# AdmiralenOla/Scoary

Hardware: AMD Instinct MI355X
Metric: gene x permutation Fisher tests/sec (higher is better)
Workload: dtype u32 bit-words (bit-sliced adders / AND + popcount), f64 for Fisher p; 1 GPU; cfg3: 50000 genes x 2000 isolates x 10 traits, --permute 10000 per GPU; counts + Fisher + label permutations + exceedance counts; gene_kind=config, gene_order=config, gene_partition=every rank its own genes (weak scaling), genes_per_gpu=50000, genes_total=50000, isolates=2000, traits=10, permutations=10000, parallelism=gene-shard x1, hip_graph=False, hip_graph_auto=False, label_tiles=generated on every rank, exchange=none (single GPU)

## Files before the change

### __graft_entry__.py

```python
import os
import subprocess
import sys

ROOT = os.path.dirname(os.path.abspath(__file__))
if ROOT not in sys.path:
    sys.path.insert(0, ROOT)

CSRC = os.path.join(ROOT, "scoary_amd", "csrc")
HIP_SRCS = [os.path.join(CSRC, f) for f in ("scoary_context.hip", "scoary_assoc.hip",
                                            "scoary_lists.hip", "scoary_listbuild.hip",
                                            "scoary_mfma.hip", "scoary_labels.hip", "scoary_tree.hip", "scoary_scipy.hip",
                                            "scoary_minp.hip", "scoary_cmh.hip", "scoary_cmh_exact.hip")]
HIP_LIB = os.path.join(ROOT, "scoary_amd", "csrc", "libscoary_hip.so")
HIP_RESOURCES = os.path.join(ROOT, "scoary_amd", "csrc", "libscoary_hip.resources.json")
HIPCC_FLAGS = ["--offload-arch=gfx950", "-O3", "-std=c++17", "-fPIC", "-shared",
               "-ffp-contract=off", "-I" + os.path.join(ROOT, "include"),
               "-Rpass-analysis=kernel-resource-usage"]


def _stale(target, sources):
    if not os.path.exists(target):
        return True
    t = os.path.getmtime(target)
    return any(os.path.getmtime(s) > t for s in sources)


def _hip_deps():
    import glob
    return (HIP_SRCS + glob.glob(os.path.join(CSRC, "*.hpp")) + glob.glob(os.path.join(CSRC, "*.inc"))
            + glob.glob(os.path.join(ROOT, "include", "*.h")))


def parse_resource_usage(text):
    import re
    out, cur = {}, None
    for line in text.splitlines():
        m = re.search(r"remark: (?:\s*)Function Name: (\S+)", line)
        if m:
            cur = out.setdefault(m.group(1), {})
            continue
        m = re.search(r"remark:\s+([A-Za-z ]+?)(?: \[[^\]]*\])?: (\d+)", line)
        if m and cur is not None:
            cur[m.group(1).strip()] = int(m.group(2))
    return out


def _rule(name, count, exclude=None, cap=None, no_static_lds=False):
    return dict(name=name, exclude=exclude, count=count, cap=cap, no_static_lds=no_static_lds)


LIST_RULES = (
    _rule("k_permute_lists", 4, cap=(("VGPRs",), 128), no_static_lds=True),
    _rule("k_permute_seglists", 1, cap=(("VGPRs",), 128), no_static_lds=True),
)
RESOURCE_RULES = LIST_RULES + (
    _rule("k_permute_mfma", 1, cap=(("VGPRs", "AGPRs"), 256)),
    _rule("k_permute_minp", 9, exclude="chunked", cap=(("VGPRs",), 128)),
    _rule("k_permute_minp_chunked", 1),
    _rule("k_stepdown_minp", 18, exclude="chunked", cap=(("VGPRs",), 128)),
    _rule("k_stepdown_minp_chunked", 2),
)
CMH_RULES = (
    _rule("k_cmhE", 1, cap=(("VGPRs",), 128)),
    _rule("k_cmh_support", 1, cap=(("VGPRs",), 128)),
    _rule("k_cmh_fill", 1, cap=(("VGPRs",), 128)),
)
CMH_EXACT_RULES = (
    _rule("k_cmh_exact", 1, cap=(("VGPRs",), 48)),
)
CMH_EXACT_ODDS_RULES = (
    _rule("k_cmh_odds_exact", 1, cap=(("VGPRs",), 152)),
)
CMH_HOMOG_RULES = (
    _rule("k_cmh_homog", 1, cap=(("VGPRs",), 64)),
)


def check_kernel_resources(res, rules=LIST_RULES):
    bad = []
    for rule in rules:
        hit = {k: v for k, v in res.items()
               if rule["name"] in k and not (rule["exclude"] and rule["exclude"] in k)}
        if len(hit) != rule["count"]:
            bad.append("expected %d %s instance%s, compiler reported %d"
                       % (rule["count"], rule["name"], "" if rule["count"] == 1 else "s", len(hit)))
        for name, r in hit.items():
            if r.get("ScratchSize", 0) or r.get("VGPRs Spill", 0) or r.get("SGPRs Spill", 0):
                bad.append("%s: scratch %s, VGPR spills %s, SGPR spills %s" % (
                    name, r.get("ScratchSize"), r.get("VGPRs Spill"), r.get("SGPRs Spill")))
            if rule["cap"]:
                fields, most = rule["cap"]
                if sum(r.get(f, 999) for f in fields) > most:
                    bad.append("%s: %s > %d" % (name, " + ".join("%d %s" % (r.get(f, 999), f) for f in fields), most))
            if rule["no_static_lds"] and r.get("LDS Size", 0) != 0:
                bad.append("%s: static LDS %d bytes (label tile must sit at LDS address 0)" % (name, r["LDS Size"]))
    for name, r in res.items():
        if r.get("ScratchSize", 0) and "k_fisher" not in name:
            bad.append("%s uses %d bytes of scratch per lane" % (name, r["ScratchSize"]))
    if bad:
        raise RuntimeError("libscoary_hip.so: kernel resource check failed:\n  " + "\n  ".join(bad))


def check_ctr_banks():
    import re
    txt = open(os.path.join(CSRC, "scoary_ctr_regs.inc")).read()
    regs = re.findall(r"SCOARY_CTR\((\d+),\s*(\d+),\s*\"v(\d+)\"\)", txt)
    if not regs:
        raise RuntimeError("scoary_ctr_regs.inc: no SCOARY_CTR entries found")
    seen = set()
    for w, k, r in regs:
        w, k, r = int(w), int(k), int(r)
        if r in seen:
            raise RuntimeError("scoary_ctr_regs.inc: v%d pinned twice" % r)
        seen.add(r)
        if (r - w) % 2 == 0:
            raise RuntimeError("scoary_ctr_regs.inc: counter plane (%d, %d) in v%d shares a bank "
                               "with its row words" % (w, k, r))


def check_isa_banks(hipcc, max_frac=0.06):
    import re
    import tempfile
    llvm = os.path.join(os.environ.get("ROCM_PATH", "/opt/rocm"), "lib", "llvm", "bin")
    out = {}
    with tempfile.TemporaryDirectory() as tmp:
        fat, co = os.path.join(tmp, "lists.o"), os.path.join(tmp, "lists.gfx950.o")
        flags = [f for f in HIPCC_FLAGS if f not in ("-shared", "-fPIC") and not f.startswith("-Rpass")]
        subprocess.check_call([hipcc] + flags + ["--cuda-device-only", "-c", "-o", fat,
                                                os.path.join(CSRC, "scoary_lists.hip")],
                              cwd=ROOT, stderr=subprocess.DEVNULL)
        subprocess.check_call([os.path.join(llvm, "clang-offload-bundler"), "--unbundle", "--type=o",
                               "--input=" + fat, "--targets=hipv4-amdgcn-amd-amdhsa--gfx950",
                               "--output=" + co])
        dis = subprocess.run([os.path.join(llvm, "llvm-objdump"), "-d", co], check=True,
                             stdout=subprocess.PIPE, text=True).stdout
    name = None
    for line in dis.splitlines():
        m = re.match(r"[0-9a-f]+ <(\S+)>:", line)
        if m:
            name = m.group(1) if ("k_permute_lists" in m.group(1) or "k_permute_seglists" in m.group(1)) else None
            if name:
                out[name] = [0, 0]
            continue
        if name:
            m = re.search(r"v_bitop3_b32 v\d+, v(\d+), v(\d+), v\d+", line)
            if m:
                out[name][0] += 1
                out[name][1] += int(m.group(1)) % 4 == int(m.group(2)) % 4
    bad = ["%s: %d of %d v_bitop3_b32 have src0 and src1 in one VGPR bank" % (k, same, n)
           for k, (n, same) in out.items() if n == 0 or same > max_frac * n]
    nlists = sum("k_permute_lists" in k for k in out)
    nseg = sum("k_permute_seglists" in k for k in out)
    if nlists != 4 or nseg != 1:
        bad.append("expected 4 k_permute_lists + 1 k_permute_seglists instances in the ISA, found %d + %d"
                   % (nlists, nseg))
    if bad:
        raise RuntimeError("libscoary_hip.so: ISA bank check failed:\n  " + "\n  ".join(bad))
    return out


def build(force=False):
    import json
    if force or _stale(HIP_LIB, _hip_deps()) or not os.path.exists(HIP_RESOURCES):
        hipcc = os.environ.get("HIPCC", "hipcc")
        cmd = [hipcc] + HIPCC_FLAGS + HIP_SRCS + ["-o", HIP_LIB]
        proc = subprocess.run(cmd, cwd=ROOT, stderr=subprocess.PIPE, text=True)
        if proc.returncode != 0:
            sys.stderr.write(proc.stderr)
            raise subprocess.CalledProcessError(proc.returncode, cmd)
        res = parse_resource_usage(proc.stderr)
        try:
            check_kernel_resources(res, RESOURCE_RULES + CMH_RULES + CMH_EXACT_RULES + CMH_EXACT_ODDS_RULES +
                                   CMH_HOMOG_RULES)
            check_ctr_banks()
            for k, (n, same) in check_isa_banks(hipcc).items():
                res.setdefault(k, {}).update({"v_bitop3_b32": n, "v_bitop3_b32 src0/src1 same bank": same})
        except RuntimeError:
            os.remove(HIP_LIB)
            raise
        with open(HIP_RESOURCES, "w") as f:
            json.dump(res, f, indent=1, sort_keys=True)
    io_src = os.path.join(ROOT, "scoary_amd", "csrc", "scoary_io.cpp")
    io_lib = os.path.join(ROOT, "scoary_amd", "csrc", "libscoary_io.so")
    if force or _stale(io_lib, [io_src, os.path.join(ROOT, "include", "scoary_io.h")]):
        subprocess.check_call([os.environ.get("CXX", "g++"), "-O3", "-std=c++17", "-fPIC",
                               "-shared", "-Wall", "-fopenmp", "-ffp-contract=off", "-I" + os.path.join(ROOT, "include"), io_src,
                               "-o", io_lib], cwd=ROOT)
    from oracle import oracle as orc
    orc.build(force=force)
    import scoary_amd
    from scoary_amd import _abi
    if not os.path.exists(_abi.LIB_PATH):
        raise RuntimeError("build() did not produce " + _abi.LIB_PATH)


def smoke():
    import numpy as np
    import torch
    from oracle import oracle as orc
    from scoary_amd.engine import AssociationEngine, pack_bits_rows

    assert torch.cuda.is_available(), "smoke() needs cuda:0"
    torch.cuda.set_device(0)
    rng = np.random.default_rng(5)
    G, N, T, P, seed = 700, 333, 3, 200, 77
    genes = (rng.random((G, N)) < rng.uniform(0.02, 0.98, (G, 1))).astype(np.uint8)
    genes[3] = 0
    genes[4] = 1
    traits = (rng.random((T, N)) < 0.4).astype(np.uint8)
    traits[1, ::29] = 2

    eng = AssociationEngine(0)
    gm = eng.pack_dense(genes)
    tb = pack_bits_rows((traits == 1).astype(np.uint8))
    mb = pack_bits_rows((traits != 2).astype(np.uint8))
    trv, mkv = eng.vecrows(tb, N), eng.vecrows(mb, N)
    dense = eng.associate(gm, trv, mkv, permutations=P, seed=seed, use_lists=False)
    eng.build_lists(gm)
    res = eng.associate(gm, trv, mkv, permutations=P, seed=seed, use_lists=True)
    torch.cuda.synchronize()
    assert np.array_equal(res["r"].cpu().numpy(), dense["r"].cpu().numpy()), \
        "list-driven and dense permutation kernels disagree"

    gb = orc.pack_rows(genes)
    want = orc.counts_packed(gb, tb, mb).transpose(1, 0, 2)
    got = res["counts"].cpu().numpy()
    assert np.array_equal(got, want), "contingency counts differ from the oracle"
    o, p = orc.fisher_many(want.reshape(-1, 4))
    assert np.max(np.abs(res["p"].cpu().numpy().ravel() - p)) < 1e-12, "Fisher p differs"
    r = orc.permute_r(gb, tb, mb, N, P, seed).T
    got_r = res["r"].cpu().numpy().view(np.uint32)
    assert np.array_equal(got_r, r), "permutation exceedance counts differ from the oracle"
    print("smoke ok: %d genes x %d isolates x %d traits x %d permutations, "
          "counts/r bit-exact, max|dp| < 1e-12" % (G, N, T, P))


if __name__ == "__main__":
    build()
    if len(sys.argv) > 1 and sys.argv[1] == "smoke":
        smoke()
```

### include/scoary_hip.h

```cpp
#ifndef SCOARY_HIP_H
#define SCOARY_HIP_H

#include <stdint.h>

#ifdef __cplusplus
extern "C" {
#endif

#define SCOARY_ABI_VERSION 11

#define SCOARY_OK 0
#define SCOARY_ERR_ARG (-1)
#define SCOARY_ERR_HIP (-2)
#define SCOARY_ERR_SIZE (-3)
#define SCOARY_ERR_DEVICE (-4)

typedef struct scoary_ctx *scoary_handle;
typedef void *scoary_stream_t;

int scoary_abi_version(void);

int scoary_create(int device, scoary_handle *out);
void scoary_destroy(scoary_handle h);
const char *scoary_last_error(scoary_handle h);
// ... 10 lines not shown

int scoary_counts(scoary_handle h, const uint32_t *d_tiled,
                  const uint32_t *d_traits, const uint32_t *d_masks, int64_t G,
                  int64_t T, int64_t N, int32_t *d_counts, int32_t *d_margins,
                  scoary_stream_t stream);
int64_t scoary_counts_traits_per_pass(int64_t T);
int64_t scoary_trait_plan_bytes(int64_t T, int64_t N);
int scoary_trait_plan(scoary_handle h, const uint32_t *d_traits, const uint32_t *d_masks,
                      int64_t T, int64_t N, int32_t *d_margins, int32_t *d_mask_class,
                      void *d_plan, scoary_stream_t stream);
int scoary_counts_planned(scoary_handle h, const uint32_t *d_tiled, const void *d_plan,
                          const int32_t *d_margins, int64_t G, int64_t T, int64_t N,
                          int32_t *d_counts, scoary_stream_t stream);

int scoary_fisher(scoary_handle h, const int32_t *d_tables, int64_t M,
                  double *d_p, double *d_or, uint32_t *d_crit,
                  scoary_stream_t stream);
int64_t scoary_fisher_scipy_max_isolates(void);
int scoary_fisher_scipy(scoary_handle h, const int32_t *d_tables, int64_t M, double *d_p,
                        uint64_t *d_skipped, scoary_stream_t stream);
int scoary_fisher_lists(scoary_handle h, const int32_t *d_tables, int64_t T, int64_t G,
                        const int32_t *d_lorder, const uint8_t *d_lflipped,
                        double *d_p, double *d_or, uint32_t *d_crit, uint32_t *d_lcrit,
                        scoary_stream_t stream);

int64_t scoary_perm_max_isolates(void);
int scoary_perm_generate(scoary_handle h, const uint32_t *d_masks,
                         const int32_t *d_margins, int64_t T, int64_t N,
                         int64_t P, int64_t perm_base, int64_t trait_base,
                         uint64_t seed, uint32_t *d_perms, scoary_stream_t stream);

int scoary_permute(scoary_handle h, const uint32_t *d_tiled,
                   const uint32_t *d_perms, const uint32_t *d_crit, int64_t G,
                   int64_t T, int64_t N, int64_t P, uint32_t *d_r,
                   scoary_stream_t stream);

int scoary_permute_seq(scoary_handle h, const uint32_t *d_tiled, const uint32_t *d_perms,
                       const uint32_t *d_crit, const uint32_t *d_thr, int64_t G, int64_t T,
                       int64_t N, int64_t P, int64_t perm_base, uint32_t *d_r,
                       uint32_t *d_nstop, scoary_stream_t stream);

int64_t scoary_minp_fill_scratch_bytes(int64_t entries);
int scoary_minp_plan(scoary_handle h, const int32_t *d_counts, int64_t T, int64_t G, int64_t *d_off,
                     int32_t *d_lo, int64_t *entries_out, scoary_stream_t stream);
int scoary_minp_fill(scoary_handle h, const int32_t *d_counts, const int64_t *d_off,
                     const int32_t *d_lo, int64_t T, int64_t G, int64_t entries, void *d_scratch,
                     double *d_tab, scoary_stream_t stream);
int scoary_permute_minp(scoary_handle h, const uint32_t *d_tiled, const uint32_t *d_perms,
                        const int64_t *d_off, const int32_t *d_lo, const double *d_tab, int64_t G,
                        int64_t T, int64_t N, int64_t P, int64_t perm_base, int64_t minp_stride,
                        double *d_minp, scoary_stream_t stream);

int64_t scoary_stepdown_chunks(scoary_handle h, int64_t G, int64_t T, int64_t P);
int64_t scoary_stepdown_scratch_bytes(scoary_handle h, int64_t G, int64_t T, int64_t N, int64_t P);
int scoary_permute_stepdown(scoary_handle h, const uint32_t *d_tiled, const uint32_t *d_perms,
                            const int64_t *d_off, const int32_t *d_lo, const double *d_tab,
                            const int32_t *d_order, const double *d_psorted, int64_t G, int64_t T,
                            int64_t N, int64_t P, int64_t perm_base, int64_t minp_stride,
                            double *d_minp, uint32_t *d_c, void *d_scratch, scoary_stream_t stream);

int64_t scoary_list_tiles_words(int64_t N, int64_t P, int64_t T);
int64_t scoary_list_tile_words(int64_t N);
int64_t scoary_list_max_isolates(void);
int64_t scoary_list_segments(int64_t N);
int scoary_list_params(int64_t N, int64_t *out5);
int scoary_perm_generate_tiles(scoary_handle h, const uint32_t *d_masks,
                               const int32_t *d_margins, int64_t T, int64_t N, int64_t P,
                               int64_t perm_base, int64_t trait_base, uint64_t seed,
                               uint32_t *d_tiles, scoary_stream_t stream);
int scoary_perm_generate_tiles_range(scoary_handle h, const uint32_t *d_masks,
                                     const int32_t *d_margins, int64_t T, int64_t N, int64_t P,
                                     int64_t perm_base, int64_t trait_base, uint64_t seed,
                                     int64_t first_tile, int64_t n_tiles, uint32_t *d_tiles,
                                     scoary_stream_t stream);
int scoary_perm_max_strata(void);
int64_t scoary_perm_strata_max_isolates(void);
int scoary_strata_margins(scoary_handle h, const uint32_t *d_labels, const uint32_t *d_masks,
                          const uint16_t *d_strata, int64_t T, int64_t N, int64_t S,
                          int32_t *d_smargins, scoary_stream_t stream);
int scoary_perm_generate_strata(scoary_handle h, const uint32_t *d_masks, const uint16_t *d_strata,
                                const int32_t *d_members, const int32_t *d_offsets,
                                const int32_t *d_smargins, int64_t T, int64_t N, int64_t S, int64_t P,
                                int64_t perm_base, int64_t trait_base, uint64_t seed,
                                uint32_t *d_perms, scoary_stream_t stream);
int scoary_perm_generate_tiles_strata_range(scoary_handle h, const uint32_t *d_masks,
                                            const uint16_t *d_strata, const int32_t *d_members,
                                            const int32_t *d_offsets, const int32_t *d_smargins,
                                            int64_t T, int64_t N, int64_t S, int64_t P,
                                            int64_t perm_base, int64_t trait_base, uint64_t seed,
                                            int64_t first_tile, int64_t n_tiles, uint32_t *d_tiles,
                                            scoary_stream_t stream);
int64_t scoary_cmh_scratch_bytes(int64_t N);
int scoary_cmh(scoary_handle h, const uint32_t *d_tiled, const uint32_t *d_labels, const uint32_t *d_masks,
               const uint16_t *d_strata, const int32_t *d_members, const int32_t *d_offsets,
               const int32_t *d_smargins, int64_t G, int64_t T, int64_t N, int64_t S, double *d_stat,
               double *d_p, double *d_odds, double *d_e2, double *d_var, int32_t *d_a, uint32_t *d_crit,
               int32_t *d_scounts, void *d_scratch, scoary_stream_t stream);
int scoary_cmh_minp_plan(scoary_handle h, const uint32_t *d_tiled, const uint32_t *d_masks,
                         const uint16_t *d_strata, const int32_t *d_members, const int32_t *d_offsets,
                         const int32_t *d_smargins, int64_t G, int64_t T, int64_t N, int64_t S,
                         void *d_scratch, int64_t *d_off, int32_t *d_lo, int64_t *entries_out,
                         scoary_stream_t stream);
int scoary_cmh_minp_fill(scoary_handle h, const double *d_e2, const double *d_var, const int64_t *d_off,
                         const int32_t *d_lo, int64_t T, int64_t G, int64_t entries, double *d_tab,
                         scoary_stream_t stream);
int64_t scoary_cmh_exact_max_isolates(void);
int scoary_cmh_exact(scoary_handle h, const uint32_t *d_tiled, const uint32_t *d_masks, const uint16_t *d_strata,
                     const int32_t *d_members, const int32_t *d_offsets, const int32_t *d_smargins, int64_t G,
                     int64_t T, int64_t N, int64_t S, const int32_t *d_a, const uint32_t *d_crit,
                     const int64_t *d_off, const int32_t *d_lo, int64_t entries, double *d_p, double *d_p_region,
                     double *d_tab, void *d_scratch, scoary_stream_t stream);
int scoary_cmh_exact_odds(scoary_handle h, const uint32_t *d_tiled, const uint32_t *d_masks,
                          const uint16_t *d_strata, const int32_t *d_members, const int32_t *d_offsets,
                          const int32_t *d_smargins, int64_t G, int64_t T, int64_t N, int64_t S,
                          const int32_t *d_a, const int64_t *d_off, const int32_t *d_lo, int64_t entries, double half,
                          double *d_or, double *d_or_lo, double *d_or_hi, void *d_scratch,
                          scoary_stream_t stream);
int scoary_cmh_homogeneity(scoary_handle h, const uint32_t *d_tiled, const uint32_t *d_labels,
                           const uint32_t *d_masks, const uint16_t *d_strata, const int32_t *d_members,
                           const int32_t *d_offsets, const int32_t *d_smargins, int64_t G, int64_t T, int64_t N,
                           int64_t S, const double *d_odds, double *d_stat_bd, double *d_stat_tarone, int32_t *d_df,
                           double *d_p, void *d_scratch, scoary_stream_t stream);
int64_t scoary_permute_lists_scratch_bytes(int64_t G, int64_t T, int64_t N, int64_t P);
int scoary_permute_lists(scoary_handle h, const uint32_t *d_tiles, const uint32_t *d_lidx,
                         int64_t entries, const int32_t *d_lstart, const int32_t *d_lngroups,
                         const int32_t *d_lorder, const uint8_t *d_lflipped,
                         const uint32_t *d_crit, const uint32_t *d_lcrit,
                         const int32_t *d_margins, void *d_scratch,
                         int64_t G, int64_t T, int64_t N, int64_t P, uint32_t *d_r,
                         int accumulate, scoary_stream_t stream);

#define SCOARY_MFMA_ROUTE_NONE 0
#define SCOARY_MFMA_ROUTE_ALL 1
#define SCOARY_MFMA_ROUTE_AUTO 2
int64_t scoary_mfma_max_isolates(void);
int64_t scoary_mfma_panels_bytes(int64_t G, int64_t N);
int64_t scoary_mfma_bfrag_bytes(int64_t N, int64_t P, int64_t T);
int64_t scoary_mfma_breakeven_entries(void);
int scoary_mfma_panels_build(scoary_handle h, const uint32_t *d_tiled, int64_t G, int64_t N,
                             const int32_t *d_order, const uint8_t *d_flipped, void *d_panels,
                             scoary_stream_t stream);
int scoary_set_mfma_route(scoary_handle h, int mode);
int64_t scoary_mfma_route(scoary_handle h, const int64_t *block_start, int64_t G, int64_t T,
                          int64_t N, int64_t P);
int scoary_mfma_plan(int num_cu, int64_t k_split, int64_t T, int64_t P, int64_t *out);
int scoary_permute_hybrid(scoary_handle h, const uint32_t *d_tiles, const uint32_t *d_lidx,
                          int64_t entries, const int32_t *d_lstart, const int32_t *d_lngroups,
                          const int32_t *d_lorder, const uint8_t *d_lflipped,
                          const uint32_t *d_crit, const uint32_t *d_lcrit,
                          const int32_t *d_margins, void *d_scratch,
                          int64_t G, int64_t T, int64_t N, int64_t P, uint32_t *d_r,
                          int accumulate, const void *d_panels, void *d_bfrag, int64_t k_split,
                          int64_t routed_entries, scoary_stream_t stream);

int64_t scoary_lists_scratch_bytes(int64_t G, int64_t N);
int64_t scoary_lists_slack_entries(void);
int scoary_lists_plan(scoary_handle h, const uint32_t *d_tiled, int64_t G, int64_t N,
                      void *d_scratch, int32_t *d_start, int32_t *d_ngroups, int32_t *d_order,
                      uint8_t *d_flipped, int64_t *entries_out, scoary_stream_t stream);
int scoary_lists_fill(scoary_handle h, const uint32_t *d_tiled, int64_t G, int64_t N,
                      const void *d_scratch, const int32_t *d_order, const uint8_t *d_flipped,
                      int64_t entries, uint32_t *d_idx, scoary_stream_t stream);


int scoary_hamming(scoary_handle h, const uint32_t *d_tiled, const uint32_t *d_vecrows,
                   int64_t R, int64_t N, int32_t *d_out, scoary_stream_t stream);

int64_t scoary_upgma_scratch_bytes(int64_t n);
int scoary_upgma(scoary_handle h, const int32_t *d_counts, int64_t n, int64_t ncols, void *d_scratch,
                 int32_t *d_merges, int32_t *d_status, scoary_stream_t stream);

int scoary_gather_bits(scoary_handle h, const uint32_t *d_rows, int64_t R, int64_t Wsrc,
                       const int32_t *d_index, int64_t K, uint32_t *d_out,
                       scoary_stream_t stream);

int scoary_tree_pairs(scoary_handle h, const int32_t *d_ops, int64_t nops, int64_t stack_depth,
                      const uint32_t *d_gene_bits, const uint32_t *d_label_bits, int64_t G,
                      int64_t L, int64_t K, int32_t *d_out, scoary_stream_t stream);

int scoary_tree_permute(scoary_handle h, const int32_t *d_ops, int64_t nops,
                        int64_t stack_depth, const uint32_t *d_gene_bits,
                        const uint32_t *d_label_bits, int64_t G, int64_t L, int64_t K,
                        const int32_t *d_obs, uint8_t *d_exceed, scoary_stream_t stream);

int scoary_row_hash(scoary_handle h, const uint32_t *d_tiled, const uint32_t *d_masks,
                    int64_t G, int64_t T, int64_t N, uint64_t *d_out, scoary_stream_t stream);

int scoary_pack_records(scoary_handle h, const int32_t *d_counts, const double *d_p,
                        const double *d_odds, const uint32_t *d_r, const uint32_t *d_nstop,
                        int64_t M, uint32_t *d_rec, scoary_stream_t stream);

int scoary_gather(scoary_handle h, void *rccl_dl, void *comm, const void *d_send, void *d_recv,
                  int64_t bytes, int rank, int nranks, int root, scoary_stream_t stream);

typedef struct scoary_graph *scoary_graph_t;
int scoary_graph_begin(scoary_handle h, scoary_stream_t stream);
int scoary_graph_end(scoary_handle h, scoary_stream_t stream, scoary_graph_t *out);
int scoary_graph_launch(scoary_handle h, scoary_graph_t g, scoary_stream_t stream);
void scoary_graph_destroy(scoary_graph_t g);

int scoary_set_timing(scoary_handle h, int enabled);
int scoary_last_kernel_ms(scoary_handle h, const char *kernel, double *ms_out);

#ifdef __cplusplus
}
#endif
#endif
```

### scoary_amd/_abi.py

```python
import ctypes
import os

_HERE = os.path.dirname(os.path.abspath(__file__))
LIB_PATH = os.environ.get("SCOARY_HIP_LIB") or os.path.join(_HERE, "csrc", "libscoary_hip.so")
HEADER_PATH = os.path.join(os.path.dirname(_HERE), "include", "scoary_hip.h")

ABI_VERSION = 11
PERM_MAX_STRATA = 1024
PERM_STRATA_MAX_ISOLATES = 20479

_i64, _u64, _i32, _vp, _cp = (ctypes.c_int64, ctypes.c_uint64, ctypes.c_int,
                              ctypes.c_void_p, ctypes.c_char_p)

SIGNATURES = {
    "scoary_abi_version": (_i32, []),
    "scoary_create": (_i32, [_i32, ctypes.POINTER(_vp)]),
    "scoary_destroy": (None, [_vp]),
    "scoary_last_error": (_cp, [_vp]),
    "scoary_tiled_quads": (_i64, [_i64]),
    "scoary_tiled_genes": (_i64, [_i64]),
    "scoary_tiled_bytes": (_i64, [_i64, _i64]),
    "scoary_row_words": (_i64, [_i64]),
    "scoary_pack_dense": (_i32, [_vp, _vp, _i64, _i64, _vp, _vp]),
    "scoary_tile_rows": (_i32, [_vp, _vp, _i64, _i64, _vp, _vp]),
    "scoary_counts": (_i32, [_vp, _vp, _vp, _vp, _i64, _i64, _i64, _vp, _vp, _vp]),
    "scoary_counts_traits_per_pass": (_i64, [_i64]),
    "scoary_trait_plan_bytes": (_i64, [_i64, _i64]),
    "scoary_trait_plan": (_i32, [_vp, _vp, _vp, _i64, _i64, _vp, _vp, _vp, _vp]),
    "scoary_counts_planned": (_i32, [_vp, _vp, _vp, _vp, _i64, _i64, _i64, _vp, _vp]),
    "scoary_fisher": (_i32, [_vp, _vp, _i64, _vp, _vp, _vp, _vp]),
    "scoary_fisher_lists": (_i32, [_vp, _vp, _i64, _i64] + [_vp] * 7),
    "scoary_fisher_scipy": (_i32, [_vp, _vp, _i64, _vp, _vp, _vp]),
    "scoary_fisher_scipy_max_isolates": (_i64, []),
    "scoary_perm_generate": (_i32, [_vp, _vp, _vp, _i64, _i64, _i64, _i64, _i64, _u64, _vp, _vp]),
    "scoary_permute": (_i32, [_vp, _vp, _vp, _vp, _i64, _i64, _i64, _i64, _vp, _vp]),
    "scoary_permute_seq": (_i32, [_vp, _vp, _vp, _vp, _vp, _i64, _i64, _i64, _i64, _i64, _vp, _vp,
                                  _vp]),
    "scoary_minp_fill_scratch_bytes": (_i64, [_i64]),
    "scoary_minp_plan": (_i32, [_vp, _vp, _i64, _i64, _vp, _vp, ctypes.POINTER(_i64), _vp]),
    "scoary_minp_fill": (_i32, [_vp, _vp, _vp, _vp, _i64, _i64, _i64, _vp, _vp, _vp]),
    "scoary_permute_minp": (_i32, [_vp] * 6 + [_i64] * 6 + [_vp, _vp]),
    "scoary_stepdown_chunks": (_i64, [_vp, _i64, _i64, _i64]),
    "scoary_stepdown_scratch_bytes": (_i64, [_vp, _i64, _i64, _i64, _i64]),
    "scoary_permute_stepdown": (_i32, [_vp] * 8 + [_i64] * 6 + [_vp] * 4),
    "scoary_list_tiles_words": (_i64, [_i64, _i64, _i64]),
    "scoary_list_tile_words": (_i64, [_i64]),
    "scoary_list_params": (_i32, [_i64, _vp]),
    "scoary_list_max_isolates": (_i64, []),
    "scoary_list_segments": (_i64, [_i64]),
    "scoary_perm_generate_tiles": (_i32, [_vp, _vp, _vp, _i64, _i64, _i64, _i64, _i64, _u64, _vp,
                                          _vp]),
    "scoary_perm_generate_tiles_range": (_i32, [_vp, _vp, _vp, _i64, _i64, _i64, _i64, _i64, _u64, _i64,
                                                _i64, _vp, _vp]),
    "scoary_perm_max_isolates": (_i64, []),
    "scoary_perm_max_strata": (_i32, []),
    "scoary_perm_strata_max_isolates": (_i64, []),
    "scoary_strata_margins": (_i32, [_vp, _vp, _vp, _vp, _i64, _i64, _i64, _vp, _vp]),
    "scoary_perm_generate_strata": (_i32, [_vp] * 6 + [_i64] * 6 + [_u64, _vp, _vp]),
    "scoary_perm_generate_tiles_strata_range": (_i32, [_vp] * 6 + [_i64] * 6 + [_u64, _i64, _i64, _vp, _vp]),
    "scoary_cmh_scratch_bytes": (_i64, [_i64]),
    "scoary_cmh": (_i32, [_vp] * 8 + [_i64] * 4 + [_vp] * 10),
    "scoary_cmh_minp_plan": (_i32, [_vp] * 7 + [_i64] * 4 + [_vp] * 3 + [ctypes.POINTER(_i64), _vp]),
    "scoary_cmh_minp_fill": (_i32, [_vp] * 5 + [_i64] * 3 + [_vp, _vp]),
    "scoary_cmh_exact_max_isolates": (_i64, []),
    "scoary_cmh_exact": (_i32, [_vp] * 7 + [_i64] * 4 + [_vp] * 4 + [_i64] + [_vp] * 5),
    "scoary_cmh_exact_odds": (_i32, [_vp] * 7 + [_i64] * 4 + [_vp] * 3 + [_i64, ctypes.c_double] + [_vp] * 5),
    "scoary_cmh_homogeneity": (_i32, [_vp] * 8 + [_i64] * 4 + [_vp] * 7),
    "scoary_permute_lists_scratch_bytes": (_i64, [_i64, _i64, _i64, _i64]),
    "scoary_permute_lists": (_i32, [_vp, _vp, _vp, _i64] + [_vp] * 8 + [_i64, _i64, _i64, _i64, _vp,
                                                                       _i32, _vp]),
    "scoary_mfma_max_isolates": (_i64, []),
    "scoary_mfma_panels_bytes": (_i64, [_i64, _i64]),
    "scoary_mfma_bfrag_bytes": (_i64, [_i64, _i64, _i64]),
    "scoary_mfma_breakeven_entries": (_i64, []),
    "scoary_mfma_panels_build": (_i32, [_vp, _vp, _i64, _i64, _vp, _vp, _vp, _vp]),
    "scoary_set_mfma_route": (_i32, [_vp, _i32]),
    "scoary_mfma_route": (_i64, [_vp, _vp, _i64, _i64, _i64, _i64]),
    "scoary_mfma_plan": (_i32, [_i32, _i64, _i64, _i64, ctypes.POINTER(_i64)]),
    "scoary_permute_hybrid": (_i32, [_vp, _vp, _vp, _i64] + [_vp] * 8 + [_i64, _i64, _i64, _i64, _vp,
                                                                        _i32, _vp, _vp, _i64, _i64, _vp]),
    "scoary_lists_scratch_bytes": (_i64, [_i64, _i64]),
    "scoary_lists_slack_entries": (_i64, []),
    "scoary_lists_plan": (_i32, [_vp, _vp, _i64, _i64, _vp, _vp, _vp, _vp, _vp,
                                 ctypes.POINTER(_i64), _vp]),
    "scoary_lists_fill": (_i32, [_vp, _vp, _i64, _i64, _vp, _vp, _vp, _i64, _vp, _vp]),
    "scoary_hamming": (_i32, [_vp, _vp, _vp, _i64, _i64, _vp, _vp]),
    "scoary_upgma_scratch_bytes": (_i64, [_i64]),
    "scoary_upgma": (_i32, [_vp, _vp, _i64, _i64, _vp, _vp, _vp, _vp]),
    "scoary_gather_bits": (_i32, [_vp, _vp, _i64, _i64, _vp, _i64, _vp, _vp]),
    "scoary_tree_pairs": (_i32, [_vp, _vp, _i64, _i64, _vp, _vp, _i64, _i64, _i64, _vp, _vp]),
    "scoary_tree_permute": (_i32, [_vp, _vp, _i64, _i64, _vp, _vp, _i64, _i64, _i64, _vp, _vp,
                                   _vp]),
    "scoary_row_hash": (_i32, [_vp, _vp, _vp, _i64, _i64, _i64, _vp, _vp]),
    "scoary_pack_records": (_i32, [_vp, _vp, _vp, _vp, _vp, _vp, _i64, _vp, _vp]),
    "scoary_gather": (_i32, [_vp, _vp, _vp, _vp, _vp, _i64, _i32, _i32, _i32, _vp]),
    "scoary_graph_begin": (_i32, [_vp, _vp]),
    "scoary_graph_end": (_i32, [_vp, _vp, ctypes.POINTER(_vp)]),
    "scoary_graph_launch": (_i32, [_vp, _vp, _vp]),
    "scoary_graph_destroy": (None, [_vp]),
    "scoary_set_timing": (_i32, [_vp, _i32]),
    "scoary_last_kernel_ms": (_i32, [_vp, _cp, ctypes.POINTER(ctypes.c_double)]),
}

_lib = None


class ScoaryHipError(RuntimeError):
    pass


def load():
    global _lib
    if _lib is not None:
        return _lib
    if not os.path.exists(LIB_PATH):
        raise ScoaryHipError(
            "HIP extension not built: %s is missing. Run "
            "`python -c 'import __graft_entry__ as g; g.build()'` (needs hipcc). "
            "scoary_amd has no CPU fallback." % LIB_PATH)
    try:
        import torch
    except ImportError:
        pass
    lib = ctypes.CDLL(LIB_PATH, mode=ctypes.RTLD_GLOBAL)
    for name, (res, args) in SIGNATURES.items():
        fn = getattr(lib, name)
        fn.restype = res
        fn.argtypes = args
    got = lib.scoary_abi_version()
    if got != ABI_VERSION:
        raise ScoaryHipError("ABI version mismatch: library %d, binding %d" % (got, ABI_VERSION))
    if (lib.scoary_perm_max_strata(), lib.scoary_perm_strata_max_isolates()) != \
            (PERM_MAX_STRATA, PERM_STRATA_MAX_ISOLATES):
        raise ScoaryHipError("the library's strata limits differ from the binding's")
    _lib = lib
    return lib
```

### scoary_amd/csrc/scoary_common.hpp

```cpp
#ifndef SCOARY_COMMON_HPP
#define SCOARY_COMMON_HPP
#include <hip/hip_runtime.h>

#include <algorithm>
#include <cmath>
#include <cstdint>
#include <cstdio>
#include <cstdlib>
#include <cstring>
#include <string>
#include <utility>
#include <vector>

#include "scoary_hip.h"

struct scoary_ctx {
  int device = 0;
  int num_cu = 256;
  std::string err;
  bool timing = false;
  int lists_lds_optin = 0;
  int labels_lds_optin = 0;
  int mfma_lds_optin = 0;
  int cmh_exact_lds_optin = 0;
  int cmh_exact_odds_lds_optin = 0;
  int mfma_route = SCOARY_MFMA_ROUTE_AUTO;
  uint32_t* scipy_primes = nullptr;
  float* scipy_inv = nullptr;
  int scipy_nprimes = 0;
  struct Timed {
    std::string name;
    hipEvent_t start, stop;
  };
  std::vector<Timed> timed;
};

struct MfmaGeom {
  int64_t stages, Q, ranges, L, gene_blocks, blocks;
  double cost;
};
MfmaGeom scoary_mfma_geom(int num_cu, int64_t k_split, int64_t T, int64_t P, int64_t ntiles);
int scoary_mfma_launch(scoary_handle h, hipStream_t s, const uint32_t* d_tiles, const void* d_panels, void* d_bfrag,
                       const uint32_t* d_lcrit, uint16_t* d_partial, int64_t k_split, int64_t G, int64_t T,
                       int64_t N, int64_t P, int64_t ntiles, int64_t gs);

int scoary_cmh_segments_launch(scoary_handle h, hipStream_t s, const uint16_t* d_strata, const int32_t* d_members,
                               int64_t N, int64_t S, void* d_scratch, const char* event);

namespace {

constexpr int kWave = 64;
constexpr int kGeneAlign = 256;

using RegQuads = std::integer_sequence<int, 1, 2, 4, 6, 8, 12, 16, 20, 24>;
constexpr int kChunkQuads = 8;

template <int... Q>
constexpr int quads_at_least(std::integer_sequence<int, Q...>, int64_t q) {
  int r = 0;
  ((r = (Q >= q && (r == 0 || Q < r)) ? Q : r), ...);
  return r;
}
template <int... Q>
constexpr int quads_max(std::integer_sequence<int, Q...>) {
  int r = 0;
  ((r = Q > r ? Q : r), ...);
  return r;
}
constexpr int kMaxRegQuads = quads_max(RegQuads{});

template <int... Q, class F>
inline bool with_quads(std::integer_sequence<int, Q...>, int64_t Qp, F&& f) {
  return ((Qp == Q && (f(std::integral_constant<int, Q>{}), true)) || ...);
}
template <class F>
inline bool with_reg_quads(int64_t Qp, F&& f) {
  return with_quads(RegQuads{}, Qp, f);
}

inline int64_t round_up(int64_t x, int64_t m) { return (x + m - 1) / m * m; }

inline int64_t tiled_quads(int64_t N) {
  int64_t q = (((N + 31) / 32) + 3) / 4;
  if (q < 1) q = 1;
  const int r = quads_at_least(RegQuads{}, q);
  return r ? r : round_up(q, kChunkQuads);
}

inline bool tiled_quads_ok(int64_t Qp) {
  return Qp > kMaxRegQuads ? Qp % kChunkQuads == 0 : with_reg_quads(Qp, [](auto) {});
}

constexpr int kSegRows = 20352;
constexpr int kSegTW = 2;
constexpr int kSegStride = ((kSegRows + 1) * kSegTW + 3) / 4 * 4;
constexpr int kSegPiece = 8;
constexpr int kMaxListIsolates = 131070;
__host__ __device__ constexpr int list_segments(int64_t N) {
  return N <= 20479 ? 1 : (N <= kMaxListIsolates ? (int)((N + kSegRows - 1) / kSegRows) : 0);
}
__host__ __device__ constexpr int list_tw(int64_t N) {
  return N <= 2559 ? 16 : (N <= 5119 ? 8 : (N <= 10239 ? 4 : (list_segments(N) ? 2 : 0)));
}
__host__ __device__ constexpr int list_lpg(int TW) { return TW >= 4 ? TW / 4 : 1; }
__host__ __device__ constexpr int list_nw(int TW) { return TW >= 4 ? 4 : TW; }
__host__ __device__ constexpr int64_t list_tile_dwords(int64_t N, int TW) {
  return ((N + 1) * TW + 3) / 4 * 4;
}
__host__ __device__ constexpr int64_t list_tile_dwords_seg(int64_t N, int TW) {
  return list_segments(N) > 1 ? (int64_t)list_segments(N) * kSegStride : list_tile_dwords(N, TW);
}
__host__ __device__ constexpr int64_t list_seg_rows(int64_t N, int s) {
  return list_segments(N) > 1 ? (N - (int64_t)s * kSegRows < kSegRows ? N - (int64_t)s * kSegRows : kSegRows) : N;
}
__host__ __device__ constexpr int64_t list_row_dword(int64_t N, int64_t row) {
  return list_segments(N) > 1 ? row / kSegRows * kSegStride + row % kSegRows * kSegTW : row * kSegTW;
}

constexpr int kListPad = 16;
constexpr int kListStartUnit = 32;
constexpr int kListChunkMB = 2;
constexpr int kListSlack = 256;

int fail(scoary_handle h, int code, const std::string& msg) {
  if (h) h->err = msg;
  return code;
}

inline int check_args(scoary_handle h, const char* what, bool ok) {
  return ok ? SCOARY_OK : fail(h, SCOARY_ERR_ARG, std::string(what) + ": bad argument");
}
inline int strata_check(scoary_handle h, const char* what, bool ok, int64_t T, int64_t N, int64_t S) {
  if (int rc = check_args(h, what, ok && T >= 1 && N >= 1 && S >= 1)) return rc;
  if (T > 65535) return fail(h, SCOARY_ERR_SIZE, std::string(what) + ": T > 65535");
  if (S > scoary_perm_max_strata())
    return fail(h, SCOARY_ERR_SIZE, std::string(what) + ": more strata than scoary_perm_max_strata()");
  if (N > scoary_perm_strata_max_isolates())
    return fail(h, SCOARY_ERR_SIZE, std::string(what) + ": more isolates than scoary_perm_strata_max_isolates()");
  return SCOARY_OK;
}

#define HIP_TRY(h, expr)                                                              \
  do {                                                                                \
    hipError_t e_ = (expr);                                                           \
    if (e_ != hipSuccess)                                                             \
      return fail(h, SCOARY_ERR_HIP, std::string(#expr) + ": " + hipGetErrorString(e_)); \
  } while (0)

struct DeviceGuard {
  int prev = -1;
  bool switched = false;
  explicit DeviceGuard(int dev) {
    if (hipGetDevice(&prev) == hipSuccess && prev != dev) switched = (hipSetDevice(dev) == hipSuccess);
  }
  ~DeviceGuard() {
    if (switched) (void)hipSetDevice(prev);
  }
};

struct KernelTimer {
  scoary_handle h;
  hipStream_t s;
  hipEvent_t start = nullptr, stop = nullptr;
  KernelTimer(scoary_handle h_, hipStream_t s_, const char* name) : h(h_), s(s_) {
    if (!name || !h->timing) return;
    if (hipEventCreate(&start) != hipSuccess || hipEventCreate(&stop) != hipSuccess) {
      start = stop = nullptr;
      return;
    }
    (void)hipEventRecord(start, s);
    h->timed.push_back({name, start, stop});
  }
  ~KernelTimer() {
    if (stop) (void)hipEventRecord(stop, s);
  }
};

__device__ __forceinline__ void philox4x32_10(uint32_t c0, uint32_t c1, uint32_t c2, uint32_t c3,
                                              uint32_t k0, uint32_t k1, uint32_t (&out)[4]) {
#pragma unroll
  for (int r = 0; r < 10; ++r) {
    const uint64_t p0 = (uint64_t)0xD2511F53u * c0, p1 = (uint64_t)0xCD9E8D57u * c2;
    const uint32_t h0 = (uint32_t)(p0 >> 32), l0 = (uint32_t)p0;
    const uint32_t h1 = (uint32_t)(p1 >> 32), l1 = (uint32_t)p1;
    const uint32_t n0 = __builtin_amdgcn_bitop3_b32(h1, c1, k0, 0x96), n2 = __builtin_amdgcn_bitop3_b32(h0, c3, k1, 0x96);
    c0 = n0;
    c1 = l1;
    c2 = n2;
    c3 = l0;
    k0 += 0x9E3779B9u;
    k1 += 0xBB67AE85u;
  }
  out[0] = c0;
  out[1] = c1;
  out[2] = c2;
  out[3] = c3;
}

struct CmhSegments {
  uint32_t count, pad[3];
  uint2 seg[1];
};

__device__ __forceinline__ void bcnt_acc(uint32_t& acc, uint32_t x) {
  asm("v_bcnt_u32_b32 %0, %1, %0" : "+v"(acc) : "v"(x));
}

__device__ __forceinline__ void and_popc(uint32_t& acc, const uint4 a, const uint4 b) {
  bcnt_acc(acc, a.x & b.x);
  bcnt_acc(acc, a.y & b.y);
  bcnt_acc(acc, a.z & b.z);
  bcnt_acc(acc, a.w & b.w);
}


template <int THREADS, class T, class Op>
__device__ __forceinline__ void block_scan(T* s, int idx, Op op) {
  __syncthreads();
  for (int o = 1; o < THREADS; o <<= 1) {
    const T v = idx >= o ? s[idx - o] : T(0);
    __syncthreads();
    s[idx] = op(s[idx], v);
    __syncthreads();
  }
}

__global__ __launch_bounds__(1024) void k_minp_scan(int64_t* __restrict__ off, int64_t M) {
  __shared__ int64_t s_wave[16];
  __shared__ int64_t s_carry;
  const int tid = threadIdx.x, lane = tid & 63, wave = tid >> 6;
  if (tid == 0) s_carry = 0;
  __syncthreads();
  for (int64_t base = 0; base < M; base += 1024) {
    const int64_t i = base + tid;
    const int64_t v = i < M ? off[i] : 0;
    int64_t x = v;
#pragma unroll
    for (int d = 1; d < 64; d <<= 1) {
      const int64_t y = __shfl_up(x, d);
      if (lane >= d) x += y;
    }
    if (lane == 63) s_wave[wave] = x;
    __syncthreads();
    int64_t before = s_carry;
    for (int w = 0; w < wave; ++w) before += s_wave[w];
    if (i < M) off[i] = before + x - v;
    __syncthreads();
    if (tid == 1023) s_carry = before + x;
    __syncthreads();
  }
  if (tid == 0) off[M] = s_carry;
}

}
#endif
```

### scoary_amd/csrc/scoary_labels.hip

```cpp
#include "scoary_common.hpp"

namespace {

constexpr uint32_t kDomBernLo = 0x53434F42u;
constexpr uint32_t kDomBernHi = 0x53434F43u;
constexpr uint32_t kDomFix = 0x53434F44u;
constexpr uint32_t kFixMaxCalls = 1u << 20;
constexpr int kCntPlanes = 10;
constexpr int kSumPlanes = 16;
constexpr int kMaxRowsPerThread = (1 << kCntPlanes) - 1;
constexpr int kLabelsMaxLds = 160 * 1024;

struct LabelPlan {
  uint32_t m, q;
  bool flip;
};
__device__ __forceinline__ uint32_t isqrt64(uint64_t v) {
  uint64_t r = 0;
  for (int s = 31; s >= 0; --s) {
    const uint64_t c = r | ((uint64_t)1 << s);
    if (c * c <= v) r = c;
  }
  return (uint32_t)r;
}
__device__ __forceinline__ LabelPlan label_plan(int32_t npos_i, int32_t nval_i) {
  const int64_t npos = npos_i, nval = nval_i;
  LabelPlan p;
  p.flip = 2 * npos > nval;
  const int64_t m = p.flip ? nval - npos : npos;
  p.m = m > 0 ? (uint32_t)m : 0u;
  p.q = 0u;
  if (m > 0 && nval > 0) {
    const uint64_t s = isqrt64((uint64_t)m * (uint64_t)(nval - m) / (uint64_t)nval);
    const uint64_t b = 12u * s * (uint64_t)(nval - 2 * m) / (5u * (uint64_t)nval);
    const uint64_t target = (uint64_t)m > b ? (uint64_t)m - b : 0u;
    p.q = (uint32_t)(256u * target / (uint64_t)nval);
  }
  return p;
}

__device__ __forceinline__ uint32_t bern_word(uint32_t i, uint32_t B, uint32_t t, uint32_t q,
                                              uint32_t k0, uint32_t k1) {
  uint32_t x = 0u, r[4];
  if (q == 0u) return 0u;
  if (q & 0xFu) {
    philox4x32_10(i, B, t, kDomBernLo, k0, k1, r);
#pragma unroll
    for (int j = 0; j < 4; ++j) x = ((q >> j) & 1u) ? (x | r[j]) : (x & r[j]);
  }
  philox4x32_10(i, B, t, kDomBernHi, k0, k1, r);
#pragma unroll
  for (int j = 0; j < 4; ++j) x = ((q >> (4 + j)) & 1u) ? (x | r[j]) : (x & r[j]);
  return x;
}

struct LabelArgs {
  const uint32_t* masks;
  const int32_t* margins;
  int N, Wp;
  int64_t P, perm_base;
  int trait_base;
  uint32_t k0, k1;
  int elt_log2;
  int ntiles, TW;
  int64_t first_flat, nflat;
  uint32_t* out;
};

template <int NB>
struct LabelBlock {
  int t, bit0;
  uint32_t Bglob;
  uint32_t* tile_base;
  uint32_t live[NB];
};
template <int NB, int OUT, bool SUB>
__device__ __forceinline__ bool label_block(const LabelArgs& a, LabelBlock<NB>& b) {
  const int elt_log2 = SUB ? a.elt_log2 : 5;
  const int elt = 1 << elt_log2;
  const int subs = 32 >> elt_log2;
  int64_t lc0 = 0;
  b.tile_base = nullptr;
  if constexpr (OUT == 0) {
    const int units = a.TW * subs / NB;
    const int64_t id = blockIdx.x;
    const int64_t qd = id >> 3;
    const int unit = (int)(qd % units);
    const int64_t fl = (qd / units) * 8 + (id & 7);
    if (fl >= a.nflat) return false;
    const int64_t f = a.first_flat + fl;
    b.t = (int)(f / a.ntiles);
    const int tile = (int)(f % a.ntiles);
    const int col = unit / subs * NB;
    b.bit0 = (unit % subs) * elt;
    lc0 = (int64_t)tile * a.TW + col;
    b.Bglob = (uint32_t)((a.perm_base >> 5) + lc0);
    b.tile_base = a.out + f * list_tile_dwords_seg(a.N, a.TW) + col;
  } else {
    b.t = blockIdx.y;
    b.Bglob = (uint32_t)((a.perm_base >> 5) + blockIdx.x / subs);
    b.bit0 = (int)(blockIdx.x % subs) * elt;
  }
#pragma unroll
  for (int w = 0; w < NB; ++w) {
    int64_t lo, hi;
    if constexpr (OUT == 0) {
      lo = 0;
      hi = a.P - (lc0 + w) * 32;
    } else {
      const int64_t first = (int64_t)(b.Bglob + w) * 32;
      lo = a.perm_base - first;
      hi = a.perm_base + a.P - first;
    }
    lo = lo < 0 ? 0 : (lo > 32 ? 32 : lo);
    hi = hi < 0 ? 0 : (hi > 32 ? 32 : hi);
    const uint32_t below_hi = hi >= 32 ? 0xffffffffu : ((1u << hi) - 1u);
    const uint32_t below_lo = lo >= 32 ? 0xffffffffu : ((1u << lo) - 1u);
    b.live[w] = hi > lo ? (below_hi & ~below_lo) : 0u;
  }
  return true;
}

template <class I>
struct LdsMap {
  I vm, own, end;
  __host__ __device__ I bytes() const { return end * 4; }
};
template <class I>
__host__ __device__ inline LdsMap<I> lds_map(I N, int stride_bits, I own_dwords) {
  LdsMap<I> m;
  m.vm = (((N * stride_bits + 31) >> 5) + 3) & ~(I)3;
  m.own = m.vm + ((((N + 31) >> 5) + 3) & ~(I)3);
  m.end = m.own + own_dwords;
  return m;
}
template <class I>
__host__ __device__ inline LdsMap<I> labels_lds(I N, int elt, int NB) { return lds_map<I>(N, elt * NB, 32 * NB); }
template <class I>
__host__ __device__ inline LdsMap<I> strata_lds(I N, int NB, I S) {
  return lds_map<I>(N, 32 * NB, 4 * S + (N + 1) / 2);
}

template <int NB>
__device__ __forceinline__ void store_row0(uint32_t* xs, int row, const uint32_t (&x)[NB], int elt_log2) {
  if (elt_log2 == 5) {
    if constexpr (NB == 2) {
      *reinterpret_cast<uint2*>(xs + (int64_t)row * 2) = make_uint2(x[0], x[1]);
    } else {
      xs[row] = x[0];
    }
  } else if (x[0]) {
    const uint32_t bp = (uint32_t)row << elt_log2;
    atomicOr(&xs[bp >> 5], x[0] << (bp & 31u));
  }
}

struct FixGroup {
  uint32_t* xs;
  const uint32_t* vm;
  uint32_t stride_bits;
  int L, l, pidx;
  bool in_group, alive;
  uint32_t pi;
  uint64_t gmask;
  uint32_t tglob, k0, k1;
};
template <int NB>
__device__ __forceinline__ FixGroup fix_group(const LabelArgs& a, const LabelBlock<NB>& b, uint32_t* xs,
                                              const uint32_t* vm, int nperm) {
  const int tid = threadIdx.x, lane = tid & 63;
  FixGroup g;
  g.xs = xs, g.vm = vm, g.stride_bits = (uint32_t)nperm;
  g.L = min(kWave, (int)blockDim.x / nperm);
  g.pidx = tid / g.L, g.l = tid & (g.L - 1);
  g.in_group = g.pidx < nperm;
  const int w = g.pidx >> 5, j = g.pidx & 31;
  g.alive = g.in_group && ((((w & (NB - 1)) ? b.live[NB - 1] : b.live[0]) >> (b.bit0 + j)) & 1u);
  g.pi = (b.Bglob + (uint32_t)w) * 32u + (uint32_t)(b.bit0 + j);
  g.gmask = (g.L == 64 ? ~(uint64_t)0 : (((uint64_t)1 << g.L) - 1)) << (lane & ~(g.L - 1));
  g.tglob = (uint32_t)(a.trait_base + b.t), g.k0 = a.k0, g.k1 = a.k1;
  return g;
}
template <class Iso>
__device__ __forceinline__ int toggle4(const FixGroup& g, const uint32_t (&rnd)[4], bool add, uint32_t n,
                                       uint32_t reject_below, Iso iso) {
  uint32_t idx[4], bit[4];
  bool ok[4];
#pragma unroll
  for (int u = 0; u < 4; ++u) {
    const uint64_t prod = (uint64_t)rnd[u] * (uint64_t)n;
    const uint32_t pos = iso((uint32_t)(prod >> 32));
    const uint32_t bp = pos * g.stride_bits + (uint32_t)g.pidx;
    idx[u] = bp >> 5;
    bit[u] = 1u << (bp & 31u);
    ok[u] = (uint32_t)prod >= reject_below;
    if (add) ok[u] = ok[u] && ((g.vm[pos >> 5] >> (pos & 31u)) & 1u);
  }
  uint32_t old[4];
#pragma unroll
  for (int u = 0; u < 4; ++u) {
    old[u] = add ? bit[u] : 0u;
    if (ok[u])
      old[u] = add ? __hip_atomic_fetch_or(&g.xs[idx[u]], bit[u], __ATOMIC_RELAXED, __HIP_MEMORY_SCOPE_WORKGROUP)
                   : __hip_atomic_fetch_and(&g.xs[idx[u]], ~bit[u], __ATOMIC_RELAXED, __HIP_MEMORY_SCOPE_WORKGROUP);
  }
  int won = 0;
#pragma unroll
  for (int u = 0; u < 4; ++u) won += add ? ((old[u] & bit[u]) ? 0 : 1) : ((old[u] & bit[u]) ? 1 : 0);
  return won;
}
template <class Iso>
__device__ __forceinline__ int toggle1(const FixGroup& g, uint32_t rnd, bool add, uint32_t n, uint32_t reject_below,
                                       Iso iso) {
  const uint64_t prod = (uint64_t)rnd * (uint64_t)n;
  if ((uint32_t)prod < reject_below) return 0;
  const uint32_t pos = iso((uint32_t)(prod >> 32));
  const uint32_t bp = pos * g.stride_bits + (uint32_t)g.pidx, b1 = 1u << (bp & 31u);
  if (add) {
    if (!((g.vm[pos >> 5] >> (pos & 31u)) & 1u)) return 0;
    return (__hip_atomic_fetch_or(&g.xs[bp >> 5], b1, __ATOMIC_RELAXED, __HIP_MEMORY_SCOPE_WORKGROUP) & b1) ? 0 : 1;
  }
  return (__hip_atomic_fetch_and(&g.xs[bp >> 5], ~b1, __ATOMIC_RELAXED, __HIP_MEMORY_SCOPE_WORKGROUP) & b1) ? 1 : 0;
}
template <bool CLAMP, class Iso>
__device__ __forceinline__ void fix_rounds(const FixGroup& g, int& d, uint32_t& base, uint32_t ctr_hi, uint32_t n,
                                           uint32_t reject_below, Iso iso) {
  while ((d >= 4 || d <= -4) && base < kFixMaxCalls) {
    const bool add = d > 0;
    const int need = add ? d : -d;
    int k = min(g.L, need >> 2);
    if constexpr (CLAMP) k = min(k, (int)(kFixMaxCalls - base));
    uint32_t r[4];
    int won = 0;
    if (g.l < k) {
      philox4x32_10(ctr_hi | (base + (uint32_t)g.l), g.pi, g.tglob, kDomFix, g.k0, g.k1, r);
      won = toggle4(g, r, add, n, reject_below, iso);
    }
    int got = 0;
#pragma unroll
    for (int bitn = 0; bitn < 3; ++bitn) got += __popcll(__ballot((won >> bitn) & 1) & g.gmask) << bitn;
    d = add ? d - got : d + got;
    base += (uint32_t)k;
  }
}
template <class Iso>
__device__ __forceinline__ void fix_tail(const FixGroup& g, int d, uint32_t base, uint32_t ctr_hi, uint32_t n,
                                         uint32_t reject_below, Iso iso) {
  const bool add = d > 0;
  int left = add ? d : -d;
  while (left > 0 && base < kFixMaxCalls) {
    uint32_t r[4];
    philox4x32_10(ctr_hi | base, g.pi, g.tglob, kDomFix, g.k0, g.k1, r);
#pragma unroll
    for (int u = 0; u < 4; ++u)
      if (left > 0) left -= toggle1(g, r[u], add, n, reject_below, iso);
    ++base;
  }
}

template <int NB, int OUT, class RowField>
__device__ __forceinline__ void emit_labels(const LabelArgs& a, const LabelBlock<NB>& b, RowField row_field) {
  const int tid = threadIdx.x, lane = tid & 63, tpb = blockDim.x, nwaves = tpb >> 6;
  const int wave = __builtin_amdgcn_readfirstlane(tid >> 6);
  const int N = a.N, elt = 1 << a.elt_log2, bit0 = b.bit0;
  uint32_t* tile_base = b.tile_base;
  if constexpr (OUT == 0) {
    const bool seg = a.TW == kSegTW;
    auto row_off = [&](int64_t row) -> int64_t { return seg ? list_row_dword(N, row) : row * a.TW; };
    if (elt == 32) {
      for (int row = tid; row < N; row += tpb) {
        uint32_t* dst = tile_base + row_off(row);
        if constexpr (NB == 2) {
          *reinterpret_cast<uint2*>(dst) = make_uint2(row_field(row, 0), row_field(row, 1));
        } else {
          dst[0] = row_field(row, 0);
        }
      }
    } else {
      for (int row = tid; row < N; row += tpb) {
        uint8_t* dst = reinterpret_cast<uint8_t*>(tile_base + row_off(row)) + (bit0 >> 3);
        const uint32_t f = row_field(row, 0);
        if (elt == 16) *reinterpret_cast<uint16_t*>(dst) = (uint16_t)f;
        else *dst = (uint8_t)f;
      }
    }
    const int nseg = seg ? list_segments(N) : 1;
    if (tid < nseg) {
      const int64_t z = nseg > 1 ? (int64_t)tid * kSegStride + list_seg_rows(N, tid) * kSegTW : row_off(N);
      if (elt == 32) {
#pragma unroll
        for (int w = 0; w < NB; ++w) tile_base[z + w] = 0u;
      } else {
        uint8_t* dst = reinterpret_cast<uint8_t*>(tile_base + z) + (bit0 >> 3);
        if (elt == 16) *reinterpret_cast<uint16_t*>(dst) = 0;
        else *dst = 0;
      }
    }
  } else {
    static_assert(OUT == 0 || NB == 1, "bit rows: one dword column per block");
    const int nchunks = (N + 63) >> 6;
    const int64_t pl = (int64_t)b.Bglob * 32 + bit0 + lane - a.perm_base;
    const bool mine = lane < elt && ((b.live[0] >> (bit0 + (lane & 31))) & 1u);
    uint32_t* prow = a.out + ((int64_t)b.t * a.P + (mine ? pl : 0)) * a.Wp;
    for (int c = wave; c < nchunks; c += nwaves) {
      const int row = c * 64 + lane;
      const uint32_t f = row < N ? row_field(row, 0) : 0u;
      uint32_t lo = 0u, hi = 0u;
      for (int j = 0; j < elt; ++j) {
        const uint64_t m64 = __ballot((f >> j) & 1u);
        if (lane == j) {
          lo = (uint32_t)m64;
          hi = (uint32_t)(m64 >> 32);
        }
      }
      if (mine) *reinterpret_cast<uint2*>(prow + 2 * c) = make_uint2(lo, hi);
    }
    if (mine)
      for (int k = 2 * nchunks + wave; k < a.Wp; k += nwaves) prow[k] = 0u;
  }
}

template <int NB, int OUT>
__global__ __launch_bounds__(1024) void k_labels(const LabelArgs a) {
  extern __shared__ __attribute__((aligned(16))) uint32_t lds[];
  const int tid = threadIdx.x, lane = tid & 63, tpb = blockDim.x;
  const int N = a.N;
  const int elt = 1 << a.elt_log2;
  LabelBlock<NB> blk;
  if (!label_block<NB, OUT, true>(a, blk)) return;
  const int t = blk.t, bit0 = blk.bit0;
  const uint32_t Bglob = blk.Bglob;
  const uint32_t (&live)[NB] = blk.live;
  const uint32_t fieldmask = elt == 32 ? 0xffffffffu : ((1u << elt) - 1u);
  const uint32_t tglob = (uint32_t)(a.trait_base + t);
  const LabelPlan plan = label_plan(__builtin_amdgcn_readfirstlane(a.margins[2 * t]),
                                    __builtin_amdgcn_readfirstlane(a.margins[2 * t + 1]));
  const uint32_t* mrow = a.masks + (int64_t)t * a.Wp;

  const LdsMap<int> lm = labels_lds(N, elt, NB);
  uint32_t* xs = lds;
  uint32_t* vm = lds + lm.vm;
  int* kc = reinterpret_cast<int*>(lds + lm.own);
  const int nmw = (N + 31) >> 5;
  for (int k = tid; k < nmw; k += tpb) vm[k] = mrow[k];
  if (tid < 32 * NB) kc[tid] = 0;
  if (elt != 32) {
    for (int k = tid; k < lm.vm; k += tpb) xs[k] = 0u;
    __syncthreads();
  }

  uint32_t cp[NB][kCntPlanes];
#pragma unroll
  for (int w = 0; w < NB; ++w)
#pragma unroll
    for (int k = 0; k < kCntPlanes; ++k) cp[w][k] = 0u;
  const int rows_per_thread = (N + tpb - 1) / tpb;
  const int kpl = 32 - __builtin_clz((unsigned)rows_per_thread | 1u);
  for (int row = tid; row < N; row += tpb) {
    const bool valid = (mrow[row >> 5] >> (row & 31)) & 1u;
    uint32_t x[NB];
#pragma unroll
    for (int w = 0; w < NB; ++w) {
      x[w] = 0u;
      if (valid)
        x[w] = ((bern_word((uint32_t)row, Bglob + (uint32_t)w, tglob, plan.q, a.k0, a.k1) & live[w]) >> bit0) &
               fieldmask;
      uint32_t carry = x[w];
#pragma unroll
      for (int k = 0; k < kCntPlanes; ++k)
        if (k < kpl) {
          const uint32_t nc = cp[w][k] & carry;
          cp[w][k] ^= carry;
          carry = nc;
        }
    }
    store_row0<NB>(xs, row, x, a.elt_log2);
  }
#pragma unroll
  for (int w = 0; w < NB; ++w) {
    uint32_t c[kSumPlanes];
#pragma unroll
    for (int k = 0; k < kSumPlanes; ++k) c[k] = k < kCntPlanes ? cp[w][k] : 0u;
#pragma unroll
    for (int s = 0; s < 6; ++s) {
      uint32_t carry = 0u;
#pragma unroll
      for (int k = 0; k < kSumPlanes; ++k)
        if (k < kpl + s + 1) {
          const uint32_t y = (uint32_t)__shfl_xor((int)c[k], 1 << s);
          const uint32_t sum = c[k] ^ y ^ carry;
          carry = (c[k] & y) | (carry & (c[k] | y));
          c[k] = sum;
        }
    }
    if (lane < 32) {
      int K = 0;
#pragma unroll
      for (int k = 0; k < kSumPlanes; ++k) K |= (int)((c[k] >> lane) & 1u) << k;
      cp[w][0] = (uint32_t)K;
    }
  }
  __syncthreads();
  if (lane < 32) {
#pragma unroll
    for (int w = 0; w < NB; ++w)
      if (cp[w][0]) atomicAdd(&kc[w * 32 + lane], (int)cp[w][0]);
  }
  __syncthreads();

  {
    const FixGroup g = fix_group<NB>(a, blk, xs, vm, elt * NB);
    int d = g.alive ? (int)plan.m - kc[g.in_group ? g.pidx : 0] : 0;
    const uint32_t reject_below = (uint32_t)(((uint64_t)1 << 32) % (uint64_t)N);
    const auto isolate = [](uint32_t pos) { return pos; };
    uint32_t base = 0;
    fix_rounds<false>(g, d, base, 0u, (uint32_t)N, reject_below, isolate);
    if (g.l == 0) fix_tail(g, d, base, 0u, (uint32_t)N, reject_below, isolate);
  }
  __syncthreads();

  auto row_field = [&](int row, int w) -> uint32_t {
    uint32_t f;
    if (elt == 32) {
      f = xs[(int64_t)row * NB + w];
    } else {
      const uint32_t bp = (uint32_t)row << a.elt_log2;
      f = (xs[bp >> 5] >> (bp & 31u)) & fieldmask;
    }
    if (plan.flip) {
      const bool valid = (vm[row >> 5] >> (row & 31)) & 1u;
      f = valid ? (~f & (live[w] >> bit0) & fieldmask) : 0u;
    }
    return f;
  };
  emit_labels<NB, OUT>(a, blk, row_field);
}

constexpr int kMaxStrata = 1024;
constexpr int kStrataMaxIsolates = 20479;

struct StrataArgs {
  const uint16_t* strata;
  const int32_t* members;
  const int32_t* offsets;
  const int32_t* smargins;
  int S;
};

template <int NB, int OUT>
__global__ __launch_bounds__(1024) void k_labels_strata(const LabelArgs a, const StrataArgs sa) {
  extern __shared__ __attribute__((aligned(16))) uint32_t lds[];
  const int tid = threadIdx.x, tpb = blockDim.x;
  const int N = a.N, S = sa.S;
  LabelBlock<NB> blk;
  if (!label_block<NB, OUT, false>(a, blk)) return;
  const int t = blk.t;
  const uint32_t Bglob = blk.Bglob;
  const uint32_t (&live)[NB] = blk.live;
  const uint32_t tglob = (uint32_t)(a.trait_base + t);
  const uint32_t* mrow = a.masks + (int64_t)t * a.Wp;

  const LdsMap<int> lm = strata_lds(N, NB, S);
  const int nmw = (N + 31) >> 5;
  uint32_t* xs = lds;
  uint32_t* vm = lds + lm.vm;
  uint4* tab = reinterpret_cast<uint4*>(lds + lm.own);
  uint16_t* mem = reinterpret_cast<uint16_t*>(tab + S);
  for (int k = tid; k < nmw; k += tpb) vm[k] = mrow[k];
  for (int s = tid; s < S; s += tpb) {
    const int off = min(max(sa.offsets[s], 0), N);
    const int n = min(max(sa.offsets[s + 1] - off, 0), N - off);
    const int32_t* mg = sa.smargins + ((int64_t)t * S + s) * 2;
    const LabelPlan plan = label_plan(mg[0], mg[1]);
    const uint32_t rej = n > 0 ? (0u - (uint32_t)n) % (uint32_t)n : 0u;
    tab[s] = make_uint4(plan.m, (uint32_t)n, rej, (uint32_t)off | (plan.q << 16) | ((plan.flip ? 1u : 0u) << 24));
  }
  for (int k = tid; k < N; k += tpb) mem[k] = (uint16_t)min(max(sa.members[k], 0), N - 1);
  __syncthreads();
  auto stratum_of = [&](int row) -> uint32_t { return tab[min((int)sa.strata[row], S - 1)].w; };

  for (int row = tid; row < N; row += tpb) {
    const bool valid = (vm[row >> 5] >> (row & 31)) & 1u;
    uint32_t x[NB];
#pragma unroll
    for (int w = 0; w < NB; ++w) x[w] = 0u;
    if (valid) {
      const uint32_t q = (stratum_of(row) >> 16) & 0xffu;
#pragma unroll
      for (int w = 0; w < NB; ++w)
        x[w] = bern_word((uint32_t)row, Bglob + (uint32_t)w, tglob, q, a.k0, a.k1) & live[w];
    }
    store_row0<NB>(xs, row, x, 5);
  }
  __syncthreads();

  {
    const FixGroup g = fix_group<NB>(a, blk, xs, vm, 32 * NB);
    const int L = g.L, l = g.l, j = g.pidx & 31;
    const uint32_t* xw = xs + (g.pidx >> 5);
    const auto member_at = [mem](uint32_t off) {
      return [mem, off](uint32_t pos) -> uint32_t { return mem[off + pos]; };
    };
    for (int s0 = 0; s0 < S; s0 += L) {
      int my_d = 0;
      uint32_t my_base = 0;
      const int s1 = min(S, s0 + L);
      for (int s = s0; s < s1; ++s) {
        const uint4 e = tab[s];
        const uint32_t n = e.y, off = e.w & 0xffffu;
        if (n == 0u) continue;
        int K = 0;
        if (g.alive)
          for (uint32_t k = (uint32_t)l; k < n; k += (uint32_t)L) K += (xw[(uint32_t)mem[off + k] * NB] >> j) & 1u;
        for (int o = 1; o < L; o <<= 1) K += __shfl_xor(K, o);
        int d = g.alive ? (int)e.x - K : 0;
        uint32_t base = 0;
        fix_rounds<true>(g, d, base, (uint32_t)s << 20, n, e.z, member_at(off));
        if (l == s - s0) my_d = d, my_base = base;
      }
      if (my_d != 0) {
        const uint4 e = tab[s0 + l];
        fix_tail(g, my_d, my_base, (uint32_t)(s0 + l) << 20, e.y, e.z, member_at(e.w & 0xffffu));
      }
    }
  }
  __syncthreads();

  auto row_field = [&](int row, int w) -> uint32_t {
    uint32_t f = xs[(int64_t)row * NB + w];
    if ((stratum_of(row) >> 24) & 1u) {
      const bool valid = (vm[row >> 5] >> (row & 31)) & 1u;
      f = valid ? (~f & live[w]) : 0u;
    }
    return f;
  };
  emit_labels<NB, OUT>(a, blk, row_field);
}

__global__ __launch_bounds__(256) void k_strata_margins(const uint32_t* __restrict__ labels,
                                                        const uint32_t* __restrict__ masks,
                                                        const uint16_t* __restrict__ strata, int N, int Wp, int S,
                                                        int32_t* __restrict__ out) {
  __shared__ int hist[2 * kMaxStrata];
  const int t = blockIdx.x, tid = threadIdx.x;
  for (int k = tid; k < 2 * S; k += blockDim.x) hist[k] = 0;
  __syncthreads();
  const uint32_t* lrow = labels + (int64_t)t * Wp;
  const uint32_t* mrow = masks + (int64_t)t * Wp;
  for (int row = tid; row < N; row += blockDim.x) {
    const uint32_t valid = (mrow[row >> 5] >> (row & 31)) & 1u;
    if (!valid) continue;
    const int s = min((int)strata[row], S - 1);
    if ((lrow[row >> 5] >> (row & 31)) & 1u) atomicAdd(&hist[2 * s], 1);
    atomicAdd(&hist[2 * s + 1], 1);
  }
  __syncthreads();
  for (int k = tid; k < 2 * S; k += blockDim.x) out[(int64_t)t * 2 * S + k] = hist[k];
}

int labels_elt(int64_t N, int min_elt) {
  for (int elt = 32; elt >= min_elt; elt >>= 1)
    if (labels_lds(N, elt, 1).bytes() <= kLabelsMaxLds) return elt;
  return 0;
}
int ilog2(int v) {
  int l = 0;
  while ((1 << l) < v) ++l;
  return l;
}
int labels_threads(int64_t blocks, int64_t N, int num_cu) {
  int tpb = 256;
  while (tpb < 1024 && blocks * (tpb / 64) < (int64_t)num_cu * 8 && N / tpb >= 4) tpb *= 2;
  while (tpb < 1024 && (N + tpb - 1) / tpb > kMaxRowsPerThread) tpb *= 2;
  return tpb;
}
template <class... Args>
int launch_block(scoary_handle h, hipStream_t s, void (*kernel)(Args...), int optin_bit, int64_t lds_bytes,
                 bool fits, const char* why, dim3 grid, int tpb, const Args&... args) {
  if (tpb < 64 || tpb > 1024 || (tpb & (tpb - 1)) || !fits) return fail(h, SCOARY_ERR_SIZE, why);
  const void* fn = reinterpret_cast<const void*>(kernel);
  if (lds_bytes > 64 * 1024 && !(h->labels_lds_optin & optin_bit)) {
    HIP_TRY(h, hipFuncSetAttribute(fn, hipFuncAttributeMaxDynamicSharedMemorySize, kLabelsMaxLds));
    h->labels_lds_optin |= optin_bit;
  }
  hipLaunchKernelGGL(kernel, grid, dim3((unsigned)tpb), (size_t)lds_bytes, s, args...);
  HIP_TRY(h, hipGetLastError());
  return SCOARY_OK;
}
int launch_labels(scoary_handle h, hipStream_t s, const LabelArgs& a, int NB, int OUT, dim3 grid, int tpb) {
  const bool fits = (int64_t)tpb * kMaxRowsPerThread >= a.N;
  return launch_block(h, s, OUT ? k_labels<1, 1> : (NB == 2 ? k_labels<2, 0> : k_labels<1, 0>),
                      1 << (NB + 8 * OUT) , labels_lds<int64_t>(a.N, 1 << a.elt_log2, NB).bytes(), fits,
                      "k_labels: more than 1023 isolates per thread (or a block size that is no power of two in "
                      "64..1024)", grid, tpb, a);
}
int launch_labels_strata(scoary_handle h, hipStream_t s, const LabelArgs& a, const StrataArgs& sa, int NB, int OUT,
                         dim3 grid, int tpb) {
  const int64_t lds_bytes = strata_lds<int64_t>(a.N, NB, sa.S).bytes();
  return launch_block(h, s, OUT ? k_labels_strata<1, 1> : (NB == 2 ? k_labels_strata<2, 0> : k_labels_strata<1, 0>),
                      1 << (16 + NB + 8 * OUT), lds_bytes, lds_bytes <= kLabelsMaxLds,
                      "k_labels_strata: rows, members and the stratum table do not fit LDS (or a block size that is "
                      "no power of two in 64..1024)", grid, tpb, a, sa);
}

LabelArgs label_args(const uint32_t* d_masks, const int32_t* d_margins, int64_t N, int64_t P, int64_t perm_base,
                     int64_t trait_base, uint64_t seed, int elt, uint32_t* d_out) {
  LabelArgs a{};
  a.masks = d_masks, a.margins = d_margins, a.N = (int)N, a.Wp = (int)scoary_row_words(N);
  a.P = P, a.perm_base = perm_base, a.trait_base = (int)trait_base;
  a.k0 = (uint32_t)seed, a.k1 = (uint32_t)(seed >> 32), a.elt_log2 = ilog2(elt), a.out = d_out;
  return a;
}

int check_tile_base(scoary_handle h, const char* what, int64_t perm_base) {
  return (perm_base & 31) ? fail(h, SCOARY_ERR_ARG, std::string(what) + ": perm_base must be a multiple of 32")
                          : SCOARY_OK;
}
int check_grid(scoary_handle h, const char* what, int64_t gx) {
  return gx > 0x7fffffffLL ? fail(h, SCOARY_ERR_SIZE, std::string(what) + ": grid too large") : SCOARY_OK;
}

int64_t row_blocks(int64_t perm_base, int64_t P, int elt) {
  return (((perm_base + P - 1) >> 5) - (perm_base >> 5) + 1) * (32 / elt);
}

struct TileShape {
  int TW, NB, tpb;
  int64_t ntiles, gx;
};
template <class Lds>
int tile_shape(scoary_handle h, const char* what, int64_t T, int64_t N, int64_t P, int64_t first_tile,
               int64_t n_tiles, int elt, Lds lds, TileShape& ts) {
  ts = TileShape{};
  ts.TW = list_tw(N);
  if (!ts.TW) return fail(h, SCOARY_ERR_SIZE, std::string(what) + ": N too large for LDS tiles");
  const int64_t tile_perms = ts.TW * 32;
  ts.ntiles = (P + tile_perms - 1) / tile_perms;
  if (first_tile + n_tiles > T * ts.ntiles)
    return fail(h, SCOARY_ERR_ARG, std::string(what) + ": tile range past the last (trait, tile)");
  if (n_tiles == 0) return SCOARY_OK;
  if (!elt) return fail(h, SCOARY_ERR_SIZE, std::string(what) + ": N too large for the label generator");
  ts.NB = (elt == 32 && 2 <= ts.TW && n_tiles * (ts.TW / 2) >= 2 * (int64_t)h->num_cu &&
           lds(2).bytes() <= kLabelsMaxLds / 2) ? 2 : 1;
  const int64_t units = (int64_t)ts.TW * (32 / elt) / ts.NB;
  ts.gx = (n_tiles + 7) / 8 * 8 * units;
  if (int rc = check_grid(h, what, ts.gx)) return rc;
  ts.tpb = labels_threads(n_tiles * units, N, h->num_cu);
  return SCOARY_OK;
}
void tile_args(LabelArgs& a, const TileShape& ts, int64_t first_tile, int64_t n_tiles) {
  a.ntiles = (int)ts.ntiles, a.TW = ts.TW, a.first_flat = first_tile, a.nflat = n_tiles;
}

}

extern "C" {

int64_t scoary_perm_max_isolates(void) {
  int64_t lo = 1, hi = (int64_t)1 << 24;
  while (lo < hi) {
    const int64_t mid = (lo + hi + 1) / 2;
    if (labels_elt(mid, 1)) lo = mid; else hi = mid - 1;
  }
  return lo;
}

int scoary_perm_generate(scoary_handle h, const uint32_t* d_masks, const int32_t* d_margins,
                         int64_t T, int64_t N, int64_t P, int64_t perm_base, int64_t trait_base,
                         uint64_t seed, uint32_t* d_perms, scoary_stream_t stream) {
  const char* what = "scoary_perm_generate";
  if (!h) return SCOARY_ERR_ARG;
  if (int rc = check_args(h, what, d_masks && d_margins && d_perms && T >= 1 && N >= 1 && P >= 1 && perm_base >= 0 &&
                                       trait_base >= 0))
    return rc;
  if (T > 65535 || trait_base + T > 0x7fffffffLL || perm_base + P > 0xffffffffLL)
    return fail(h, SCOARY_ERR_SIZE, "scoary_perm_generate: T > 65535 or permutation index >= 2^32");
  const int elt = labels_elt(N, 1);
  if (!elt) return fail(h, SCOARY_ERR_SIZE, "scoary_perm_generate: more isolates than scoary_perm_max_isolates()");
  DeviceGuard guard(h->device);
  hipStream_t s = static_cast<hipStream_t>(stream);
  const LabelArgs a = label_args(d_masks, d_margins, N, P, perm_base, trait_base, seed, elt, d_perms);
  const int64_t gx = row_blocks(perm_base, P, elt);
  if (int rc = check_grid(h, what, gx)) return rc;
  KernelTimer kt(h, s, "k_perm_generate");
  return launch_labels(h, s, a, 1, 1, dim3((unsigned)gx, (unsigned)T), labels_threads(gx * T, N, h->num_cu));
}

int scoary_perm_generate_tiles_range(scoary_handle h, const uint32_t* d_masks, const int32_t* d_margins,
                                     int64_t T, int64_t N, int64_t P, int64_t perm_base,
                                     int64_t trait_base, uint64_t seed, int64_t first_tile,
                                     int64_t n_tiles, uint32_t* d_tiles, scoary_stream_t stream) {
  const char* what = "scoary_perm_generate_tiles";
  if (!h) return SCOARY_ERR_ARG;
  if (int rc = check_args(h, what, d_masks && d_margins && d_tiles && T >= 1 && N >= 1 && P >= 1 && perm_base >= 0 &&
                                       trait_base >= 0 && first_tile >= 0 && n_tiles >= 0))
    return rc;
  if (int rc = check_tile_base(h, what, perm_base)) return rc;
  if (T > 65535 || perm_base + P > 0xffffffffLL)
    return fail(h, SCOARY_ERR_SIZE, "scoary_perm_generate_tiles: T > 65535 or permutation index >= 2^32");
  const int elt = labels_elt(N, 8);
  TileShape ts;
  if (int rc = tile_shape(h, what, T, N, P, first_tile, n_tiles, elt,
                          [&](int nb) { return labels_lds(N, 32, nb); }, ts))
    return rc;
  if (ts.gx == 0) return SCOARY_OK;
  DeviceGuard guard(h->device);
  hipStream_t s = static_cast<hipStream_t>(stream);
  LabelArgs a = label_args(d_masks, d_margins, N, P, perm_base, trait_base, seed, elt, d_tiles);
  tile_args(a, ts, first_tile, n_tiles);
  KernelTimer kt(h, s, "k_perm_generate_tiles");
  return launch_labels(h, s, a, ts.NB, 0, dim3((unsigned)ts.gx), ts.tpb);
}

int scoary_perm_generate_tiles(scoary_handle h, const uint32_t* d_masks, const int32_t* d_margins,
                               int64_t T, int64_t N, int64_t P, int64_t perm_base,
                               int64_t trait_base, uint64_t seed, uint32_t* d_tiles,
                               scoary_stream_t stream) {
  const int TW = list_tw(N);
  const int64_t ntiles = TW && P > 0 ? (P + TW * 32 - 1) / (TW * 32) : 0;
  return scoary_perm_generate_tiles_range(h, d_masks, d_margins, T, N, P, perm_base, trait_base, seed,
                                          0, T * ntiles, d_tiles, stream);
}


int scoary_perm_max_strata(void) { return kMaxStrata; }
int64_t scoary_perm_strata_max_isolates(void) { return kStrataMaxIsolates; }

int scoary_strata_margins(scoary_handle h, const uint32_t* d_labels, const uint32_t* d_masks,
                          const uint16_t* d_strata, int64_t T, int64_t N, int64_t S, int32_t* d_smargins,
                          scoary_stream_t stream) {
  if (!h) return SCOARY_ERR_ARG;
  if (int rc = strata_check(h, "scoary_strata_margins", d_labels && d_masks && d_strata && d_smargins, T, N, S))
    return rc;
  DeviceGuard guard(h->device);
  hipStream_t s = static_cast<hipStream_t>(stream);
  KernelTimer kt(h, s, "k_strata_margins");
  hipLaunchKernelGGL(k_strata_margins, dim3((unsigned)T), dim3(256), 0, s, d_labels, d_masks, d_strata, (int)N,
                     (int)scoary_row_words(N), (int)S, d_smargins);
  HIP_TRY(h, hipGetLastError());
  return SCOARY_OK;
}

int scoary_perm_generate_strata(scoary_handle h, const uint32_t* d_masks, const uint16_t* d_strata,
                                const int32_t* d_members, const int32_t* d_offsets, const int32_t* d_smargins,
                                int64_t T, int64_t N, int64_t S, int64_t P, int64_t perm_base, int64_t trait_base,
                                uint64_t seed, uint32_t* d_perms, scoary_stream_t stream) {
  const char* what = "scoary_perm_generate_strata";
  if (!h) return SCOARY_ERR_ARG;
  if (int rc = strata_check(h, what, d_masks && d_strata && d_members && d_offsets && d_smargins && d_perms &&
                                         P >= 1 && perm_base >= 0 && trait_base >= 0, T, N, S))
    return rc;
  if (trait_base + T > 0x7fffffffLL || perm_base + P > 0xffffffffLL)
    return fail(h, SCOARY_ERR_SIZE, "scoary_perm_generate_strata: permutation index >= 2^32");
  DeviceGuard guard(h->device);
  hipStream_t s = static_cast<hipStream_t>(stream);
  const LabelArgs a = label_args(d_masks, nullptr, N, P, perm_base, trait_base, seed, 32, d_perms);
  const StrataArgs sa{d_strata, d_members, d_offsets, d_smargins, (int)S};
  const int64_t gx = row_blocks(perm_base, P, 32);
  if (int rc = check_grid(h, what, gx)) return rc;
  KernelTimer kt(h, s, "k_perm_generate_strata");
  return launch_labels_strata(h, s, a, sa, 1, 1, dim3((unsigned)gx, (unsigned)T),
                              labels_threads(gx * T, N, h->num_cu));
}

int scoary_perm_generate_tiles_strata_range(scoary_handle h, const uint32_t* d_masks, const uint16_t* d_strata,
                                            const int32_t* d_members, const int32_t* d_offsets,
                                            const int32_t* d_smargins, int64_t T, int64_t N, int64_t S, int64_t P,
                                            int64_t perm_base, int64_t trait_base, uint64_t seed,
                                            int64_t first_tile, int64_t n_tiles, uint32_t* d_tiles,
                                            scoary_stream_t stream) {
  const char* what = "scoary_perm_generate_tiles_strata_range";
  if (!h) return SCOARY_ERR_ARG;
  if (int rc = strata_check(h, what, d_masks && d_strata && d_members && d_offsets && d_smargins && d_tiles &&
                                         P >= 1 && perm_base >= 0 && trait_base >= 0 && first_tile >= 0 &&
                                         n_tiles >= 0, T, N, S))
    return rc;
  if (int rc = check_tile_base(h, what, perm_base)) return rc;
  if (trait_base + T > 0x7fffffffLL || perm_base + P > 0xffffffffLL)
    return fail(h, SCOARY_ERR_SIZE, "scoary_perm_generate_tiles_strata_range: permutation index >= 2^32");
  TileShape ts;
  if (int rc = tile_shape(h, what, T, N, P, first_tile, n_tiles, 32,
                          [&](int nb) { return strata_lds(N, nb, S); }, ts))
    return rc;
  if (ts.gx == 0) return SCOARY_OK;
  DeviceGuard guard(h->device);
  hipStream_t s = static_cast<hipStream_t>(stream);
  LabelArgs a = label_args(d_masks, nullptr, N, P, perm_base, trait_base, seed, 32, d_tiles);
  tile_args(a, ts, first_tile, n_tiles);
  const StrataArgs sa{d_strata, d_members, d_offsets, d_smargins, (int)S};
  KernelTimer kt(h, s, "k_perm_generate_tiles_strata");
  return launch_labels_strata(h, s, a, sa, ts.NB, 0, dim3((unsigned)ts.gx), ts.tpb);
}

}
```

### scoary_amd/csrc/scoary_lists.hip

```cpp
#include "scoary_common.hpp"

namespace {


__device__ __forceinline__ void scoary_bank_defs() {
  asm volatile(".ifndef scoary_bank_defs\n"
               ".set scoary_bank_defs, 1\n"
#include "scoary_vgpr_banks.inc"
               ".endif");
}
#define SCOARY_SYM3(LUT)                                                        \
  ".if scoary_bank_%1 != scoary_bank_%2\n v_bitop3_b32 %0, %1, %2, %3 bitop3:" LUT \
  "\n.elseif scoary_bank_%1 != scoary_bank_%3\n v_bitop3_b32 %0, %1, %3, %2 bitop3:" LUT \
  "\n.else\n v_bitop3_b32 %0, %2, %3, %1 bitop3:" LUT "\n.endif"
__device__ __forceinline__ uint32_t bit_xor3(uint32_t a, uint32_t b, uint32_t c) {
  uint32_t d;
  asm(SCOARY_SYM3("0x96") : "=v"(d) : "v"(a), "v"(b), "v"(c));
  return d;
}
__device__ __forceinline__ uint32_t bit_maj(uint32_t a, uint32_t b, uint32_t c) {
  uint32_t d;
  asm(SCOARY_SYM3("0xe8") : "=v"(d) : "v"(a), "v"(b), "v"(c));
  return d;
}
// ... 268 lines not shown
                                                           const uint32_t* __restrict__ lidx,
                                                           const int32_t* __restrict__ lstart,
                                                           const int32_t* __restrict__ lngroups,
                                                           const uint2* __restrict__ lcrit, int G,
                                                           int N, int64_t P, int ntiles,
                                                           int groups_per_block, int64_t lidx_bytes,
                                                           int nseg, uint16_t* __restrict__ partial) {
  extern __shared__ __attribute__((aligned(16))) uint32_t tile_lds[];
  scoary_bank_defs();
  constexpr int LPG = 1, NW = kSegTW, TW = kSegTW, GPW = kWave;
  static_assert(kSegTW == 2, "two permutation words per lane");
  const int ngroups = (G + GPW - 1) / GPW;
  const int t = blockIdx.x / ntiles, tile = blockIdx.x % ntiles;
  const int tid = threadIdx.x, lane = tid & 63, nwaves = blockDim.x >> 6;
  const int wave = __builtin_amdgcn_readfirstlane(tid >> 6);
  const int q_lo = blockIdx.y * groups_per_block;
  const int q_hi = min(ngroups, q_lo + groups_per_block);
  const uint32_t lane_off = (uint32_t)lane * 16u;
  uint16_t* out = partial + (int64_t)blockIdx.x * ((int64_t)ngroups * GPW);
  const uint32_t lds0 = (uint32_t)(uintptr_t)(const __attribute__((address_space(3))) uint32_t*)tile_lds;
  const uint32_t three = 3u;
  const uint32_t* src = tiles + (int64_t)blockIdx.x * ((int64_t)nseg * kSegStride);
  const int rounds = (q_hi - q_lo + nwaves - 1) / nwaves;
  for (int rnd = 0; rnd < rounds; ++rnd) {
    const int q = q_lo + rnd * nwaves + wave;
    const bool active = q < q_hi;
    uint32_t c0[16], c1[16], c2[16], c3[16];
#pragma unroll
    for (int k = 0; k < 16; ++k) c0[k] = c1[k] = c2[k] = c3[k] = 0u;
    for (int sgm = 0; sgm < nseg; ++sgm) {
      const int64_t qg = (int64_t)min(q, q_hi - 1) * GPW;
      const Group cur = open_group(lidx, lstart, lngroups, (int64_t)sgm * G + qg, 2, lidx_bytes);
      Ent ring[4] = {load_from(cur, lane_off, 0), load_from(cur, lane_off, 1), load_from(cur, lane_off, 2),
                     load_from(cur, lane_off, 3)};
      __syncthreads();
      {
        const uint4* src4 = reinterpret_cast<const uint4*>(src + (int64_t)sgm * kSegStride);
        constexpr int n4 = kSegStride / 4;
        for (int i = wave * kWave; i < n4; i += nwaves * kWave)
          if (i + lane < n4) lds_dma16(lds0 + (uint32_t)i * 16u, lane_off, src4 + i);
        asm volatile("s_waitcnt vmcnt(0)" ::: "memory");
      }
      __syncthreads();
      if (active) {
        const int nhalf = cur.nhalf;
        const int nsuper = (nhalf + 1) >> 1;
        constexpr int kVecSub = 2;
#define SCOARY_READ4(H, X, E) read4x4_half<H>(X, E, three)
#include "scoary_list_walk.inc"
#undef SCOARY_READ4
      }
    }
    if (active) {
      const int lg = fresh_lane();
      const int slot = min(q * GPW + lg, G - 1);
      const bool have = q * GPW + lg < G;
      const uint2 cr = lcrit[(int64_t)t * G + slot];
      uint32_t valid[NW];
#pragma unroll
      for (int w = 0; w < NW; ++w) {
        const int64_t p_first = ((int64_t)tile * TW + w) * 32;
        valid[w] = p_first >= P ? 0u : (P - p_first >= 32 ? 0xffffffffu : ((1u << (P - p_first)) - 1u));
      }
      int cnt = __popc(region_bits<KC>(c0, cr.x, cr.y) & valid[0]) +
                __popc(region_bits<KC>(c1, cr.x, cr.y) & valid[1]);
      if (!have) cnt = 0;
      out[(int64_t)q * GPW + lg] = (uint16_t)cnt;
    }
  }
}

__global__ __launch_bounds__(256) void k_lists_reduce(const uint16_t* __restrict__ partial,
                                                      int ntiles, int64_t gs, int G,
                                                      const int32_t* __restrict__ order,
                                                      int accumulate, uint32_t* __restrict__ r) {
  __shared__ uint32_t s_part[4][kWave];
  const int lane = threadIdx.x & 63, part = threadIdx.x >> 6;
  const int k = blockIdx.x * kWave + lane;
  const int t = blockIdx.y;
  uint32_t sum = 0u;
  if (k < G) {
    const uint16_t* in = partial + (int64_t)t * ntiles * gs + k;
#pragma unroll 4
    for (int tile = part; tile < ntiles; tile += 4) sum += in[(int64_t)tile * gs];
  }
  s_part[part][lane] = sum;
  __syncthreads();
  if (part != 0 || k >= G) return;
  sum = s_part[0][lane] + s_part[1][lane] + s_part[2][lane] + s_part[3][lane];
  uint32_t* dst = r + (int64_t)t * G + order[k];
  *dst = accumulate ? *dst + sum : sum;
}

}

extern "C" {

int64_t scoary_list_tiles_words(int64_t N, int64_t P, int64_t T) {
  const int TW = list_tw(N);
  if (!TW) return 0;
  const int64_t tile_perms = TW * 32;
  const int64_t ntiles = (P + tile_perms - 1) / tile_perms;
  return T * ntiles * list_tile_dwords_seg(N, TW);
}
int64_t scoary_list_tile_words(int64_t N) { return list_tw(N) ? list_tile_dwords_seg(N, list_tw(N)) : 0; }
int64_t scoary_list_max_isolates(void) { return kMaxListIsolates; }
int64_t scoary_list_segments(int64_t N) { return N < 1 ? 0 : list_segments(N); }
int scoary_list_params(int64_t N, int64_t* out5) {
  if (!out5) return SCOARY_ERR_ARG;
  const int TW = list_tw(N);
  out5[0] = TW;
  out5[1] = TW * 4;
  out5[2] = TW ? kWave / list_lpg(TW) : 0;
  out5[3] = TW ? 64 / TW : 0;
  out5[4] = TW ? (list_segments(N) > 1 ? kSegPiece : 4 * list_lpg(TW)) : 0;
  return TW ? SCOARY_OK : SCOARY_ERR_SIZE;
}

extern "C++" {
static int64_t list_chunk_bytes(int TW) {
  return (int64_t)(TW <= 4 ? 16 : kListChunkMB) << 20;
}
struct ListGeom {
  int64_t ntiles, ngroups, gs, gpb, chunks;
};
static ListGeom list_geom(int num_cu, int64_t G, int64_t T, int64_t N, int64_t P, int64_t entries,
                          int64_t first = 0) {
  ListGeom g{};
  const int TW = list_tw(N), GPW = kWave / list_lpg(TW);
  const int64_t tile_perms = TW * 32;
  g.ntiles = (P + tile_perms - 1) / tile_perms;
  g.ngroups = (G + GPW - 1) / GPW;
  g.gs = g.ngroups * GPW;
  int64_t chunks = ((int64_t)num_cu * 16 + g.ntiles * T - 1) / (g.ntiles * T);
  const int64_t chunk_bytes = list_chunk_bytes(TW);
  const int64_t by_l2 = (entries * 4 + chunk_bytes - 1) / chunk_bytes;
  if (chunks < by_l2) chunks = by_l2;
  if (chunks > 65535) chunks = 65535;
  if (chunks < 1) chunks = 1;
  const int64_t walked = g.ngroups - first;
  g.gpb = (walked + chunks - 1) / chunks;
  g.gpb = (g.gpb + 15) / 16 * 16;
  g.chunks = g.gpb ? (walked + g.gpb - 1) / g.gpb : 0;
  return g;
}

template <typename Kernel, typename... Extra>
static int launch_lists(scoary_handle h, hipStream_t s, Kernel kernel, const char* name, size_t lds, int optin,
                        const uint32_t* d_tiles, const uint32_t* d_lidx, int64_t entries,
                        const int32_t* d_lstart, const int32_t* d_lngroups, const int32_t* d_lorder,
                        const uint8_t* d_lflipped, const uint32_t* d_crit, const uint32_t* d_lcrit_in,
                        const int32_t* d_margins, uint32_t* d_scratch, int64_t G, int64_t T, int64_t N,
                        int64_t P, uint32_t* d_r, int accumulate, const void* d_panels, void* d_bfrag,
                        int64_t k_split, int64_t routed_entries, Extra... extra) {
  uint32_t* d_lcrit_sc = d_scratch;
  uint16_t* d_partial = reinterpret_cast<uint16_t*>(d_scratch + 2 * T * G);
  const uint32_t* d_lcrit = d_lcrit_in ? d_lcrit_in : d_lcrit_sc;
  if (!d_lcrit_in) {
    KernelTimer kt(h, s, "k_lists_crit");
    hipLaunchKernelGGL(k_lists_crit, dim3((unsigned)((G + 255) / 256), (unsigned)T), dim3(256), 0, s,
                       reinterpret_cast<const uint2*>(d_crit), d_margins, d_lorder, d_lflipped,
                       (int)G, reinterpret_cast<uint2*>(d_lcrit_sc));
  }
  const int64_t gpw = kWave / list_lpg(list_tw(N));
  const int64_t q_first = (k_split + gpw - 1) / gpw;
  const ListGeom g = list_geom(h->num_cu, G, T, N, P, entries - routed_entries, q_first);
  if (k_split > 0) {
    const int rc = scoary_mfma_launch(h, s, d_tiles, d_panels, d_bfrag, d_lcrit, d_partial, k_split, G, T, N, P,
                                      g.ntiles, g.gs);
    if (rc != SCOARY_OK) return rc;
  }
  if (T * g.ntiles > 0x7fffffffLL || g.chunks > 65535)
    return fail(h, SCOARY_ERR_SIZE, "scoary_permute_lists: grid too large");
  if (!(h->lists_lds_optin & optin)) {
    const void* fn = reinterpret_cast<const void*>(kernel);
    hipFuncAttributes attr;
    HIP_TRY(h, hipFuncGetAttributes(&attr, fn));
    if (attr.sharedSizeBytes != 0)
      return fail(h, SCOARY_ERR_SIZE, std::string("scoary_permute_lists: ") + name +
                                          " has static LDS; the label tile would not sit at LDS address 0");
    HIP_TRY(h, hipFuncSetAttribute(fn, hipFuncAttributeMaxDynamicSharedMemorySize, 160 * 1024));
    h->lists_lds_optin |= optin;
  }
  if (g.chunks > 0) {
    KernelTimer kt(h, s, name);
    hipLaunchKernelGGL(kernel, dim3((unsigned)(T * g.ntiles), (unsigned)g.chunks), dim3(1024), lds, s, d_tiles,
                       d_lidx, d_lstart, d_lngroups, reinterpret_cast<const uint2*>(d_lcrit), (int)G,
                       (int)N, P, (int)g.ntiles, (int)g.gpb,
                       (entries + kListSlack) * (int64_t)sizeof(uint32_t), extra..., d_partial);
  }
  {
    KernelTimer kt(h, s, "k_lists_reduce");
    hipLaunchKernelGGL(k_lists_reduce, dim3((unsigned)((G + kWave - 1) / kWave), (unsigned)T), dim3(256), 0, s,
                       d_partial, (int)g.ntiles, g.gs, (int)G, d_lorder, accumulate, d_r);
  }
  HIP_TRY(h, hipGetLastError());
  return SCOARY_OK;
}
}

int64_t scoary_permute_lists_scratch_bytes(int64_t G, int64_t T, int64_t N, int64_t P) {
  if (G < 1 || T < 1 || N < 1 || P < 1 || !list_tw(N)) return 0;
  const ListGeom g = list_geom(256, G, T, N, P, 0);
  return 2 * T * G * (int64_t)sizeof(uint32_t) + (T * g.ntiles * g.gs * (int64_t)sizeof(uint16_t) + 3) / 4 * 4;
}

int scoary_permute_lists(scoary_handle h, const uint32_t* d_tiles, const uint32_t* d_lidx,
                         int64_t entries, const int32_t* d_lstart, const int32_t* d_lngroups,
                         const int32_t* d_lorder, const uint8_t* d_lflipped,
                         const uint32_t* d_crit, const uint32_t* d_lcrit, const int32_t* d_margins,
                         void* d_scratch, int64_t G, int64_t T, int64_t N, int64_t P,
                         uint32_t* d_r, int accumulate, scoary_stream_t stream) {
  return scoary_permute_hybrid(h, d_tiles, d_lidx, entries, d_lstart, d_lngroups, d_lorder, d_lflipped, d_crit,
                               d_lcrit, d_margins, d_scratch, G, T, N, P, d_r, accumulate, nullptr, nullptr, 0, 0,
                               stream);
}

int scoary_permute_hybrid(scoary_handle h, const uint32_t* d_tiles, const uint32_t* d_lidx,
                          int64_t entries, const int32_t* d_lstart, const int32_t* d_lngroups,
                          const int32_t* d_lorder, const uint8_t* d_lflipped,
                          const uint32_t* d_crit, const uint32_t* d_lcrit, const int32_t* d_margins,
                          void* d_scratch, int64_t G, int64_t T, int64_t N, int64_t P,
                          uint32_t* d_r, int accumulate, const void* d_panels, void* d_bfrag,
                          int64_t k_split, int64_t routed_entries, scoary_stream_t stream) {
  if (!h) return SCOARY_ERR_ARG;
  if (k_split < 0 || k_split > G || routed_entries < 0 || routed_entries > entries ||
      (k_split > 0 && (!d_panels || !d_bfrag || N > scoary_mfma_max_isolates() ||
                       (k_split % 256 != 0 && k_split != G))))
    return fail(h, SCOARY_ERR_ARG, "scoary_permute_hybrid: bad k_split (scoary_mfma_route gives a valid one)");
  if (!d_tiles || !d_lidx || !d_lstart || !d_lngroups || !d_lorder || !d_lflipped ||
      (!d_crit && !d_lcrit) || (!d_lcrit && !d_margins) || !d_scratch || !d_r || G < 1 || T < 1 ||
      N < 1 || P < 1 || entries < 0)
    return fail(h, SCOARY_ERR_ARG, "scoary_permute_lists: bad argument");
  const int TW = list_tw(N);
  if (!TW)
    return fail(h, SCOARY_ERR_SIZE, "scoary_permute_lists: label tile does not fit in LDS for this N");
  if (T > 65535) return fail(h, SCOARY_ERR_SIZE, "scoary_permute_lists: T > 65535");
  DeviceGuard guard(h->device);
  hipStream_t s = static_cast<hipStream_t>(stream);
  uint32_t* sc = static_cast<uint32_t*>(d_scratch);
  if (list_segments(N) > 1)
    return launch_lists(h, s, &k_permute_seglists<16>, "k_permute_seglists", (size_t)kSegStride * sizeof(uint32_t),
                        32, d_tiles, d_lidx, entries, d_lstart, d_lngroups, d_lorder, d_lflipped, d_crit, d_lcrit,
                        d_margins, sc, G, T, N, P, d_r, accumulate, nullptr, nullptr, 0, 0, list_segments(N));
#define LAUNCH(TWV, KCV)                                                                             \
  return launch_lists(h, s, &k_permute_lists<list_lpg(TWV), list_nw(TWV), KCV>, "k_permute_lists",  \
                      (size_t)list_tile_dwords(N, TWV) * sizeof(uint32_t), TWV, d_tiles, d_lidx,     \
                      entries, d_lstart, d_lngroups, d_lorder, d_lflipped, d_crit, d_lcrit, d_margins, \
                      sc, G, T, N, P, d_r, accumulate, d_panels, d_bfrag, k_split, routed_entries,       \
                      (int)((k_split + kWave / list_lpg(TWV) - 1) / (kWave / list_lpg(TWV))))
  if (TW == 16) LAUNCH(16, 11);
  if (TW == 8) LAUNCH(8, 12);
  if (TW == 4) LAUNCH(4, 13);
  LAUNCH(2, 14);
#undef LAUNCH
}

}
```

### scoary_amd/csrc/scoary_mfma.hip

```cpp
#include "scoary_common.hpp"

const double kMfmaNsPerGene = 58.0;
const double kListNsPerEntry = 0.18;
const double kMfmaBlockStartStages = 6.0;
const double kMfmaTraitSwitchStages = 2.0;

namespace {

typedef int v8i __attribute__((ext_vector_type(8)));
typedef int v4i __attribute__((ext_vector_type(4)));
typedef float v16f __attribute__((ext_vector_type(16)));

constexpr int kKSteps = 32;
constexpr int kBlockGenes = 256;
constexpr int kBlockWaves = 8;
constexpr int kFragBytes = 1024;
constexpr int kStageBytes = 2 * kKSteps * kFragBytes;
constexpr int kHalfBytes = kStageBytes / 2;
constexpr int kRingSlots = 4;
constexpr int kAhead = kRingSlots - 2;
constexpr int kRingBytes = kRingSlots * kHalfBytes;
constexpr int kDmaPerHalf = kHalfBytes / kBlockWaves / kFragBytes;
constexpr int kThrBytes = 32 * 8;
constexpr int kMfmaLds = kRingBytes + kBlockWaves * kThrBytes;
static_assert(kRingSlots >= 4 && kMfmaLds <= 160 * 1024 && (kAhead - 1) * kDmaPerHalf < 64,
              "a half stage is issued at least two ticks ahead, within the LDS of a CU and the vmcnt field");

__device__ __forceinline__ uint32_t fp4_of_bits8(uint32_t b) {
  uint32_t y = b | (b << 12);
  y = (y | (y << 6)) & 0x03030303u;
  return __builtin_amdgcn_perm(0u, 0x22200200u, y);
}
__device__ __forceinline__ v4i fp4_of_bits32(uint32_t w) {
  return v4i{(int)fp4_of_bits8(w & 0xffu), (int)fp4_of_bits8((w >> 8) & 0xffu),
             (int)fp4_of_bits8((w >> 16) & 0xffu), (int)fp4_of_bits8(w >> 24)};
}

__global__ __launch_bounds__(256) void k_mfma_panels(const uint32_t* __restrict__ tiled, int64_t Gp, int G, int N,
                                                     const int32_t* __restrict__ order,
                                                     const uint8_t* __restrict__ flipped, int64_t total,
                                                     v4i* __restrict__ panels) {
  const int64_t idx = (int64_t)blockIdx.x * 256 + threadIdx.x;
  if (idx >= total) return;
  const int lane = (int)(idx & 63);
  const int64_t f = idx >> 6;
  const int k = (int)(f & 31), i = (int)((f >> 5) & 1);
  const int64_t slot = (f >> 6) * 64 + i * 32 + (lane & 31);
  const int w = 2 * k + (lane >> 5);
  uint32_t bits = 0u;
  if (slot < G && 32 * w < N) {
    const int g = order[slot];
    bits = tiled[((int64_t)(w >> 2) * Gp + g) * 4 + (w & 3)];
    if (flipped[g]) bits = ~bits;
    if (32 * w + 32 > N) bits &= (1u << (N - 32 * w)) - 1u;
  }
  panels[idx] = fp4_of_bits32(bits);
}

__global__ __launch_bounds__(256) void k_mfma_bfrag(const uint32_t* __restrict__ tiles, int N, int ntiles,
                                                    int64_t tile_dwords, int S, v4i* __restrict__ bfrag) {
  const int s = blockIdx.x, t = blockIdx.y;
  const int lane = threadIdx.x & 63, wave = threadIdx.x >> 6;
  const uint32_t* tile = tiles + ((int64_t)t * ntiles + (s >> 3)) * tile_dwords + 2 * (s & 7);
  v4i* out = bfrag + ((int64_t)t * S + s) * (kStageBytes / 16);
  for (int k = wave; k < kKSteps; k += 4) {
    const int row = k * 64 + lane;
    uint2 w = make_uint2(0u, 0u);
    if (row < N) w = *reinterpret_cast<const uint2*>(tile + (int64_t)row * 16);
#pragma unroll
    for (int j = 0; j < 2; ++j) {
      const uint32_t x = j ? w.y : w.x;
      uint32_t mine = 0u;
#pragma unroll
      for (int c = 0; c < 32; ++c) {
        const uint64_t bal = __ballot((x >> c) & 1u);
        const uint32_t v = (lane >> 5) ? (uint32_t)(bal >> 32) : (uint32_t)bal;
        if ((lane & 31) == c) mine = v;
      }
      out[(k * 2 + j) * 64 + lane] = fp4_of_bits32(mine);
    }
  }
}

__device__ __forceinline__ void mfma_dma16(uint32_t lds, uint32_t lane_off, const unsigned char* src) {
  uint32_t m0_saved;
  asm volatile("s_mov_b32 %0, m0\n\ts_mov_b32 m0, %1\n\ts_nop 0\n\t"
               "global_load_lds_dwordx4 %2, %3\n\ts_mov_b32 m0, %0"
               : "=&s"(m0_saved)
               : "s"(lds), "v"(lane_off), "s"(src)
               : "memory");
}

__device__ __forceinline__ void mfma_dma4(uint32_t lds, uint32_t lane_off, const unsigned char* src) {
  uint32_t m0_saved;
  asm volatile("s_mov_b32 %0, m0\n\ts_mov_b32 m0, %1\n\ts_nop 0\n\t"
               "global_load_lds_dword %2, %3\n\ts_mov_b32 m0, %0"
               : "=&s"(m0_saved)
               : "s"(lds), "v"(lane_off), "s"(src)
               : "memory");
}

__device__ __forceinline__ int xcd_item(int orig, int n) {
  const int q = n >> 3, r = n & 7, x = orig & 7;
  return (x < r ? x * (q + 1) : r * (q + 1) + (x - r) * q) + (orig >> 3);
}

__global__ __launch_bounds__(kBlockWaves * 64) __attribute__((amdgpu_waves_per_eu(2, 2)))
void k_permute_mfma(const v4i* __restrict__ panels, const unsigned char* __restrict__ bfrag,
                    const uint2* __restrict__ lcrit, int G, int64_t P, int S, int64_t Q, int L, int nblk_genes,
                    int ntiles, int64_t gs, uint16_t* __restrict__ partial) {
  extern __shared__ __attribute__((aligned(16))) unsigned char lds[];
  const int item = xcd_item(blockIdx.x, gridDim.x);
  const int gb = item % nblk_genes, rng = item / nblk_genes;
  const int64_t q0 = (int64_t)rng * L;
  const int ns = (int)min((int64_t)L, Q - q0);
  int t = (int)(q0 / S), s = (int)(q0 % S);
  int jt = rng - (int)((int64_t)t * S / L);
  const int tid = threadIdx.x, lane = tid & 63, half = lane >> 5, l31 = lane & 31;
  const int wave = __builtin_amdgcn_readfirstlane(tid >> 6);
  const bool late = wave >= kBlockWaves / 2;
  const int wslot0 = gb * kBlockGenes + wave * 32;
  const int rows_mine = min(32, G - wslot0) - 4 * half;
  v16f negc;
  float hw[16];
  const uint32_t lds0 = (uint32_t)(uintptr_t)(const __attribute__((address_space(3))) unsigned char*)lds;
  const uint32_t lane_off = (uint32_t)lane * 16u;
  const int thr_slot0 = min(wslot0, G - 1);
  const uint32_t thr_lds = kRingBytes + (uint32_t)wave * kThrBytes;
  auto fetch_thresholds = [&](int tt) {
    uint32_t l = lane_off;
    asm volatile("" : "+v"(l));
    l >>= 4;
    const uint32_t off = (uint32_t)min((int)(l >> 1), G - 1 - thr_slot0) * 8u + (l & 1u) * 4u;
    mfma_dma4(lds0 + thr_lds, off, reinterpret_cast<const unsigned char*>(lcrit + ((int64_t)tt * G + thr_slot0)));
  };
  auto take_thresholds = [&]() {
    int h4 = 4 * half, mine = rows_mine;
    asm volatile("" : "+v"(h4), "+v"(mine));
    const uint2* thr = reinterpret_cast<const uint2*>(lds + thr_lds) + h4;
#pragma unroll
    for (int r = 0; r < 16; ++r) {
      const int row = (r & 3) + 8 * (r >> 2);
      const uint2 cr = thr[row];
      negc[r] = -0.5f * (float)((int)cr.x + (int)cr.y - 1);
      hw[r] = row < mine ? 0.5f * (float)((int)cr.y - 1 - (int)cr.x) : 1e30f;
    }
    asm volatile("" : "+v"(negc));
#pragma unroll
    for (int r = 0; r < 16; ++r) asm volatile("" : "+v"(hw[r]));
  };
  v4i a[kKSteps];
  {
    fetch_thresholds(t);
    const v4i* ap = panels + ((int64_t)gb * kBlockWaves + wave) * (kKSteps * 64) + lane;
#pragma unroll
    for (int k = 0; k < kKSteps; ++k) a[k] = ap[k * 64];
#pragma unroll
    for (int k = 0; k < kKSteps; ++k) asm volatile("" : "+v"(a[k]));
    asm volatile("s_waitcnt vmcnt(0)" ::: "memory");
    take_thresholds();
  }

  const unsigned char* bsrc = bfrag + q0 * kStageBytes + wave * (kHalfBytes / kBlockWaves);
  const int nh = 2 * ns;
  auto issue_half = [&](int n) {
    const unsigned char* src = bsrc + (int64_t)min(n, nh - 1) * kHalfBytes;
    const uint32_t dst = lds0 + (uint32_t)(n % kRingSlots) * kHalfBytes + (uint32_t)wave * (kHalfBytes / kBlockWaves);
#pragma unroll
    for (int p = 0; p < kDmaPerHalf; ++p) mfma_dma16(dst + p * kFragBytes, lane_off, src + p * kFragBytes);
  };
#pragma unroll
  for (int n = 0; n < kAhead; ++n) issue_half(n);
  int tick = 0;
  auto next_tick = [&]() {
    asm volatile("s_waitcnt vmcnt(%0)" ::"n"((kAhead - 1) * kDmaPerHalf) : "memory");
    __builtin_amdgcn_s_barrier();
    issue_half(tick + kAhead);
    ++tick;
  };

  uint32_t ex[16];
#pragma unroll
  for (int r = 0; r < 16; ++r) ex[r] = 0u;
  const int ragged = (int)(P - (int64_t)(S - 1) * 64);

  v16f acc[2];
  auto region_test = [&](int nvalid) {
    if (nvalid < 64) {
      const bool v0 = l31 < nvalid, v1 = l31 + 32 < nvalid;
#pragma unroll
      for (int r = 0; r < 16; ++r) {
        acc[0][r] = v0 ? acc[0][r] : __builtin_nanf("");
        acc[1][r] = v1 ? acc[1][r] : __builtin_nanf("");
      }
    }
#pragma unroll
    for (int r = 0; r < 16; ++r)
      ex[r] += (uint32_t)(__builtin_fabsf(acc[0][r]) > hw[r]) + (uint32_t)(__builtin_fabsf(acc[1][r]) > hw[r]);
  };
  const int jt0 = jt;
  auto end_segment = [&](int tt) {
    uint16_t* out = partial + ((int64_t)tt * ntiles + jt) * gs + wslot0;
    int rl = l31, h4 = 4 * half, mine = rows_mine;
    asm volatile("" : "+v"(rl), "+v"(h4), "+v"(mine));
    uint32_t count = 0u;
#pragma unroll
    for (int r = 0; r < 16; ++r) {
      uint32_t v = ex[r];
#pragma unroll
      for (int off = 16; off > 0; off >>= 1) v += __shfl_xor(v, off);
      ex[r] = 0u;
      count = rl == r ? v : count;
    }
    const int row = (rl & 3) + 8 * (rl >> 2);
    if (rl < 16 && row < mine) out[h4 + row] = (uint16_t)count;
    jt = 0;
  };
  if (late) next_tick();
  int rslot = 0;
  for (int st = 0; st < ns; ++st) {
#pragma unroll
    for (int h = 0; h < 2; ++h) {
      next_tick();
      const unsigned char* bbuf = lds + rslot * kHalfBytes + lane * 16;
      rslot = rslot == kRingSlots - 1 ? 0 : rslot + 1;
      v4i bq[3][2];
      auto read_b = [&](int kk) {
#pragma unroll
        for (int j = 0; j < 2; ++j)
          bq[kk % 3][j] = *reinterpret_cast<const v4i*>(bbuf + (kk * 2 + j) * kFragBytes);
      };
      read_b(0);
      read_b(1);
      if (h == 0) {
        __builtin_amdgcn_sched_barrier(0);
        if (st > 0) {
          const bool entered = s == 0;
          region_test(entered ? ragged : 64);
          if (entered) {
            end_segment(t - 1);
            take_thresholds();
          }
        }
        if (s == S - 1 && st + 1 < ns) fetch_thresholds(t + 1);
        __builtin_amdgcn_sched_barrier(0);
      }
#pragma unroll
      for (int kk = 0; kk < kKSteps / 2; ++kk) {
        const int k = h * (kKSteps / 2) + kk;
        if (kk + 2 < kKSteps / 2) read_b(kk + 2);
        __builtin_amdgcn_sched_barrier(0);
        const v8i aa = v8i{a[k].x, a[k].y, a[k].z, a[k].w, 0, 0, 0, 0};
#pragma unroll
        for (int j = 0; j < 2; ++j) {
          const v4i x = bq[kk % 3][j];
          acc[j] = __builtin_amdgcn_mfma_scale_f32_32x32x64_f8f6f4(aa, v8i{x.x, x.y, x.z, x.w, 0, 0, 0, 0},
                                                                   k == 0 ? negc : acc[j], 4, 4, 0, 0x7f7f7f7f, 0,
                                                                   0x7f7f7f7f);
        }
        __builtin_amdgcn_sched_barrier(0);
      }
    }
    if (++s == S) s = 0, ++t;
  }
  if (!late) next_tick();
  const bool trait_done = s == 0;
  region_test(trait_done ? ragged : 64);
  asm volatile("s_waitcnt vmcnt(0)" ::: "memory");
  end_segment(trait_done ? t - 1 : t);

  {
    int rl = l31, h4 = 4 * half, mine = rows_mine;
    asm volatile("" : "+v"(rl), "+v"(h4), "+v"(mine));
    const int row = (rl & 3) + 8 * (rl >> 2);
    const bool stores = rl < 16 && row < mine;
    const int t0 = (int)(q0 / S);
    for (int tt = t0; tt < t; ++tt) {
      uint16_t* out = partial + (int64_t)tt * ntiles * gs + wslot0 + h4 + row;
      for (int tile = (tt == t0 ? jt0 : 0) + 1; tile < ntiles; ++tile)
        if (stores) out[(int64_t)tile * gs] = 0;
    }
  }
}

}

struct MfmaRange {
  int64_t L, ranges, switches;
};
static std::vector<MfmaRange> mfma_ranges(int64_t T, int64_t P, int64_t ntiles) {
  std::vector<MfmaRange> out;
  const int64_t S = (P + 63) / 64, Q = T * S;
  for (int64_t L = std::min<int64_t>(Q, 1023); L >= 1; --L) {
    const int64_t ranges = (Q + L - 1) / L;
    if ((Q + ranges - 1) / ranges != L) continue;
    bool ok = true;
    for (int64_t t = 0; t < std::min(T, L) && ok; ++t) ok = ((t + 1) * S - 1) / L - t * S / L + 1 <= ntiles;
    if (!ok) continue;
    MfmaRange c{L, ranges, 0};
    for (int64_t r = 0; r < std::min(ranges, S); ++r)
      c.switches = std::max(c.switches, (std::min(Q, (r + 1) * L) - 1) / S - r * L / S);
    out.push_back(c);
  }
  return out;
}

static MfmaGeom mfma_pick(const std::vector<MfmaRange>& cands, int num_cu, int64_t gene_blocks, int64_t S,
                          int64_t T) {
  MfmaGeom g{};
  g.stages = S;
  g.Q = T * S;
  g.gene_blocks = gene_blocks;
  for (const MfmaRange& c : cands) {
    const int64_t blocks = gene_blocks * c.ranges;
    const double cost = (double)((blocks + num_cu - 1) / num_cu) *
                        ((double)c.L + kMfmaBlockStartStages + (double)c.switches * kMfmaTraitSwitchStages);
    if (g.L == 0 || cost < g.cost) g.cost = cost, g.ranges = c.ranges, g.L = c.L, g.blocks = blocks;
  }
  return g;
}

MfmaGeom scoary_mfma_geom(int num_cu, int64_t k_split, int64_t T, int64_t P, int64_t ntiles) {
  return mfma_pick(mfma_ranges(T, P, ntiles), num_cu, (k_split + kBlockGenes - 1) / kBlockGenes, (P + 63) / 64, T);
}

int scoary_mfma_launch(scoary_handle h, hipStream_t s, const uint32_t* d_tiles, const void* d_panels, void* d_bfrag,
                       const uint32_t* d_lcrit, uint16_t* d_partial, int64_t k_split, int64_t G, int64_t T,
                       int64_t N, int64_t P, int64_t ntiles, int64_t gs) {
  const MfmaGeom g = scoary_mfma_geom(h->num_cu, k_split, T, P, ntiles);
  if (g.blocks > 0x7fffffffLL || g.stages > 0x7fffffffLL / 64)
    return fail(h, SCOARY_ERR_SIZE, "scoary_permute_hybrid: grid too large");
  if (!h->mfma_lds_optin) {
    HIP_TRY(h, hipFuncSetAttribute(reinterpret_cast<const void*>(&k_permute_mfma),
                                   hipFuncAttributeMaxDynamicSharedMemorySize, 160 * 1024));
    h->mfma_lds_optin = 1;
  }
  {
    KernelTimer kt(h, s, "k_mfma_bfrag");
    hipLaunchKernelGGL(k_mfma_bfrag, dim3((unsigned)g.stages, (unsigned)T), dim3(256), 0, s, d_tiles, (int)N,
                       (int)ntiles, list_tile_dwords(N, 16), (int)g.stages, static_cast<v4i*>(d_bfrag));
  }
  {
    KernelTimer kt(h, s, "k_permute_mfma");
    hipLaunchKernelGGL(k_permute_mfma, dim3((unsigned)g.blocks), dim3(kBlockWaves * 64), kMfmaLds, s,
                       static_cast<const v4i*>(d_panels), static_cast<const unsigned char*>(d_bfrag),
                       reinterpret_cast<const uint2*>(d_lcrit), (int)G, P, (int)g.stages, g.Q, (int)g.L,
                       (int)g.gene_blocks, (int)ntiles, gs, d_partial);
  }
  HIP_TRY(h, hipGetLastError());
  return SCOARY_OK;
}

extern "C" {

int64_t scoary_mfma_max_isolates(void) { return kKSteps * 64; }
int64_t scoary_mfma_panels_bytes(int64_t G, int64_t N) {
  if (G < 1 || N < 1 || N > kKSteps * 64) return 0;
  return round_up(G, kBlockGenes) * (2 * kKSteps * 16);
}
int64_t scoary_mfma_bfrag_bytes(int64_t N, int64_t P, int64_t T) {
  if (N < 1 || N > kKSteps * 64 || P < 1 || T < 1) return 0;
  return T * ((P + 63) / 64) * kStageBytes;
}
int64_t scoary_mfma_breakeven_entries(void) { return (int64_t)std::ceil(kMfmaNsPerGene / kListNsPerEntry); }

int scoary_mfma_panels_build(scoary_handle h, const uint32_t* d_tiled, int64_t G, int64_t N, const int32_t* d_order,
                             const uint8_t* d_flipped, void* d_panels, scoary_stream_t stream) {
  if (!h) return SCOARY_ERR_ARG;
  if (!d_tiled || !d_order || !d_flipped || !d_panels || G < 1 || N < 1)
    return fail(h, SCOARY_ERR_ARG, "scoary_mfma_panels_build: bad argument");
  if (N > kKSteps * 64 || G > 0x7fffffffLL - kBlockGenes)
    return fail(h, SCOARY_ERR_SIZE, "scoary_mfma_panels_build: N > 2048 or G >= 2^31");
  DeviceGuard guard(h->device);
  hipStream_t s = static_cast<hipStream_t>(stream);
  const int64_t total = scoary_mfma_panels_bytes(G, N) / 16;
  KernelTimer kt(h, s, "k_mfma_panels");
  hipLaunchKernelGGL(k_mfma_panels, dim3((unsigned)((total + 255) / 256)), dim3(256), 0, s, d_tiled,
                     scoary_tiled_genes(G), (int)G, (int)N, d_order, d_flipped, total, static_cast<v4i*>(d_panels));
  HIP_TRY(h, hipGetLastError());
  return SCOARY_OK;
}

int scoary_mfma_plan(int num_cu, int64_t k_split, int64_t T, int64_t P, int64_t* out) {
  if (num_cu < 1 || k_split < 1 || T < 1 || P < 1 || !out) return SCOARY_ERR_ARG;
  const MfmaGeom g = scoary_mfma_geom(num_cu, k_split, T, P, (P + 511) / 512);
  out[0] = g.gene_blocks, out[1] = g.ranges, out[2] = g.L, out[3] = g.blocks;
  return SCOARY_OK;
}

int scoary_set_mfma_route(scoary_handle h, int mode) {
  if (!h) return SCOARY_ERR_ARG;
  if (mode < SCOARY_MFMA_ROUTE_NONE || mode > SCOARY_MFMA_ROUTE_AUTO)
    return fail(h, SCOARY_ERR_ARG, "scoary_set_mfma_route: mode is 0 (none), 1 (all) or 2 (auto)");
  h->mfma_route = mode;
  return SCOARY_OK;
}

int64_t scoary_mfma_route(scoary_handle h, const int64_t* block_start, int64_t G, int64_t T, int64_t N, int64_t P) {
  if (!h || G < 1 || T < 1 || P < 1 || N < 1 || N > kKSteps * 64 || h->mfma_route == SCOARY_MFMA_ROUTE_NONE)
    return 0;
  if (h->mfma_route == SCOARY_MFMA_ROUTE_ALL) return G;
  if (!block_start) return 0;
  const int64_t nb = G / kBlockGenes, total = block_start[(G + kBlockGenes - 1) / kBlockGenes];
  const double tests = (double)T * (double)P / 1e5;
  const double stage_ns = kMfmaNsPerGene * h->num_cu * kBlockGenes * 64 / 1e5;
  double best = kListNsPerEntry * (double)total * tests;
  int64_t best_nb = 0;
  const std::vector<MfmaRange> cands = mfma_ranges(T, P, (P + 511) / 512);
  for (int64_t b = 1; b <= nb; ++b) {
    const MfmaGeom g = mfma_pick(cands, h->num_cu, b, (P + 63) / 64, T);
    if (g.blocks < h->num_cu) continue;
    const double cost = g.cost * stage_ns + kListNsPerEntry * (double)(total - block_start[b]) * tests;
    if (cost < best) best = cost, best_nb = b;
  }
  return best_nb * kBlockGenes;
}

}
```

### scoary_amd/engine.py

```python
import ctypes

import numpy as np

from . import _abi


def _torch():
    import torch
    return torch


def pack_bits_rows(dense01):
    dense01 = np.ascontiguousarray(dense01, dtype=np.uint8)
    R, N = dense01.shape
    W = (N + 63) // 64
    by = np.packbits(dense01, axis=1, bitorder="little")
    out = np.zeros((R, W * 8), dtype=np.uint8)
    out[:, :by.shape[1]] = by
    return out.view("<u8")


class GeneMatrix:

    def __init__(self, tiled, G, N):
# ... 13 lines not shown
            self.minp_caches.pop("fisher", None)
        else:
            self.minp_caches["fisher"] = slot


class ListMemoryError(_abi.ScoaryHipError):
    """The index lists of a gene matrix would not fit the memory budget (build_lists): the
    caller falls back to the dense permutation kernels, which need no lists."""


class GeneLists:

    def __init__(self, idx, start, ngroups, order, flipped, entries):
        self.idx, self.start, self.ngroups = idx, start, ngroups
        self.order, self.flipped, self.entries = order, flipped, entries
        self.panels, self.block_start, self.routes = None, None, {}


class MinpTables:

    def __init__(self, off, lo, tab, entries):
        self.off, self.lo, self.tab, self.entries = off, lo, tab, int(entries)


class TableSource:

    def __init__(self, kind, key, build, observed):
        self.kind, self.key, self.build, self.observed = kind, key, build, observed


class TraitPlan:

    def __init__(self, margins, mask_class, buf, traits, masks, N):
        self.margins, self.mask_class, self.buf, self.N = margins, mask_class, buf, int(N)
        self.traits, self.masks = traits, masks
        self.versions = (traits._version, masks._version)

    def fits(self, traits, masks):
        return (traits is self.traits and masks is self.masks
                and self.versions == (traits._version, masks._version))


class StrataPlan:

    def __init__(self, strata, members, offsets, smargins, S, N, sizes, checked=False):
        self.strata, self.members, self.offsets, self.smargins = strata, members, offsets, smargins
        self.S, self.N, self.T, self.sizes = int(S), int(N), int(smargins.shape[0]), sizes
        if not checked:
            off = offsets.cpu().numpy().astype(np.int64)
            mem = members.cpu().numpy().astype(np.int64)
            if off.shape != (self.S + 1,) or off[0] != 0 or off[-1] != self.N or (np.diff(off) < 0).any():
                raise ValueError("StrataPlan: the stratum offsets must rise from 0 to N = %d in S + 1 = %d entries"
                                 % (self.N, self.S + 1))
            if mem.shape != (self.N,) or not np.array_equal(np.sort(mem), np.arange(self.N)):
                raise ValueError("StrataPlan: members must hold every isolate 0 .. N - 1 exactly once")

    def rows(self, t0, t1):
        if t0 == 0 and t1 == self.T:
            return self
        return StrataPlan(self.strata, self.members, self.offsets, self.smargins[t0:t1], self.S, self.N, self.sizes,
                          checked=True)


class Workspace:

    def __init__(self, eng, genes, T, permutations, use_lists, perm_buffer=None):
        torch = _torch()
        G, N = genes.G, genes.N
        self.key = (G, N, int(T), int(permutations), bool(use_lists and permutations > 0))
        self.eng = eng
        self.counts = eng._empty((T, G, 4), torch.int32)
        self.margins = eng._empty((T, 2), torch.int32)
        self.mask_class = eng._empty((T,), torch.int32)
        self.plan_buf = eng._empty((int(eng.lib.scoary_trait_plan_bytes(int(T), N)) // 4,), torch.int32)
        self.p = eng._empty((T, G), torch.float64)
        self.odds = eng._empty((T, G), torch.float64)
        self.crit = eng._empty((T, G, 2), torch.int32) if permutations > 0 else None
        self.r = eng._empty((T, G), torch.int32) if permutations > 0 else None
        self.tiles = self.scratch = self.perms = self.lcrit = self.bfrag = None
        self.label_shards = None
        self.auto = None
        self.batch = 0
        if permutations > 0 and use_lists:
            self.batch = eng.list_batch(T, N, permutations, G)
            nb0 = min(self.batch, permutations)
            words = int(eng.lib.scoary_list_tiles_words(N, nb0, T))
            if eng.label_shards is not None:
                words = max(words, eng.label_shards.padded_words(*eng.tiles_per_batch(N, nb0, T)))
            self.tiles = eng._empty((words,), torch.int32)
            self.label_shards = eng.label_shards
            self.scratch = eng.permute_lists_scratch(G, T, N, nb0)
            self.lcrit = eng._empty((T, G, 2), torch.int32)
            if genes.lists is not None and genes.lists.panels is not None:
                self.bfrag = eng._empty((int(eng.lib.scoary_mfma_bfrag_bytes(N, nb0, T)) // 4,), torch.int32)
        elif permutations > 0:
            if perm_buffer is not None:
                self.perms = perm_buffer
            else:
                self.perms = eng._empty((T, eng.perm_batch(T, N, permutations), eng.row_words(N)),
                                        torch.int32)

    def fits(self, genes, T, permutations, use_lists):
        if self.tiles is not None and self.label_shards is not self.eng.label_shards:
            return False
        return self.key == (genes.G, genes.N, int(T), int(permutations),
                            bool(use_lists and permutations > 0))


class StepGraph:

    def __init__(self, eng, graph, stream):
        self.eng, self.graph, self.stream = eng, graph, stream
        self.done = None

    def launch(self):
        eng = self.eng
        eng._check(eng.lib.scoary_graph_launch(eng.h, self.graph, eng._stream()),
                   "scoary_graph_launch")
        if self.done is None:
            self.done = _torch().cuda.Event()
        self.done.record(_torch().cuda.current_stream(eng.device))

    def close(self):
        if self.graph:
            if self.done is not None:
                self.done.synchronize()
            self.eng.lib.scoary_graph_destroy(self.graph)
            self.graph = None

    def __del__(self):
        try:
            self.close()
        except Exception:
            pass


class AssociationEngine:
    def __init__(self, device=None):
        torch = _torch()
        if not torch.cuda.is_available():
            raise _abi.ScoaryHipError(
                "no GPU visible: scoary_amd runs on MI355X (gfx950) only and has no CPU path")
        self.lib = _abi.load()
        if device is None:
            device = torch.cuda.current_device()
        self.device = torch.device("cuda", int(device) if not isinstance(device, torch.device)
                                   else device.index or 0)
        h = ctypes.c_void_p()
        rc = self.lib.scoary_create(self.device.index, ctypes.byref(h))
        if rc != 0:
            raise _abi.ScoaryHipError("scoary_create(device=%d) failed: %d" % (self.device.index, rc))
        self.h = h
        self.label_shards = None

    def close(self):
        if getattr(self, "h", None):
            self.lib.scoary_destroy(self.h)
            self.h = None

    def __del__(self):
        try:
            self.close()
        except Exception:
            pass

    def _side_stream(self):
        if getattr(self, "_side", None) is None:
            self._side = _torch().cuda.Stream(device=self.device)
        return self._side

    def _stream(self):
        return ctypes.c_void_p(_torch().cuda.current_stream(self.device).cuda_stream)

    def _check(self, rc, what):
        if rc != 0:
            msg = self.lib.scoary_last_error(self.h)
            raise _abi.ScoaryHipError("%s failed (%d): %s" % (what, rc, (msg or b"").decode()))

    @staticmethod
    def _ptr(t):
        return ctypes.c_void_p(t.data_ptr())

    def quads(self, N):
        return int(self.lib.scoary_tiled_quads(int(N)))

    def row_words(self, N):
        return int(self.lib.scoary_row_words(int(N)))

    def padded_genes(self, G):
        return int(self.lib.scoary_tiled_genes(int(G)))

    def _empty(self, shape, dtype):
        return _torch().empty(shape, dtype=dtype, device=self.device)

    def pack_dense(self, dense):
        torch = _torch()
        if isinstance(dense, np.ndarray):
            dense = torch.from_numpy(np.ascontiguousarray(dense, dtype=np.uint8))
        dense = dense.to(self.device, dtype=torch.uint8).contiguous()
        G, N = dense.shape
        tiled = self._empty((self.quads(N), self.padded_genes(G), 4), torch.int32)
        self._check(self.lib.scoary_pack_dense(self.h, self._ptr(dense), G, N, self._ptr(tiled),
                                               self._stream()), "scoary_pack_dense")
        return GeneMatrix(tiled, G, N)

    def tile_rows(self, rows64, N):
        torch = _torch()
        if isinstance(rows64, np.ndarray):
            rows64 = torch.from_numpy(np.ascontiguousarray(rows64).view(np.int64))
        rows64 = rows64.to(self.device).contiguous()
        G, W = rows64.shape
        if W != (N + 63) // 64:
            raise ValueError("rows64 has %d words per row, N=%d needs %d" % (W, N, (N + 63) // 64))
        tiled = self._empty((self.quads(N), self.padded_genes(G), 4), torch.int32)
        self._check(self.lib.scoary_tile_rows(self.h, self._ptr(rows64), G, N, self._ptr(tiled),
                                              self._stream()), "scoary_tile_rows")
        return GeneMatrix(tiled, G, N)

    def vecrows(self, rows64, N):
        torch = _torch()
        rows64 = np.ascontiguousarray(rows64, dtype=np.uint64)
        R, W = rows64.shape
        Wp = self.row_words(N)
        buf = np.zeros((R, Wp), dtype=np.uint32)
        buf[:, :2 * W] = rows64.view(np.uint32).reshape(R, 2 * W)
        return torch.from_numpy(buf.view(np.int32)).to(self.device)

    def list_budget_bytes(self):
        import os
        mb = os.environ.get("SCOARY_LIST_BUDGET_MB")
        if mb:
            return int(float(mb) * (1 << 20))
        torch = _torch()
        free, _total = torch.cuda.mem_get_info(self.device)
        cached = torch.cuda.memory_reserved(self.device) - torch.cuda.memory_allocated(self.device)
        return int((free + max(cached, 0)) * 0.6)

    def list_kernel_name(self, N):
        return "k_permute_seglists" if int(self.lib.scoary_list_segments(int(N))) > 1 else "k_permute_lists"

    def build_lists(self, genes, budget_bytes=None):
        torch = _torch()
        lanes, _stride, _gpw, _classes, _piece = self.list_params(genes.N)
        if not lanes:
            raise ValueError("N=%d is too large for the list-driven kernel" % genes.N)
        G, N = genes.G, genes.N
        scratch = self._empty((int(self.lib.scoary_lists_scratch_bytes(G, N)) // 8 + 1,),
                              torch.int64)
        nseg = max(1, int(self.lib.scoary_list_segments(N)))
        shape = (G,) if nseg == 1 else (nseg, G)
        start = self._empty(shape, torch.int32)
        ngroups = self._empty(shape, torch.int32)
        order = self._empty((G,), torch.int32)
        flipped = self._empty((G,), torch.uint8)
        entries = ctypes.c_int64()
        self._check(self.lib.scoary_lists_plan(
            self.h, self._ptr(genes.tiled), G, N, self._ptr(scratch), self._ptr(start),
            self._ptr(ngroups), self._ptr(order), self._ptr(flipped), ctypes.byref(entries),
            self._stream()), "scoary_lists_plan")
        total = int(entries.value)
        need = 4 * (total + int(self.lib.scoary_lists_slack_entries()))
        if budget_bytes is None:
            budget_bytes = self.list_budget_bytes()
        if need > budget_bytes:
            raise ListMemoryError("index lists of a %d x %d matrix need %.1f MB, budget %.1f MB"
                                  % (G, N, need / 2**20, budget_bytes / 2**20))
        idx = self._empty((total + int(self.lib.scoary_lists_slack_entries()),), torch.int32)
        self._check(self.lib.scoary_lists_fill(
            self.h, self._ptr(genes.tiled), G, N, self._ptr(scratch), self._ptr(order),
            self._ptr(flipped), total, self._ptr(idx), self._stream()), "scoary_lists_fill")
        genes.lists = GeneLists(idx, start, ngroups, order, flipped, total)
        self._build_panels(genes, budget_bytes - need)
        return genes.lists

    def _build_panels(self, genes, budget_bytes):
        torch = _torch()
        L, G, N = genes.lists, genes.G, genes.N
        nbytes = int(self.lib.scoary_mfma_panels_bytes(G, N))
        if nbytes == 0 or nbytes > budget_bytes:
            return
        panels = self._empty((nbytes // 4,), torch.int32)
        self._check(self.lib.scoary_mfma_panels_build(
            self.h, self._ptr(genes.tiled), G, N, self._ptr(L.order), self._ptr(L.flipped),
            self._ptr(panels), self._stream()), "scoary_mfma_panels_build")
        starts = L.start[::256].to(torch.int64).cpu().numpy() * 32
        L.block_start = np.ascontiguousarray(np.append(starts, np.int64(L.entries)), dtype=np.int64)
        L.panels = panels

    def mfma_split(self, genes, T, P):
        L = genes.lists
        if L is None or L.panels is None:
            return 0
        key = (getattr(self, "_mfma_mode", "auto"), int(T), int(P))
        k = L.routes.get(key)
        if k is None:
            k = L.routes[key] = int(self.lib.scoary_mfma_route(
                self.h, ctypes.c_void_p(L.block_start.ctypes.data), genes.G, int(T), genes.N, int(P)))
        return k

    def set_mfma_route(self, mode):
        self._check(self.lib.scoary_set_mfma_route(self.h, {"none": 0, "all": 1, "auto": 2}[mode]),
                    "scoary_set_mfma_route")
        self._mfma_mode = mode

    def list_params(self, N):
        out = (ctypes.c_int64 * 5)()
        self.lib.scoary_list_params(int(N), out)
        return tuple(int(x) for x in out)

    def lists_supported(self, N):
        return int(N) <= int(self.lib.scoary_list_max_isolates())

    def perm_generate_tiles(self, masks, margins, N, P, perm_base, seed, out=None, trait_base=0,
                            tile_range=None, strata=None):
        torch = _torch()
        T = masks.shape[0]
        if out is None:
            out = self._empty((int(self.lib.scoary_list_tiles_words(N, P, T)),), torch.int32)
        if strata is not None:
            self._strata_fits(strata, T, N)
            if tile_range is None:
                tile_range = (0, self.tiles_per_batch(N, P, T)[0])
            self._check(self.lib.scoary_perm_generate_tiles_strata_range(
                self.h, self._ptr(masks), *self._strata_ptrs(strata), T, N, strata.S, P, perm_base, trait_base,
                ctypes.c_uint64(seed), int(tile_range[0]), int(tile_range[1]), self._ptr(out), self._stream()),
                "scoary_perm_generate_tiles_strata_range")
        elif tile_range is None:
            self._check(self.lib.scoary_perm_generate_tiles(
                self.h, self._ptr(masks), self._ptr(margins), T, N, P, perm_base, trait_base,
                ctypes.c_uint64(seed), self._ptr(out), self._stream()), "scoary_perm_generate_tiles")
        else:
            self._check(self.lib.scoary_perm_generate_tiles_range(
                self.h, self._ptr(masks), self._ptr(margins), T, N, P, perm_base, trait_base,
                ctypes.c_uint64(seed), int(tile_range[0]), int(tile_range[1]), self._ptr(out),
                self._stream()), "scoary_perm_generate_tiles_range")
        return out

    def tiles_per_batch(self, N, P, T):
        tw = self.list_params(N)[0]
        return int(T) * (-(-int(P) // (32 * tw))), int(self.lib.scoary_list_tile_words(int(N)))

    def permute_lists_scratch(self, G, T, N, P):
        torch = _torch()
        nbytes = int(self.lib.scoary_permute_lists_scratch_bytes(G, T, N, P))
        return self._empty(((nbytes + 3) // 4,), torch.int32)

    def permute_lists(self, genes, tiles, crit, margins, P, r, scratch=None, lcrit=None,
                      accumulate=True, bfrag=None):
        L = genes.lists
        T = (lcrit if lcrit is not None else crit).shape[0]
        if scratch is None:
            scratch = self.permute_lists_scratch(genes.G, T, genes.N, P)
        routed = 0
        k_split = self.mfma_split(genes, T, P)
        if k_split > 0:
            if bfrag is None:
                bfrag = self._empty((int(self.lib.scoary_mfma_bfrag_bytes(genes.N, P, T)) // 4,), _torch().int32)
            routed = int(L.block_start[-1 if k_split >= genes.G else k_split // 256])
        self._check(self.lib.scoary_permute_hybrid(
            self.h, self._ptr(tiles), self._ptr(L.idx), L.entries, self._ptr(L.start),
            self._ptr(L.ngroups), self._ptr(L.order), self._ptr(L.flipped),
            self._ptr(crit) if lcrit is None else None,
            self._ptr(lcrit) if lcrit is not None else None,
            self._ptr(margins), self._ptr(scratch), genes.G, T, genes.N, P, self._ptr(r),
            1 if accumulate else 0, self._ptr(L.panels) if k_split > 0 else None,
            self._ptr(bfrag) if k_split > 0 else None, k_split, routed, self._stream()),
            "scoary_permute_hybrid")
        return r

    def trait_plan(self, traits, masks, N, out=None):
        torch = _torch()
        T = traits.shape[0]
        margins, mask_class, buf = out if out is not None else (
            self._empty((T, 2), torch.int32), self._empty((T,), torch.int32),
            self._empty((int(self.lib.scoary_trait_plan_bytes(int(T), int(N))) // 4,), torch.int32))
        self._check(self.lib.scoary_trait_plan(self.h, self._ptr(traits), self._ptr(masks), T, int(N),
                                               self._ptr(margins), self._ptr(mask_class), self._ptr(buf),
                                               self._stream()), "scoary_trait_plan")
        return TraitPlan(margins, mask_class, buf, traits, masks, N)

    def counts(self, genes, traits, masks, out=None, plan=None):
        torch = _torch()
        T = traits.shape[0]
        counts = out[0] if out is not None else self._empty((T, genes.G, 4), torch.int32)
        if plan is None:
            plan = self.trait_plan(traits, masks, genes.N,
                                   out=None if out is None or len(out) < 4 else tuple(out[1:4]))
        elif not plan.fits(traits, masks) or plan.N != genes.N:
            raise ValueError("the trait plan was built from other trait / mask tensors")
        self._check(self.lib.scoary_counts_planned(
            self.h, self._ptr(genes.tiled), self._ptr(plan.buf), self._ptr(plan.margins),
            genes.G, T, genes.N, self._ptr(counts), self._stream()), "scoary_counts_planned")
        return counts, plan.margins

    def fisher(self, tables, want_crit=True, out=None, lists=None, lcrit=None):
        torch = _torch()
        tables = tables.contiguous()
        shape = tables.shape[:-1]
        M = int(np.prod(shape)) if len(shape) else 1
        if out is not None:
            p, odds, crit = out
        else:
            p = self._empty(shape, torch.float64)
            odds = self._empty(shape, torch.float64)
            crit = self._empty(tuple(shape) + (2,), torch.int32) if want_crit else None
        if lists is not None:
            if len(shape) != 2:
                raise ValueError("fisher(lists=...) wants tables shaped [T, G, 4]")
            if lcrit is None:
                lcrit = self._empty(tuple(shape) + (2,), torch.int32)
            self._check(self.lib.scoary_fisher_lists(
                self.h, self._ptr(tables), shape[0], shape[1], self._ptr(lists.order),
                self._ptr(lists.flipped), self._ptr(p), self._ptr(odds),
                self._ptr(crit) if crit is not None else None, self._ptr(lcrit),
                self._stream()), "scoary_fisher_lists")
            return p, odds, crit, lcrit
        self._check(self.lib.scoary_fisher(self.h, self._ptr(tables), M, self._ptr(p),
                                           self._ptr(odds),
                                           self._ptr(crit) if crit is not None else None,
                                           self._stream()), "scoary_fisher")
        return p, odds, crit

    def fisher_scipy(self, tables, p):
        torch = _torch()
        tables = tables.contiguous()
        if not p.is_contiguous() or p.dtype != torch.float64 or tuple(p.shape) != tuple(tables.shape[:-1]):
            raise ValueError("fisher_scipy: p must be a contiguous float64 tensor shaped like the tables")
        M = int(np.prod(tables.shape[:-1])) if len(tables.shape) > 1 else 1
        skipped = torch.zeros(1, dtype=torch.int64, device=self.device)
        self._check(self.lib.scoary_fisher_scipy(self.h, self._ptr(tables), M, self._ptr(p), self._ptr(skipped),
                                                 self._stream()), "scoary_fisher_scipy")
        return int(skipped.item())

    def fisher_scipy_max_isolates(self):
        return int(self.lib.scoary_fisher_scipy_max_isolates())

    def strata_max(self):
        return int(self.lib.scoary_perm_max_strata()), int(self.lib.scoary_perm_strata_max_isolates())

    def strata_plan(self, strata_host, trait_rows, mask_rows, N, S=None):
        torch = _torch()
        N = int(N)
        st = np.asarray(strata_host)
        if st.ndim != 1 or st.shape[0] != N or N < 1 or not np.issubdtype(st.dtype, np.integer):
            raise ValueError("strata_plan: strata must be %d integers, one per isolate" % N)
        st = st.astype(np.int64)
        S = int(st.max()) + 1 if S is None else int(S)
        max_s, max_n = self.strata_max()
        if st.min() < 0 or st.max() >= S:
            raise ValueError("strata_plan: stratum indices must lie in [0, S)")
        if S > max_s:
            raise ValueError("strata_plan: %d strata, the generator takes %d (scoary_perm_max_strata)" % (S, max_s))
        if N > max_n:
            raise ValueError("strata_plan: %d isolates, the stratified generator takes %d "
                             "(scoary_perm_strata_max_isolates)" % (N, max_n))
        sizes = np.bincount(st, minlength=S)
        members = np.argsort(st, kind="stable").astype(np.int32)
        offsets = np.concatenate(([0], np.cumsum(sizes))).astype(np.int32)
        T = int(trait_rows.shape[0])
        dev = [torch.from_numpy(x).to(self.device) for x in
               (st.astype(np.uint16).view(np.int16), members, offsets)]
        smargins = self._empty((T, S, 2), torch.int32)
        self._check(self.lib.scoary_strata_margins(self.h, self._ptr(trait_rows), self._ptr(mask_rows),
                                                   self._ptr(dev[0]), T, N, S, self._ptr(smargins),
                                                   self._stream()), "scoary_strata_margins")
        return StrataPlan(dev[0], dev[1], dev[2], smargins, S, N, sizes)

    @staticmethod
    def _strata_fits(strata, T, N):
        if strata.T != int(T) or strata.N != int(N) or not strata.smargins.is_contiguous():
            raise ValueError("the strata plan was built for other traits (%d traits, %d isolates)"
                             % (strata.T, strata.N))

    def _strata_ptrs(self, strata):
        return tuple(self._ptr(x) for x in (strata.strata, strata.members, strata.offsets, strata.smargins))

    def _cmh_scratch(self, N):
        return self._empty(((int(self.lib.scoary_cmh_scratch_bytes(N)) + 7) // 8,), _torch().int64)

    def cmh(self, genes, traits, masks, strata, scounts=False):
        torch = _torch()
        T, G, N = int(traits.shape[0]), genes.G, genes.N
        self._strata_fits(strata, T, N)
        if int(masks.shape[0]) != T or not (traits.is_contiguous() and masks.is_contiguous()):
            raise ValueError("cmh: label and validity rows must be contiguous [T, Wp] tensors of the same traits")
        out = {k: self._empty((T, G), torch.float64) for k in ("stat", "p", "odds", "e2", "var")}
        out["a"] = self._empty((T, G), torch.int32)
        out["crit"] = self._empty((T, G, 2), torch.int32)
        if scounts:
            out["scounts"] = self._empty((T, G, strata.S, 2), torch.int32)
        scratch = self._cmh_scratch(N)
        self._check(self.lib.scoary_cmh(
            self.h, self._ptr(genes.tiled), self._ptr(traits), self._ptr(masks), *self._strata_ptrs(strata),
            G, T, N, strata.S, *(self._ptr(out[k]) for k in ("stat", "p", "odds", "e2", "var", "a", "crit")),
            self._ptr(out["scounts"]) if scounts else None, self._ptr(scratch), self._stream()), "scoary_cmh")
        return out

    def cmh_homogeneity(self, genes, traits, masks, strata, cmh_res):
        torch = _torch()
        T, G, N = int(traits.shape[0]), genes.G, genes.N
        self._strata_fits(strata, T, N)
        if int(masks.shape[0]) != T or not (traits.is_contiguous() and masks.is_contiguous()):
            raise ValueError("cmh_homogeneity: label and validity rows must be contiguous [T, Wp] tensors of the "
                             "same traits")
        odds = cmh_res["odds"]
        if not odds.is_contiguous() or tuple(odds.shape) != (T, G) or odds.dtype != torch.float64:
            raise ValueError("cmh_homogeneity: cmh()'s odds [T, G] of the same traits, contiguous")
        out = {k: self._empty((T, G), torch.float64) for k in ("stat_bd", "stat_tarone", "p")}
        out["df"] = self._empty((T, G), torch.int32)
        scratch = self._cmh_scratch(N)
        self._check(self.lib.scoary_cmh_homogeneity(
            self.h, self._ptr(genes.tiled), self._ptr(traits), self._ptr(masks), *self._strata_ptrs(strata),
            G, T, N, strata.S, self._ptr(odds), *(self._ptr(out[k]) for k in ("stat_bd", "stat_tarone", "df", "p")),
            self._ptr(scratch), self._stream()), "scoary_cmh_homogeneity")
        return out

    def perm_generate(self, masks, margins, N, P, perm_base, seed, out=None, trait_base=0, strata=None):
        torch = _torch()
        T = masks.shape[0]
        Wp = self.row_words(N)
# ... 236 lines not shown
            tables = cached["tables"] if cached else source.build(t0, t1)
            if plan is not None and cached is None and len(groups) == 1:
                genes.minp_caches[source.kind] = {"plan": plan, "budget": table_budget_bytes, "groups": groups,
                                                  "tables": tables, "key": source.key}
            if begin is not None:
                begin(t0, t1, source.observed(t0, t1, tables))
            batch = self.perm_batch(Tg, N, p1 - p0, budget_bytes=label_budget_bytes)
            if buf is None or buf.numel() < Tg * batch * Wp:
                buf = self._empty((Tg * batch * Wp,), torch.int32)
            done = p0
            while done < p1:
                nb = min(batch, p1 - done)
                perms = buf[:Tg * nb * Wp].view(Tg, nb, Wp)
                self.perm_generate(masks[t0:t1], margins[t0:t1], N, nb, done, seed, out=perms, trait_base=t0,
                                   strata=strata.rows(t0, t1) if strata is not None else None)
                launch(t0, t1, tables, perms, nb, done)
                done += nb
            del tables

    @staticmethod
    def r_fwer(minp, p):
        torch = _torch()
        srt = torch.sort(minp, dim=1).values.contiguous()
        return torch.searchsorted(srt, p.contiguous(), right=True).to(torch.int32)

    def westfall_young(self, genes, traits, masks, permutations, seed, res, fwer=False, stepdown=False,
                       table_budget_bytes=8 << 30, plan=None, strata=None, reduce=None, cmh_fwer=False,
                       cmh_stepdown=False, label_budget_bytes=8 << 30):
        kw = dict(res=res, table_budget_bytes=table_budget_bytes, label_budget_bytes=label_budget_bytes, plan=plan,
                  strata=strata)
        out = {}
        if fwer or stepdown or not (cmh_fwer or cmh_stepdown):
            if stepdown:
                out["r_fwer_sd"], minp = self.minp_stepdown(genes, traits, masks, permutations, seed, **kw)
            else:
                minp = self.minp(genes, traits, masks, permutations, seed, **kw)
            out["minp"] = minp if reduce is None else reduce(minp)
            if fwer:
                out["r_fwer"] = self.r_fwer(out["minp"], res["p"])
        if cmh_fwer or cmh_stepdown:
            if strata is None or "cmh_e2" not in res:
                raise ValueError("cmh_fwer / cmh_stepdown need the result of a step with cmh=True and its strata")
            source = self.cmh_source(genes, masks, strata, self._cmh_of(res))
            u_obs = self._empty(tuple(res["cmh_a"].shape), _torch().float64)
            if cmh_stepdown:
                out["r_cmh_fwer_sd"], out["minu"] = self.minp_stepdown(genes, traits, masks, permutations, seed,
                                                                       source=source, observed_out=u_obs, **kw)
            else:
                out["minu"] = self.minp(genes, traits, masks, permutations, seed, source=source,
                                        observed_out=u_obs, **kw)
            out["u_obs"] = u_obs
            if cmh_fwer:
                out["r_cmh_fwer"] = self.r_fwer(out["minu"], u_obs)
        return out

    def stepdown_chunks(self, G, T, P):
        return int(self.lib.scoary_stepdown_chunks(self.h, int(G), int(T), int(P)))

    def permute_stepdown(self, genes, perms, tables, order, p_sorted, c, minp=None, P=None, perm_base=0):
        torch = _torch()
        T = int(perms.shape[0])
        if P is None:
            P = int(perms.shape[1])
        G = genes.G
        if not (perms.is_contiguous() and order.is_contiguous() and p_sorted.is_contiguous() and c.is_contiguous()):
            raise ValueError("permute_stepdown: label rows, order, p_sorted and c must be contiguous")
        if tuple(order.shape) != (T, G) or tuple(p_sorted.shape) != (T, G) or tuple(c.shape) != (T, G) or \
                order.dtype != torch.int32 or p_sorted.dtype != torch.float64 or c.dtype != torch.int32:
            raise ValueError("permute_stepdown: order int32, p_sorted float64 and c int32 must be [T, G]")
        stride = 0
        if minp is not None:
            if minp.stride(1) != 1 or (T > 1 and minp.stride(0) != minp.shape[1]):
                raise ValueError("permute_stepdown: minp rows must be contiguous")
            stride = int(minp.shape[1])
        need = int(self.lib.scoary_stepdown_scratch_bytes(self.h, G, T, genes.N, int(P)))
        scratch = self._empty(((need + 7) // 8,), torch.int64)
        self._check(self.lib.scoary_permute_stepdown(
            self.h, self._ptr(genes.tiled), self._ptr(perms), self._ptr(tables.off), self._ptr(tables.lo),
            self._ptr(tables.tab), self._ptr(order), self._ptr(p_sorted), G, T, genes.N, int(P), int(perm_base),
            stride, self._ptr(minp) if minp is not None else None, self._ptr(c), self._ptr(scratch),
            self._stream()), "scoary_permute_stepdown")
        return c

    def minp_stepdown(self, genes, traits, masks, permutations, seed=0, res=None, table_budget_bytes=8 << 30,
                      label_budget_bytes=8 << 30, plan=None, strata=None, source=None, observed_out=None):
        torch = _torch()
        counts, margins = self._minp_inputs(genes, traits, masks, res, plan)
        if source is None:
            source = self.fisher_source(counts, res["p"] if res is not None else None)
        T, G, P = int(counts.shape[0]), genes.G, int(permutations)
        ps = self._empty((T, G), torch.float64)
        order32 = self._empty((T, G), torch.int32)
        c = torch.zeros((T, G), dtype=torch.int32, device=self.device)
        minp = torch.ones((T, P), dtype=torch.float64, device=self.device)

        keep = self._keep_observed(observed_out)

        def begin(t0, t1, observed):
            ps[t0:t1], order32[t0:t1] = torch.sort(observed.contiguous(), dim=1, stable=True)
            if keep is not None:
                keep(t0, t1, observed)

        def launch(t0, t1, tables, perms, nb, done):
            self.permute_stepdown(genes, perms, tables, order32[t0:t1], ps[t0:t1], c[t0:t1], minp=minp[t0:t1], P=nb,
                                  perm_base=done)
        self._minp_batches(genes, masks, counts, margins, 0, P, seed, table_budget_bytes, label_budget_bytes, plan,
                           launch, source, strata=strata, begin=begin)
        pos = torch.arange(G, device=self.device).expand(T, G)
        first = torch.ones((T, G), dtype=torch.bool, device=self.device)
        first[:, 1:] = ps[:, 1:] != ps[:, :-1]
        head = torch.cummax(torch.where(first, pos, torch.zeros_like(pos)), dim=1).values
        r_rank = torch.cummax(c.gather(1, head), dim=1).values
        r_sd = torch.empty_like(c)
        r_sd.scatter_(1, order32.to(torch.int64), r_rank)
        return r_sd, minp

    def perm_batch(self, T, N, P, budget_bytes=8 << 30):
        per = T * self.row_words(N) * 4
        return int(max(1, min(P, budget_bytes // max(per, 1))))

    def list_batch(self, T, N, permutations, G=0, budget_bytes=8 << 30, scratch_bytes=4 << 30):
        per = max(int(self.lib.scoary_list_tiles_words(N, 512, T)) * 4, 1)
        batch = (budget_bytes // per) * 512
        if G > 0:
            tile_perms = 32 * self.list_params(N)[0]
            per_tile = 2 * int(T) * (int(G) + 64)
            batch = min(batch, max(1, scratch_bytes // per_tile) * tile_perms // 512 * 512)
        return int(max(512, min(-(-permutations // 512) * 512, batch)))

    def workspace(self, genes, T, permutations=0, use_lists=None, perm_buffer=None):
        return Workspace(self, genes, T, permutations, self._lists_default(genes, use_lists), perm_buffer)

    def _lists_default(self, genes, use_lists):
        return (genes.lists is not None and self.lists_supported(genes.N)) if use_lists is None else use_lists

    AUTO_GRAPH_MAX_TESTS = 5e8

    def auto_graph_eligible(self, genes, T, permutations):
        import os
        if os.environ.get("SCOARY_AUTO_GRAPH", "1") == "0":
            return False
        return float(genes.G) * int(T) * max(int(permutations), 1) <= self.AUTO_GRAPH_MAX_TESTS

    def _auto_graph(self, genes, traits, masks, permutations, seed, use_lists, ws, plan, strata=None):
        torch = _torch()
        if getattr(self, "_timing", False) or torch.cuda.is_current_stream_capturing():
            return None
        L = genes.lists
        refs = (genes.tiled, traits, masks, plan, plan.margins, plan.mask_class, plan.buf) + \
            ((L.idx, L.start, L.ngroups, L.order, L.flipped) if L is not None else ()) + \
            ((L.panels,) if L is not None and L.panels is not None else ()) + \
            ((strata, strata.strata, strata.members, strata.offsets, strata.smargins) if strata is not None else ())
        scalars = (genes.G, genes.N, int(traits.shape[0]), int(permutations), int(seed), bool(use_lists),
                   getattr(self, "_mfma_mode", "auto"), strata is not None,
                   tuple(getattr(x, "_version", 0) for x in refs))
        st = ws.auto
        same = st is not None and st["scalars"] == scalars and len(st["refs"]) == len(refs) and \
            all(a is b for a, b in zip(st["refs"], refs))
        if not same:
            if st is not None and st["graph"] is not None:
                st["graph"].close()
            ws.auto = {"refs": refs, "scalars": scalars, "graph": None, "res": None}
            return None
        if st["graph"] is None:
            st["graph"], st["res"] = self.capture(genes, traits, masks, permutations, seed, ws,
                                                  use_lists=use_lists, plan=plan, strata=strata)
            torch.cuda.current_stream(self.device).wait_stream(st["graph"].stream)
            return st["res"]
        st["graph"].launch()
        return st["res"]

    def _label_tiles(self, ws, masks, margins, N, nb, base, seed, strata=None):
        sh = ws.label_shards
        if sh is None or sh.world == 1:
            self.perm_generate_tiles(masks, margins, N, nb, base, seed, out=ws.tiles, strata=strata)
            return
        nflat, tile_words = self.tiles_per_batch(N, nb, masks.shape[0])
        _per, first, count = sh.share(nflat)
        self.perm_generate_tiles(masks, margins, N, nb, base, seed, out=ws.tiles,
                                 tile_range=(first, count), strata=strata)
        sh.all_gather(ws.tiles, nflat, tile_words)

    def associate(self, genes, traits, masks, permutations=0, seed=0, perm_buffer=None,
                  use_lists=None, workspace=None, plan=None, graph=None, records=None, fwer=False,
                  table_budget_bytes=8 << 30, stepdown=False, strata=None, cmh=False, cmh_fwer=False,
                  cmh_stepdown=False, cmh_exact=False, cmh_exact_odds=False, cmh_exact_level=0.95,
                  cmh_homogeneity=False):
        if (fwer or stepdown) and permutations <= 0:
            raise ValueError("fwer=True / stepdown=True need permutations > 0")
        if (cmh_fwer or cmh_stepdown) and (permutations <= 0 or not cmh):
            raise ValueError("cmh_fwer=True / cmh_stepdown=True need cmh=True and permutations > 0")
        if cmh_exact and not cmh:
            raise ValueError("cmh_exact=True needs cmh=True (and its strata)")
        if cmh_exact_odds and not cmh:
            raise ValueError("cmh_exact_odds=True needs cmh=True (and its strata)")
        if cmh_exact_odds and not 0.0 < float(cmh_exact_level) < 1.0:
            raise ValueError("cmh_exact_level must lie inside (0, 1), not %r" % (cmh_exact_level,))
        if cmh_homogeneity and not cmh:
            raise ValueError("cmh_homogeneity=True needs cmh=True (and its strata)")
        if cmh and strata is None:
            raise ValueError("cmh=True needs strata (a StrataPlan of these traits)")
        if strata is not None and (permutations > 0 or cmh):
            self._strata_fits(strata, traits.shape[0], genes.N)
        elif permutations <= 0:
            strata = None
        res = self._associate(genes, traits, masks, permutations, seed, perm_buffer, use_lists,
                              workspace, plan, graph if records is None and not (fwer or stepdown or cmh) else False,
                              strata=strata, cmh=cmh)
        if fwer or stepdown or cmh_fwer or cmh_stepdown:
            res = {**res, **self.westfall_young(genes, traits, masks, permutations, seed, res, fwer, stepdown,
                                                table_budget_bytes, plan, strata, cmh_fwer=cmh_fwer,
                                                cmh_stepdown=cmh_stepdown)}
        if cmh_exact:
            exact = self.cmh_exact(genes, masks, strata, self._cmh_of(res))
            res = {**res, "cmh_exact_p": exact["p"], "cmh_exact_region_p": exact["p_region"]}
        if cmh_exact_odds:
            odds = self.cmh_exact_odds(genes, masks, strata, self._cmh_of(res), level=cmh_exact_level)
            res = {**res, "cmh_exact_odds": odds["odds"], "cmh_exact_odds_lower": odds["lower"],
                   "cmh_exact_odds_upper": odds["upper"]}
        if cmh_homogeneity:
            homog = self.cmh_homogeneity(genes, traits, masks, strata, self._cmh_of(res))
            res = {**res, "cmh_homog_p": homog["p"], "cmh_homog_stat": homog["stat_tarone"],
                   "cmh_homog_df": homog["df"]}
        if records is not None:
            res = dict(res)
            res["records"] = self.pack_records(res, out=records)
        return res

    def _associate(self, genes, traits, masks, permutations, seed, perm_buffer, use_lists, workspace,
                   plan, graph, strata=None, cmh=False):
        torch = _torch()
        T = traits.shape[0]
        use_lists = self._lists_default(genes, use_lists)
        if use_lists and permutations > 0 and genes.lists is None:
            raise ValueError("use_lists=True but the gene matrix has no index lists: call "
                             "build_lists(genes) once per data set first")
        ws = workspace
        if ws is None:
            ws = Workspace(self, genes, T, permutations, use_lists, perm_buffer)
        elif not ws.fits(genes, T, permutations, use_lists):
            raise ValueError("workspace was made for another problem shape")
        if graph is None and workspace is not None and plan is not None and perm_buffer is None \
                and ws.label_shards is None and self.auto_graph_eligible(genes, T, permutations):
            res = self._auto_graph(genes, traits, masks, permutations, seed, use_lists, ws, plan, strata)
            if res is not None:
                return res
        counts, margins = self.counts(genes, traits, masks,
                                      out=(ws.counts, ws.margins, ws.mask_class, ws.plan_buf), plan=plan)
        lists = permutations > 0 and use_lists
        if lists:
            main = torch.cuda.current_stream(self.device)
            side = self._side_stream()
            side.wait_stream(main)
            with torch.cuda.stream(side):
                self._label_tiles(ws, masks, margins, genes.N, min(ws.batch, permutations), 0, seed, strata)
            p, odds, crit, lcrit = self.fisher(counts, out=(ws.p, ws.odds, ws.crit),
                                               lists=genes.lists, lcrit=ws.lcrit)
        else:
            p, odds, crit = self.fisher(counts, out=(ws.p, ws.odds, ws.crit))
        extra = self._cmh_results(genes, traits, masks, strata, permutations) if cmh else {}
        counted = [({"crit": None, "lcrit": lcrit} if lists else {"crit": crit}, ws.r)]
        if "r_cmh" in extra:
            counted.append(({"crit": extra["cmh_crit"]}, extra["r_cmh"]))
        done = 0
        if lists:
            main.wait_stream(side)
            while done < permutations:
                nb = min(ws.batch, permutations - done)
                if done > 0:
                    self._label_tiles(ws, masks, margins, genes.N, nb, done, seed, strata)
                for regions, r in counted:
                    self.permute_lists(genes, ws.tiles, margins=margins, P=nb, r=r, scratch=ws.scratch,
                                       accumulate=done > 0, bfrag=ws.bfrag, **regions)
                done += nb
        elif permutations > 0:
            ws.r.zero_()
            batch = ws.perms.shape[1]
            while done < permutations:
                nb = min(batch, permutations - done)
                self.perm_generate(masks, margins, genes.N, nb, done, seed, out=ws.perms, strata=strata)
                for regions, r in counted:
                    self.permute(genes, ws.perms[:, :nb] if nb == batch else ws.perms, r=r, P=nb, **regions)
                done += nb
        return {"counts": counts, "margins": margins, "p": p, "odds": odds, "crit": crit, "r": ws.r, **extra}

    def _cmh_results(self, genes, traits, masks, strata, permutations):
        torch = _torch()
        c = self.cmh(genes, traits, masks, strata)
        out = {"cmh_" + k: c[k] for k in self.CMH_RESULT}
        if permutations > 0:
            out["r_cmh"] = torch.zeros((traits.shape[0], genes.G), dtype=torch.int32, device=self.device)
        return out

    CMH_RESULT = ("stat", "p", "odds", "crit", "e2", "var", "a")

    @classmethod
    def _cmh_of(cls, res):
        return {k: res["cmh_" + k] for k in cls.CMH_RESULT}

    def capture(self, genes, traits, masks, permutations, seed, workspace, use_lists=None, plan=None,
                records=None, strata=None):
        torch = _torch()
        if torch.cuda.is_current_stream_capturing():
            raise _abi.ScoaryHipError("capture(): the current stream is already capturing")
        if workspace.label_shards is not None and workspace.label_shards.world > 1:
            raise _abi.ScoaryHipError("capture(): label shards are active -- their all-gather is a collective "
                                      "and cannot be recorded into a hipGraph")
        self.associate(genes, traits, masks, permutations=permutations, seed=seed,
                       use_lists=use_lists, workspace=workspace, plan=plan, graph=False, records=records,
                       strata=strata)
        torch.cuda.synchronize(self.device)
        stream = torch.cuda.Stream(device=self.device)
        with torch.cuda.stream(stream):
            self._check(self.lib.scoary_graph_begin(self.h, self._stream()), "scoary_graph_begin")
            failed = True
            try:
                res = self.associate(genes, traits, masks, permutations=permutations, seed=seed,
                                     use_lists=use_lists, workspace=workspace, plan=plan, graph=False,
                                     records=records, strata=strata)
                failed = False
            finally:
                g = ctypes.c_void_p()
                rc = self.lib.scoary_graph_end(self.h, self._stream(), ctypes.byref(g))
                if (failed or rc != 0) and g.value:
                    self.lib.scoary_graph_destroy(g)
                    g = ctypes.c_void_p()
            self._check(rc, "scoary_graph_end")
        return StepGraph(self, g, stream), res

    def pack_records(self, res, nstop=None, out=None):
        torch = _torch()
        T, G = res["p"].shape
        if out is None:
            out = self._empty((T, G, 10), torch.int32)
        r = res.get("r")
        self._check(self.lib.scoary_pack_records(
            self.h, self._ptr(res["counts"]), self._ptr(res["p"]), self._ptr(res["odds"]),
            self._ptr(r) if r is not None else None,
            self._ptr(nstop) if nstop is not None else None, T * G, self._ptr(out),
            self._stream()), "scoary_pack_records")
        return out

    def row_hash(self, genes, masks):
        torch = _torch()
        T = masks.shape[0]
        out = self._empty((T, genes.G, 2), torch.int64)
        self._check(self.lib.scoary_row_hash(self.h, self._ptr(genes.tiled), self._ptr(masks),
                                             genes.G, T, genes.N, self._ptr(out), self._stream()),
                    "scoary_row_hash")
        return out.cpu().numpy().view(np.uint64)

    def upgma_merges(self, rows01):
        torch = _torch()
        R, N = rows01.shape
        counts = self.hamming(rows01, device=True)
        scratch = self._empty(((int(self.lib.scoary_upgma_scratch_bytes(R)) + 7) // 8,), torch.int64)
        merges = self._empty((max(R - 1, 1), 2), torch.int32)
        status = self._empty((1,), torch.int32)
        self._check(self.lib.scoary_upgma(self.h, self._ptr(counts), R, N, self._ptr(scratch),
                                          self._ptr(merges), self._ptr(status), self._stream()),
                    "scoary_upgma")
        if int(status.cpu()[0]) != 0:
            return None
        return merges.cpu().numpy()[:R - 1]

    def hamming(self, rows01, device=False):
        torch = _torch()
        rows01 = np.ascontiguousarray(rows01, dtype=np.uint8)
        R, N = rows01.shape
        bits = pack_bits_rows(rows01)
        gm = self.tile_rows(bits, N)
        vec = self.vecrows(bits, N)
        out = self._empty((R, R), torch.int32)
        self._check(self.lib.scoary_hamming(self.h, self._ptr(gm.tiled), self._ptr(vec), R, N,
                                            self._ptr(out), self._stream()), "scoary_hamming")
        return out if device else out.cpu().numpy()

    def gather_bits(self, rows, index):
        torch = _torch()
        rows = rows.contiguous()
        R, Wsrc = rows.shape
        K = int(index.shape[0])
        out = self._empty((R, (K + 31) // 32), torch.int32)
        self._check(self.lib.scoary_gather_bits(self.h, self._ptr(rows), R, Wsrc,
                                                self._ptr(index), K, self._ptr(out),
                                                self._stream()), "scoary_gather_bits")
        return out

    def tree_pairs(self, ops, depth, gene_bits, label_bits, K):
        torch = _torch()
        G, L = gene_bits.shape[0], label_bits.shape[0]
        out = self._empty((G, L, 3), torch.int32)
        self._check(self.lib.scoary_tree_pairs(self.h, self._ptr(ops), int(ops.shape[0]),
                                               int(depth), self._ptr(gene_bits),
                                               self._ptr(label_bits), G, L, int(K),
                                               self._ptr(out), self._stream()),
                    "scoary_tree_pairs")
        return out

    def tree_permute(self, ops, depth, gene_bits, label_bits, K, obs):
        torch = _torch()
        G, L = gene_bits.shape[0], label_bits.shape[0]
        out = self._empty((G, L), torch.uint8)
        self._check(self.lib.scoary_tree_permute(self.h, self._ptr(ops), int(ops.shape[0]),
                                                 int(depth), self._ptr(gene_bits),
                                                 self._ptr(label_bits), G, L, int(K),
                                                 self._ptr(obs.contiguous()), self._ptr(out),
                                                 self._stream()), "scoary_tree_permute")
        return out

    def set_timing(self, on):
        self._check(self.lib.scoary_set_timing(self.h, 1 if on else 0), "scoary_set_timing")
        self._timing = bool(on)

    def kernel_ms(self, name):
        ms = ctypes.c_double()
        self._check(self.lib.scoary_last_kernel_ms(self.h, name.encode(), ctypes.byref(ms)),
                    "scoary_last_kernel_ms")
        return ms.value
```

Before: 1940 billion tests/s.

## Fuse MFMA B-fragment construction into label-tile generation kernels

```diff
diff --git a/__graft_entry__.py b/__graft_entry__.py
--- a/__graft_entry__.py
+++ b/__graft_entry__.py
@@ -45,8 +45,9 @@
     return out
 
 
-def _rule(name, count, exclude=None, cap=None, no_static_lds=False):
-    return dict(name=name, exclude=exclude, count=count, cap=cap, no_static_lds=no_static_lds)
+def _rule(name, count, exclude=None, cap=None, no_static_lds=False, sgpr_spills=0):
+    return dict(name=name, exclude=exclude, count=count, cap=cap, no_static_lds=no_static_lds,
+                sgpr_spills=sgpr_spills)
 
 
 LIST_RULES = (
@@ -59,6 +60,12 @@
     _rule("k_permute_minp_chunked", 1),
     _rule("k_stepdown_minp", 18, exclude="chunked", cap=(("VGPRs",), 128)),
     _rule("k_stepdown_minp_chunked", 2),
+)
+LABELS_BFRAG_RULES = (
+    _rule("k_labelsILi2ELi2E", 1, cap=(("VGPRs",), 64), sgpr_spills=4),
+    _rule("k_labelsILi1ELi2E", 1, cap=(("VGPRs",), 64), sgpr_spills=4),
+    _rule("k_labels_strataILi2ELi2E", 1, cap=(("VGPRs",), 56)),
+    _rule("k_labels_strataILi1ELi2E", 1, cap=(("VGPRs",), 56)),
 )
 CMH_RULES = (
     _rule("k_cmhE", 1, cap=(("VGPRs",), 128)),
@@ -85,7 +92,7 @@
             bad.append("expected %d %s instance%s, compiler reported %d"
                        % (rule["count"], rule["name"], "" if rule["count"] == 1 else "s", len(hit)))
         for name, r in hit.items():
-            if r.get("ScratchSize", 0) or r.get("VGPRs Spill", 0) or r.get("SGPRs Spill", 0):
+            if r.get("ScratchSize", 0) or r.get("VGPRs Spill", 0) or r.get("SGPRs Spill", 0) > rule.get("sgpr_spills", 0):
                 bad.append("%s: scratch %s, VGPR spills %s, SGPR spills %s" % (
                     name, r.get("ScratchSize"), r.get("VGPRs Spill"), r.get("SGPRs Spill")))
             if rule["cap"]:
@@ -170,8 +177,8 @@
             raise subprocess.CalledProcessError(proc.returncode, cmd)
         res = parse_resource_usage(proc.stderr)
         try:
-            check_kernel_resources(res, RESOURCE_RULES + CMH_RULES + CMH_EXACT_RULES + CMH_EXACT_ODDS_RULES +
-                                   CMH_HOMOG_RULES)
+            check_kernel_resources(res, RESOURCE_RULES + LABELS_BFRAG_RULES + CMH_RULES + CMH_EXACT_RULES +
+                                   CMH_EXACT_ODDS_RULES + CMH_HOMOG_RULES)
             check_ctr_banks()
             for k, (n, same) in check_isa_banks(hipcc).items():
                 res.setdefault(k, {}).update({"v_bitop3_b32": n, "v_bitop3_b32 src0/src1 same bank": same})
diff --git a/include/scoary_hip.h b/include/scoary_hip.h
--- a/include/scoary_hip.h
+++ b/include/scoary_hip.h
@@ -186,6 +186,27 @@
                           int64_t G, int64_t T, int64_t N, int64_t P, uint32_t *d_r,
                           int accumulate, const void *d_panels, void *d_bfrag, int64_t k_split,
                           int64_t routed_entries, scoary_stream_t stream);
+int scoary_perm_generate_tiles_bfrag_range(scoary_handle h, const uint32_t *d_masks,
+                                           const int32_t *d_margins, int64_t T, int64_t N, int64_t P,
+                                           int64_t perm_base, int64_t trait_base, uint64_t seed,
+                                           int64_t first_tile, int64_t n_tiles, uint32_t *d_tiles,
+                                           void *d_bfrag, scoary_stream_t stream);
+int scoary_perm_generate_tiles_strata_bfrag_range(scoary_handle h, const uint32_t *d_masks,
+                                                  const uint16_t *d_strata, const int32_t *d_members,
+                                                  const int32_t *d_offsets, const int32_t *d_smargins,
+                                                  int64_t T, int64_t N, int64_t S, int64_t P,
+                                                  int64_t perm_base, int64_t trait_base, uint64_t seed,
+                                                  int64_t first_tile, int64_t n_tiles,
+                                                  uint32_t *d_tiles, void *d_bfrag,
+                                                  scoary_stream_t stream);
+int scoary_permute_hybrid_bfrag(scoary_handle h, const uint32_t *d_tiles, const uint32_t *d_lidx,
+                                int64_t entries, const int32_t *d_lstart, const int32_t *d_lngroups,
+                                const int32_t *d_lorder, const uint8_t *d_lflipped,
+                                const uint32_t *d_crit, const uint32_t *d_lcrit,
+                                const int32_t *d_margins, void *d_scratch,
+                                int64_t G, int64_t T, int64_t N, int64_t P, uint32_t *d_r,
+                                int accumulate, const void *d_panels, void *d_bfrag, int64_t k_split,
+                                int64_t routed_entries, int bfrag_ready, scoary_stream_t stream);
 
 int64_t scoary_lists_scratch_bytes(int64_t G, int64_t N);
 int64_t scoary_lists_slack_entries(void);
diff --git a/scoary_amd/_abi.py b/scoary_amd/_abi.py
--- a/scoary_amd/_abi.py
+++ b/scoary_amd/_abi.py
@@ -52,12 +52,16 @@
                                           _vp]),
     "scoary_perm_generate_tiles_range": (_i32, [_vp, _vp, _vp, _i64, _i64, _i64, _i64, _i64, _u64, _i64,
                                                 _i64, _vp, _vp]),
+    "scoary_perm_generate_tiles_bfrag_range": (_i32, [_vp, _vp, _vp, _i64, _i64, _i64, _i64, _i64, _u64, _i64,
+                                                      _i64, _vp, _vp, _vp]),
     "scoary_perm_max_isolates": (_i64, []),
     "scoary_perm_max_strata": (_i32, []),
     "scoary_perm_strata_max_isolates": (_i64, []),
     "scoary_strata_margins": (_i32, [_vp, _vp, _vp, _vp, _i64, _i64, _i64, _vp, _vp]),
     "scoary_perm_generate_strata": (_i32, [_vp] * 6 + [_i64] * 6 + [_u64, _vp, _vp]),
     "scoary_perm_generate_tiles_strata_range": (_i32, [_vp] * 6 + [_i64] * 6 + [_u64, _i64, _i64, _vp, _vp]),
+    "scoary_perm_generate_tiles_strata_bfrag_range": (_i32, [_vp] * 6 + [_i64] * 6 + [_u64, _i64, _i64, _vp, _vp,
+                                                                                     _vp]),
     "scoary_cmh_scratch_bytes": (_i64, [_i64]),
     "scoary_cmh": (_i32, [_vp] * 8 + [_i64] * 4 + [_vp] * 10),
     "scoary_cmh_minp_plan": (_i32, [_vp] * 7 + [_i64] * 4 + [_vp] * 3 + [ctypes.POINTER(_i64), _vp]),
@@ -79,6 +83,8 @@
     "scoary_mfma_plan": (_i32, [_i32, _i64, _i64, _i64, ctypes.POINTER(_i64)]),
     "scoary_permute_hybrid": (_i32, [_vp, _vp, _vp, _i64] + [_vp] * 8 + [_i64, _i64, _i64, _i64, _vp,
                                                                         _i32, _vp, _vp, _i64, _i64, _vp]),
+    "scoary_permute_hybrid_bfrag": (_i32, [_vp, _vp, _vp, _i64] + [_vp] * 8 + [_i64, _i64, _i64, _i64, _vp,
+                                                                              _i32, _vp, _vp, _i64, _i64, _i32, _vp]),
     "scoary_lists_scratch_bytes": (_i64, [_i64, _i64]),
     "scoary_lists_slack_entries": (_i64, []),
     "scoary_lists_plan": (_i32, [_vp, _vp, _i64, _i64, _vp, _vp, _vp, _vp, _vp,
diff --git a/scoary_amd/csrc/scoary_common.hpp b/scoary_amd/csrc/scoary_common.hpp
--- a/scoary_amd/csrc/scoary_common.hpp
+++ b/scoary_amd/csrc/scoary_common.hpp
@@ -42,7 +42,7 @@
 MfmaGeom scoary_mfma_geom(int num_cu, int64_t k_split, int64_t T, int64_t P, int64_t ntiles);
 int scoary_mfma_launch(scoary_handle h, hipStream_t s, const uint32_t* d_tiles, const void* d_panels, void* d_bfrag,
                        const uint32_t* d_lcrit, uint16_t* d_partial, int64_t k_split, int64_t G, int64_t T,
-                       int64_t N, int64_t P, int64_t ntiles, int64_t gs);
+                       int64_t N, int64_t P, int64_t ntiles, int64_t gs, bool bfrag_ready);
 
 int scoary_cmh_segments_launch(scoary_handle h, hipStream_t s, const uint16_t* d_strata, const int32_t* d_members,
                                int64_t N, int64_t S, void* d_scratch, const char* event);
@@ -195,6 +195,47 @@
   out[1] = c1;
   out[2] = c2;
   out[3] = c3;
+}
+
+typedef int v4i __attribute__((ext_vector_type(4)));
+constexpr int kKSteps = 32;
+constexpr int kFragBytes = 1024;
+constexpr int kStageBytes = 2 * kKSteps * kFragBytes;
+
+__device__ __forceinline__ uint32_t fp4_of_bits8(uint32_t b) {
+  uint32_t y = b | (b << 12);
+  y = (y | (y << 6)) & 0x03030303u;
+  return __builtin_amdgcn_perm(0u, 0x22200200u, y);
+}
+__device__ __forceinline__ v4i fp4_of_bits32(uint32_t w) {
+  return v4i{(int)fp4_of_bits8(w & 0xffu), (int)fp4_of_bits8((w >> 8) & 0xffu),
+             (int)fp4_of_bits8((w >> 16) & 0xffu), (int)fp4_of_bits8(w >> 24)};
+}
+
+__device__ __forceinline__ uint32_t bit_transpose32(uint32_t x) {
+  const uint32_t lane = threadIdx.x;
+#define SCOARY_TRANSPOSE_STAGE(S, M)                                                                     \
+  {                                                                                                      \
+    const uint32_t p = (uint32_t)__builtin_amdgcn_ds_swizzle((int)x, ((S) << 10) | 0x1f);                \
+    const bool up = lane & (S);                                                                          \
+    const uint32_t r = __builtin_amdgcn_alignbit(p, p, up ? (S) : 32 - (S)), keep = up ? ~(M) : (M);     \
+    x = (x & keep) | (r & ~keep);                                                                        \
+  }
+  SCOARY_TRANSPOSE_STAGE(16, 0x0000ffffu)
+  SCOARY_TRANSPOSE_STAGE(8, 0x00ff00ffu)
+  SCOARY_TRANSPOSE_STAGE(4, 0x0f0f0f0fu)
+  SCOARY_TRANSPOSE_STAGE(2, 0x33333333u)
+  SCOARY_TRANSPOSE_STAGE(1, 0x55555555u)
+#undef SCOARY_TRANSPOSE_STAGE
+  return x;
+}
+
+template <class RowWord>
+__device__ __forceinline__ void mfma_bfrag_emit(v4i* __restrict__ bfrag, int S, int t, int s, int j, int wave,
+                                                int nwaves, RowWord row_word) {
+  const int lane = threadIdx.x & 63;
+  v4i* out = bfrag + ((int64_t)t * S + s) * (kStageBytes / 16) + j * 64 + lane;
+  for (int k = wave; k < kKSteps; k += nwaves) out[k * 128] = fp4_of_bits32(bit_transpose32(row_word(k * 64 + lane)));
 }
 
 struct CmhSegments {
diff --git a/scoary_amd/csrc/scoary_labels.hip b/scoary_amd/csrc/scoary_labels.hip
--- a/scoary_amd/csrc/scoary_labels.hip
+++ b/scoary_amd/csrc/scoary_labels.hip
@@ -65,6 +65,7 @@
   int ntiles, TW;
   int64_t first_flat, nflat;
   uint32_t* out;
+  v4i* bfrag;
 };
 
 template <int NB>
@@ -72,6 +73,7 @@
   int t, bit0;
   uint32_t Bglob;
   uint32_t* tile_base;
+  int stage, jcol;
   uint32_t live[NB];
 };
 template <int NB, int OUT, bool SUB>
@@ -81,7 +83,8 @@
   const int subs = 32 >> elt_log2;
   int64_t lc0 = 0;
   b.tile_base = nullptr;
-  if constexpr (OUT == 0) {
+  b.stage = -1, b.jcol = 0;
+  if constexpr (OUT != 1) {
     const int units = a.TW * subs / NB;
     const int64_t id = blockIdx.x;
     const int64_t qd = id >> 3;
@@ -96,6 +99,10 @@
     lc0 = (int64_t)tile * a.TW + col;
     b.Bglob = (uint32_t)((a.perm_base >> 5) + lc0);
     b.tile_base = a.out + f * list_tile_dwords_seg(a.N, a.TW) + col;
+    if constexpr (OUT == 2) {
+      const int stage = tile * 8 + (col >> 1);
+      if ((int64_t)stage * 64 < a.P) b.stage = stage, b.jcol = col & 1;
+    }
   } else {
     b.t = blockIdx.y;
     b.Bglob = (uint32_t)((a.perm_base >> 5) + blockIdx.x / subs);
@@ -104,7 +111,7 @@
 #pragma unroll
   for (int w = 0; w < NB; ++w) {
     int64_t lo, hi;
-    if constexpr (OUT == 0) {
+    if constexpr (OUT != 1) {
       lo = 0;
       hi = a.P - (lc0 + w) * 32;
     } else {
@@ -262,9 +269,9 @@
 __device__ __forceinline__ void emit_labels(const LabelArgs& a, const LabelBlock<NB>& b, RowField row_field) {
   const int tid = threadIdx.x, lane = tid & 63, tpb = blockDim.x, nwaves = tpb >> 6;
   const int wave = __builtin_amdgcn_readfirstlane(tid >> 6);
-  const int N = a.N, elt = 1 << a.elt_log2, bit0 = b.bit0;
+  const int N = a.N, elt = OUT == 2 ? 32 : 1 << a.elt_log2, bit0 = b.bit0;
   uint32_t* tile_base = b.tile_base;
-  if constexpr (OUT == 0) {
+  if constexpr (OUT != 1) {
     const bool seg = a.TW == kSegTW;
     auto row_off = [&](int64_t row) -> int64_t { return seg ? list_row_dword(N, row) : row * a.TW; };
     if (elt == 32) {
@@ -296,8 +303,16 @@
         else *dst = 0;
       }
     }
+    if constexpr (OUT == 2) {
+      if (b.stage >= 0) {
+#pragma unroll
+        for (int w = 0; w < NB; ++w)
+          mfma_bfrag_emit(a.bfrag, (int)((a.P + 63) >> 6), b.t, b.stage, b.jcol + w, wave, nwaves,
+                          [&](int row) { return row < N ? row_field(row, w) : 0u; });
+      }
+    }
   } else {
-    static_assert(OUT == 0 || NB == 1, "bit rows: one dword column per block");
+    static_assert(OUT != 1 || NB == 1, "bit rows: one dword column per block");
     const int nchunks = (N + 63) >> 6;
     const int64_t pl = (int64_t)b.Bglob * 32 + bit0 + lane - a.perm_base;
     const bool mine = lane < elt && ((b.live[0] >> (bit0 + (lane & 31))) & 1u);
@@ -321,13 +336,30 @@
 }
 
 template <int NB, int OUT>
+__device__ __forceinline__ bool emit_dead_block(const LabelArgs& a, const LabelBlock<NB>& b) {
+  if constexpr (OUT == 2) {
+    uint32_t any = 0u;
+#pragma unroll
+    for (int w = 0; w < NB; ++w) any |= b.live[w];
+    if (any == 0u) {
+      emit_labels<NB, OUT>(a, b, [](int, int) { return 0u; });
+      return true;
+    }
+  }
+  return false;
+}
+
+template <int NB, int OUT>
 __global__ __launch_bounds__(1024) void k_labels(const LabelArgs a) {
   extern __shared__ __attribute__((aligned(16))) uint32_t lds[];
   const int tid = threadIdx.x, lane = tid & 63, tpb = blockDim.x;
   const int N = a.N;
-  const int elt = 1 << a.elt_log2;
+  constexpr bool SUB = OUT != 2;
+  const int elt_log2 = SUB ? a.elt_log2 : 5;
+  const int elt = 1 << elt_log2;
   LabelBlock<NB> blk;
-  if (!label_block<NB, OUT, true>(a, blk)) return;
+  if (!label_block<NB, OUT, SUB>(a, blk)) return;
+  if (emit_dead_block<NB, OUT>(a, blk)) return;
   const int t = blk.t, bit0 = blk.bit0;
   const uint32_t Bglob = blk.Bglob;
   const uint32_t (&live)[NB] = blk.live;
@@ -374,7 +406,7 @@
           carry = nc;
         }
     }
-    store_row0<NB>(xs, row, x, a.elt_log2);
+    store_row0<NB>(xs, row, x, elt_log2);
   }
 #pragma unroll
   for (int w = 0; w < NB; ++w) {
@@ -424,7 +456,7 @@
     if (elt == 32) {
       f = xs[(int64_t)row * NB + w];
     } else {
-      const uint32_t bp = (uint32_t)row << a.elt_log2;
+      const uint32_t bp = (uint32_t)row << elt_log2;
       f = (xs[bp >> 5] >> (bp & 31u)) & fieldmask;
     }
     if (plan.flip) {
@@ -454,6 +486,7 @@
   const int N = a.N, S = sa.S;
   LabelBlock<NB> blk;
   if (!label_block<NB, OUT, false>(a, blk)) return;
+  if (emit_dead_block<NB, OUT>(a, blk)) return;
   const int t = blk.t;
   const uint32_t Bglob = blk.Bglob;
   const uint32_t (&live)[NB] = blk.live;
@@ -589,16 +622,22 @@
 }
 int launch_labels(scoary_handle h, hipStream_t s, const LabelArgs& a, int NB, int OUT, dim3 grid, int tpb) {
   const bool fits = (int64_t)tpb * kMaxRowsPerThread >= a.N;
-  return launch_block(h, s, OUT ? k_labels<1, 1> : (NB == 2 ? k_labels<2, 0> : k_labels<1, 0>),
-                      1 << (NB + 8 * OUT) , labels_lds<int64_t>(a.N, 1 << a.elt_log2, NB).bytes(), fits,
+  return launch_block(h, s,
+                      OUT == 1 ? k_labels<1, 1>
+                               : (OUT == 2 ? (NB == 2 ? k_labels<2, 2> : k_labels<1, 2>)
+                                           : (NB == 2 ? k_labels<2, 0> : k_labels<1, 0>)),
+                      1 << (NB + 4 * OUT) , labels_lds<int64_t>(a.N, 1 << a.elt_log2, NB).bytes(), fits,
                       "k_labels: more than 1023 isolates per thread (or a block size that is no power of two in "
                       "64..1024)", grid, tpb, a);
 }
 int launch_labels_strata(scoary_handle h, hipStream_t s, const LabelArgs& a, const StrataArgs& sa, int NB, int OUT,
                          dim3 grid, int tpb) {
   const int64_t lds_bytes = strata_lds<int64_t>(a.N, NB, sa.S).bytes();
-  return launch_block(h, s, OUT ? k_labels_strata<1, 1> : (NB == 2 ? k_labels_strata<2, 0> : k_labels_strata<1, 0>),
-                      1 << (16 + NB + 8 * OUT), lds_bytes, lds_bytes <= kLabelsMaxLds,
+  return launch_block(h, s,
+                      OUT == 1 ? k_labels_strata<1, 1>
+                               : (OUT == 2 ? (NB == 2 ? k_labels_strata<2, 2> : k_labels_strata<1, 2>)
+                                           : (NB == 2 ? k_labels_strata<2, 0> : k_labels_strata<1, 0>)),
+                      1 << (16 + NB + 4 * OUT), lds_bytes, lds_bytes <= kLabelsMaxLds,
                       "k_labels_strata: rows, members and the stratum table do not fit LDS (or a block size that is "
                       "no power of two in 64..1024)", grid, tpb, a, sa);
 }
@@ -648,8 +687,14 @@
   ts.tpb = labels_threads(n_tiles * units, N, h->num_cu);
   return SCOARY_OK;
 }
-void tile_args(LabelArgs& a, const TileShape& ts, int64_t first_tile, int64_t n_tiles) {
+void tile_args(LabelArgs& a, const TileShape& ts, int64_t first_tile, int64_t n_tiles, void* d_bfrag) {
   a.ntiles = (int)ts.ntiles, a.TW = ts.TW, a.first_flat = first_tile, a.nflat = n_tiles;
+  a.bfrag = static_cast<v4i*>(d_bfrag);
+}
+int check_bfrag_shape(scoary_handle h, const char* what, int64_t N, int elt) {
+  return (N > scoary_mfma_max_isolates() || list_tw(N) != 16 || elt != 32)
+             ? fail(h, SCOARY_ERR_SIZE, std::string(what) + ": more isolates than scoary_mfma_max_isolates()")
+             : SCOARY_OK;
 }
 
 }
@@ -686,19 +731,23 @@
   return launch_labels(h, s, a, 1, 1, dim3((unsigned)gx, (unsigned)T), labels_threads(gx * T, N, h->num_cu));
 }
 
-int scoary_perm_generate_tiles_range(scoary_handle h, const uint32_t* d_masks, const int32_t* d_margins,
-                                     int64_t T, int64_t N, int64_t P, int64_t perm_base,
-                                     int64_t trait_base, uint64_t seed, int64_t first_tile,
-                                     int64_t n_tiles, uint32_t* d_tiles, scoary_stream_t stream) {
-  const char* what = "scoary_perm_generate_tiles";
+extern "C++" {
+static int generate_tiles(scoary_handle h, const uint32_t* d_masks, const int32_t* d_margins, int64_t T, int64_t N,
+                          int64_t P, int64_t perm_base, int64_t trait_base, uint64_t seed, int64_t first_tile,
+                          int64_t n_tiles, uint32_t* d_tiles, bool fragments, void* d_bfrag,
+                          scoary_stream_t stream) {
+  const char* what = fragments ? "scoary_perm_generate_tiles_bfrag_range" : "scoary_perm_generate_tiles";
   if (!h) return SCOARY_ERR_ARG;
   if (int rc = check_args(h, what, d_masks && d_margins && d_tiles && T >= 1 && N >= 1 && P >= 1 && perm_base >= 0 &&
-                                       trait_base >= 0 && first_tile >= 0 && n_tiles >= 0))
+                                       trait_base >= 0 && first_tile >= 0 && n_tiles >= 0 &&
+                                       (d_bfrag || !fragments)))
     return rc;
   if (int rc = check_tile_base(h, what, perm_base)) return rc;
   if (T > 65535 || perm_base + P > 0xffffffffLL)
     return fail(h, SCOARY_ERR_SIZE, "scoary_perm_generate_tiles: T > 65535 or permutation index >= 2^32");
   const int elt = labels_elt(N, 8);
+  if (fragments)
+    if (int rc = check_bfrag_shape(h, what, N, elt)) return rc;
   TileShape ts;
   if (int rc = tile_shape(h, what, T, N, P, first_tile, n_tiles, elt,
                           [&](int nb) { return labels_lds(N, 32, nb); }, ts))
@@ -707,9 +756,27 @@
   DeviceGuard guard(h->device);
   hipStream_t s = static_cast<hipStream_t>(stream);
   LabelArgs a = label_args(d_masks, d_margins, N, P, perm_base, trait_base, seed, elt, d_tiles);
-  tile_args(a, ts, first_tile, n_tiles);
+  tile_args(a, ts, first_tile, n_tiles, d_bfrag);
   KernelTimer kt(h, s, "k_perm_generate_tiles");
-  return launch_labels(h, s, a, ts.NB, 0, dim3((unsigned)ts.gx), ts.tpb);
+  return launch_labels(h, s, a, ts.NB, fragments ? 2 : 0, dim3((unsigned)ts.gx), ts.tpb);
+}
+}
+
+int scoary_perm_generate_tiles_range(scoary_handle h, const uint32_t* d_masks, const int32_t* d_margins,
+                                     int64_t T, int64_t N, int64_t P, int64_t perm_base,
+                                     int64_t trait_base, uint64_t seed, int64_t first_tile,
+                                     int64_t n_tiles, uint32_t* d_tiles, scoary_stream_t stream) {
+  return generate_tiles(h, d_masks, d_margins, T, N, P, perm_base, trait_base, seed, first_tile, n_tiles, d_tiles,
+                        false, nullptr, stream);
+}
+
+int scoary_perm_generate_tiles_bfrag_range(scoary_handle h, const uint32_t* d_masks, const int32_t* d_margins,
+                                           int64_t T, int64_t N, int64_t P, int64_t perm_base,
+                                           int64_t trait_base, uint64_t seed, int64_t first_tile,
+                                           int64_t n_tiles, uint32_t* d_tiles, void* d_bfrag,
+                                           scoary_stream_t stream) {
+  return generate_tiles(h, d_masks, d_margins, T, N, P, perm_base, trait_base, seed, first_tile, n_tiles, d_tiles,
+                        true, d_bfrag, stream);
 }
 
 int scoary_perm_generate_tiles(scoary_handle h, const uint32_t* d_masks, const int32_t* d_margins,
@@ -763,21 +830,24 @@
                               labels_threads(gx * T, N, h->num_cu));
 }
 
-int scoary_perm_generate_tiles_strata_range(scoary_handle h, const uint32_t* d_masks, const uint16_t* d_strata,
-                                            const int32_t* d_members, const int32_t* d_offsets,
-                                            const int32_t* d_smargins, int64_t T, int64_t N, int64_t S, int64_t P,
-                                            int64_t perm_base, int64_t trait_base, uint64_t seed,
-                                            int64_t first_tile, int64_t n_tiles, uint32_t* d_tiles,
-                                            scoary_stream_t stream) {
-  const char* what = "scoary_perm_generate_tiles_strata_range";
+extern "C++" {
+static int generate_tiles_strata(scoary_handle h, const uint32_t* d_masks, const uint16_t* d_strata,
+                                 const int32_t* d_members, const int32_t* d_offsets, const int32_t* d_smargins,
+                                 int64_t T, int64_t N, int64_t S, int64_t P, int64_t perm_base, int64_t trait_base,
+                                 uint64_t seed, int64_t first_tile, int64_t n_tiles, uint32_t* d_tiles,
+                                 bool fragments, void* d_bfrag, scoary_stream_t stream) {
+  const char* what = fragments ? "scoary_perm_generate_tiles_strata_bfrag_range"
+                               : "scoary_perm_generate_tiles_strata_range";
   if (!h) return SCOARY_ERR_ARG;
   if (int rc = strata_check(h, what, d_masks && d_strata && d_members && d_offsets && d_smargins && d_tiles &&
                                          P >= 1 && perm_base >= 0 && trait_base >= 0 && first_tile >= 0 &&
-                                         n_tiles >= 0, T, N, S))
+                                         n_tiles >= 0 && (d_bfrag || !fragments), T, N, S))
     return rc;
   if (int rc = check_tile_base(h, what, perm_base)) return rc;
   if (trait_base + T > 0x7fffffffLL || perm_base + P > 0xffffffffLL)
-    return fail(h, SCOARY_ERR_SIZE, "scoary_perm_generate_tiles_strata_range: permutation index >= 2^32");
+    return fail(h, SCOARY_ERR_SIZE, std::string(what) + ": permutation index >= 2^32");
+  if (fragments)
+    if (int rc = check_bfrag_shape(h, what, N, 32)) return rc;
   TileShape ts;
   if (int rc = tile_shape(h, what, T, N, P, first_tile, n_tiles, 32,
                           [&](int nb) { return strata_lds(N, nb, S); }, ts))
@@ -786,10 +856,31 @@
   DeviceGuard guard(h->device);
   hipStream_t s = static_cast<hipStream_t>(stream);
   LabelArgs a = label_args(d_masks, nullptr, N, P, perm_base, trait_base, seed, 32, d_tiles);
-  tile_args(a, ts, first_tile, n_tiles);
+  tile_args(a, ts, first_tile, n_tiles, d_bfrag);
   const StrataArgs sa{d_strata, d_members, d_offsets, d_smargins, (int)S};
   KernelTimer kt(h, s, "k_perm_generate_tiles_strata");
-  return launch_labels_strata(h, s, a, sa, ts.NB, 0, dim3((unsigned)ts.gx), ts.tpb);
-}
-
-}
+  return launch_labels_strata(h, s, a, sa, ts.NB, fragments ? 2 : 0, dim3((unsigned)ts.gx), ts.tpb);
+}
+}
+
+int scoary_perm_generate_tiles_strata_range(scoary_handle h, const uint32_t* d_masks, const uint16_t* d_strata,
+                                            const int32_t* d_members, const int32_t* d_offsets,
+                                            const int32_t* d_smargins, int64_t T, int64_t N, int64_t S, int64_t P,
+                                            int64_t perm_base, int64_t trait_base, uint64_t seed,
+                                            int64_t first_tile, int64_t n_tiles, uint32_t* d_tiles,
+                                            scoary_stream_t stream) {
+  return generate_tiles_strata(h, d_masks, d_strata, d_members, d_offsets, d_smargins, T, N, S, P, perm_base,
+                               trait_base, seed, first_tile, n_tiles, d_tiles, false, nullptr, stream);
+}
+
+int scoary_perm_generate_tiles_strata_bfrag_range(scoary_handle h, const uint32_t* d_masks, const uint16_t* d_strata,
+                                                  const int32_t* d_members, const int32_t* d_offsets,
+                                                  const int32_t* d_smargins, int64_t T, int64_t N, int64_t S,
+                                                  int64_t P, int64_t perm_base, int64_t trait_base, uint64_t seed,
+                                                  int64_t first_tile, int64_t n_tiles, uint32_t* d_tiles,
+                                                  void* d_bfrag, scoary_stream_t stream) {
+  return generate_tiles_strata(h, d_masks, d_strata, d_members, d_offsets, d_smargins, T, N, S, P, perm_base,
+                               trait_base, seed, first_tile, n_tiles, d_tiles, true, d_bfrag, stream);
+}
+
+}
diff --git a/scoary_amd/csrc/scoary_lists.hip b/scoary_amd/csrc/scoary_lists.hip
--- a/scoary_amd/csrc/scoary_lists.hip
+++ b/scoary_amd/csrc/scoary_lists.hip
@@ -444,7 +444,7 @@
                         const uint8_t* d_lflipped, const uint32_t* d_crit, const uint32_t* d_lcrit_in,
                         const int32_t* d_margins, uint32_t* d_scratch, int64_t G, int64_t T, int64_t N,
                         int64_t P, uint32_t* d_r, int accumulate, const void* d_panels, void* d_bfrag,
-                        int64_t k_split, int64_t routed_entries, Extra... extra) {
+                        int64_t k_split, int64_t routed_entries, bool bfrag_ready, Extra... extra) {
   uint32_t* d_lcrit_sc = d_scratch;
   uint16_t* d_partial = reinterpret_cast<uint16_t*>(d_scratch + 2 * T * G);
   const uint32_t* d_lcrit = d_lcrit_in ? d_lcrit_in : d_lcrit_sc;
@@ -459,7 +459,7 @@
   const ListGeom g = list_geom(h->num_cu, G, T, N, P, entries - routed_entries, q_first);
   if (k_split > 0) {
     const int rc = scoary_mfma_launch(h, s, d_tiles, d_panels, d_bfrag, d_lcrit, d_partial, k_split, G, T, N, P,
-                                      g.ntiles, g.gs);
+                                      g.ntiles, g.gs, bfrag_ready);
     if (rc != SCOARY_OK) return rc;
   }
   if (T * g.ntiles > 0x7fffffffLL || g.chunks > 65535)
@@ -515,7 +515,21 @@
                           void* d_scratch, int64_t G, int64_t T, int64_t N, int64_t P,
                           uint32_t* d_r, int accumulate, const void* d_panels, void* d_bfrag,
                           int64_t k_split, int64_t routed_entries, scoary_stream_t stream) {
+  return scoary_permute_hybrid_bfrag(h, d_tiles, d_lidx, entries, d_lstart, d_lngroups, d_lorder, d_lflipped, d_crit,
+                                     d_lcrit, d_margins, d_scratch, G, T, N, P, d_r, accumulate, d_panels, d_bfrag,
+                                     k_split, routed_entries, 0, stream);
+}
+
+int scoary_permute_hybrid_bfrag(scoary_handle h, const uint32_t* d_tiles, const uint32_t* d_lidx,
+                                int64_t entries, const int32_t* d_lstart, const int32_t* d_lngroups,
+                                const int32_t* d_lorder, const uint8_t* d_lflipped,
+                                const uint32_t* d_crit, const uint32_t* d_lcrit, const int32_t* d_margins,
+                                void* d_scratch, int64_t G, int64_t T, int64_t N, int64_t P,
+                                uint32_t* d_r, int accumulate, const void* d_panels, void* d_bfrag,
+                                int64_t k_split, int64_t routed_entries, int bfrag_ready, scoary_stream_t stream) {
   if (!h) return SCOARY_ERR_ARG;
+  if (bfrag_ready != 0 && bfrag_ready != 1)
+    return fail(h, SCOARY_ERR_ARG, "scoary_permute_hybrid_bfrag: bfrag_ready is 0 or 1");
   if (k_split < 0 || k_split > G || routed_entries < 0 || routed_entries > entries ||
       (k_split > 0 && (!d_panels || !d_bfrag || N > scoary_mfma_max_isolates() ||
                        (k_split % 256 != 0 && k_split != G))))
@@ -534,12 +548,13 @@
   if (list_segments(N) > 1)
     return launch_lists(h, s, &k_permute_seglists<16>, "k_permute_seglists", (size_t)kSegStride * sizeof(uint32_t),
                         32, d_tiles, d_lidx, entries, d_lstart, d_lngroups, d_lorder, d_lflipped, d_crit, d_lcrit,
-                        d_margins, sc, G, T, N, P, d_r, accumulate, nullptr, nullptr, 0, 0, list_segments(N));
+                        d_margins, sc, G, T, N, P, d_r, accumulate, nullptr, nullptr, 0, 0, false, list_segments(N));
 #define LAUNCH(TWV, KCV)                                                                             \
   return launch_lists(h, s, &k_permute_lists<list_lpg(TWV), list_nw(TWV), KCV>, "k_permute_lists",  \
                       (size_t)list_tile_dwords(N, TWV) * sizeof(uint32_t), TWV, d_tiles, d_lidx,     \
                       entries, d_lstart, d_lngroups, d_lorder, d_lflipped, d_crit, d_lcrit, d_margins, \
                       sc, G, T, N, P, d_r, accumulate, d_panels, d_bfrag, k_split, routed_entries,       \
+                      bfrag_ready != 0,                                                              \
                       (int)((k_split + kWave / list_lpg(TWV) - 1) / (kWave / list_lpg(TWV))))
   if (TW == 16) LAUNCH(16, 11);
   if (TW == 8) LAUNCH(8, 12);
diff --git a/scoary_amd/csrc/scoary_mfma.hip b/scoary_amd/csrc/scoary_mfma.hip
--- a/scoary_amd/csrc/scoary_mfma.hip
+++ b/scoary_amd/csrc/scoary_mfma.hip
@@ -8,14 +8,10 @@
 namespace {
 
 typedef int v8i __attribute__((ext_vector_type(8)));
-typedef int v4i __attribute__((ext_vector_type(4)));
 typedef float v16f __attribute__((ext_vector_type(16)));
 
-constexpr int kKSteps = 32;
 constexpr int kBlockGenes = 256;
 constexpr int kBlockWaves = 8;
-constexpr int kFragBytes = 1024;
-constexpr int kStageBytes = 2 * kKSteps * kFragBytes;
 constexpr int kHalfBytes = kStageBytes / 2;
 constexpr int kRingSlots = 4;
 constexpr int kAhead = kRingSlots - 2;
@@ -25,16 +21,6 @@
 constexpr int kMfmaLds = kRingBytes + kBlockWaves * kThrBytes;
 static_assert(kRingSlots >= 4 && kMfmaLds <= 160 * 1024 && (kAhead - 1) * kDmaPerHalf < 64,
               "a half stage is issued at least two ticks ahead, within the LDS of a CU and the vmcnt field");
-
-__device__ __forceinline__ uint32_t fp4_of_bits8(uint32_t b) {
-  uint32_t y = b | (b << 12);
-  y = (y | (y << 6)) & 0x03030303u;
-  return __builtin_amdgcn_perm(0u, 0x22200200u, y);
-}
-__device__ __forceinline__ v4i fp4_of_bits32(uint32_t w) {
-  return v4i{(int)fp4_of_bits8(w & 0xffu), (int)fp4_of_bits8((w >> 8) & 0xffu),
-             (int)fp4_of_bits8((w >> 16) & 0xffu), (int)fp4_of_bits8(w >> 24)};
-}
 
 __global__ __launch_bounds__(256) void k_mfma_panels(const uint32_t* __restrict__ tiled, int64_t Gp, int G, int N,
                                                      const int32_t* __restrict__ order,
@@ -60,26 +46,11 @@
 __global__ __launch_bounds__(256) void k_mfma_bfrag(const uint32_t* __restrict__ tiles, int N, int ntiles,
                                                     int64_t tile_dwords, int S, v4i* __restrict__ bfrag) {
   const int s = blockIdx.x, t = blockIdx.y;
-  const int lane = threadIdx.x & 63, wave = threadIdx.x >> 6;
+  const int wave = __builtin_amdgcn_readfirstlane(threadIdx.x >> 6);
   const uint32_t* tile = tiles + ((int64_t)t * ntiles + (s >> 3)) * tile_dwords + 2 * (s & 7);
-  v4i* out = bfrag + ((int64_t)t * S + s) * (kStageBytes / 16);
-  for (int k = wave; k < kKSteps; k += 4) {
-    const int row = k * 64 + lane;
-    uint2 w = make_uint2(0u, 0u);
-    if (row < N) w = *reinterpret_cast<const uint2*>(tile + (int64_t)row * 16);
-#pragma unroll
-    for (int j = 0; j < 2; ++j) {
-      const uint32_t x = j ? w.y : w.x;
-      uint32_t mine = 0u;
-#pragma unroll
-      for (int c = 0; c < 32; ++c) {
-        const uint64_t bal = __ballot((x >> c) & 1u);
-        const uint32_t v = (lane >> 5) ? (uint32_t)(bal >> 32) : (uint32_t)bal;
-        if ((lane & 31) == c) mine = v;
-      }
-      out[(k * 2 + j) * 64 + lane] = fp4_of_bits32(mine);
-    }
-  }
+#pragma unroll
+  for (int j = 0; j < 2; ++j)
+    mfma_bfrag_emit(bfrag, S, t, s, j, wave, 4, [&](int row) { return row < N ? tile[(int64_t)row * 16 + j] : 0u; });
 }
 
 __device__ __forceinline__ void mfma_dma16(uint32_t lds, uint32_t lane_off, const unsigned char* src) {
@@ -326,7 +297,7 @@
 
 int scoary_mfma_launch(scoary_handle h, hipStream_t s, const uint32_t* d_tiles, const void* d_panels, void* d_bfrag,
                        const uint32_t* d_lcrit, uint16_t* d_partial, int64_t k_split, int64_t G, int64_t T,
-                       int64_t N, int64_t P, int64_t ntiles, int64_t gs) {
+                       int64_t N, int64_t P, int64_t ntiles, int64_t gs, bool bfrag_ready) {
   const MfmaGeom g = scoary_mfma_geom(h->num_cu, k_split, T, P, ntiles);
   if (g.blocks > 0x7fffffffLL || g.stages > 0x7fffffffLL / 64)
     return fail(h, SCOARY_ERR_SIZE, "scoary_permute_hybrid: grid too large");
@@ -335,7 +306,7 @@
                                    hipFuncAttributeMaxDynamicSharedMemorySize, 160 * 1024));
     h->mfma_lds_optin = 1;
   }
-  {
+  if (!bfrag_ready) {
     KernelTimer kt(h, s, "k_mfma_bfrag");
     hipLaunchKernelGGL(k_mfma_bfrag, dim3((unsigned)g.stages, (unsigned)T), dim3(256), 0, s, d_tiles, (int)N,
                        (int)ntiles, list_tile_dwords(N, 16), (int)g.stages, static_cast<v4i*>(d_bfrag));
diff --git a/scoary_amd/engine.py b/scoary_amd/engine.py
--- a/scoary_amd/engine.py
+++ b/scoary_amd/engine.py
@@ -189,6 +189,7 @@
             raise _abi.ScoaryHipError("scoary_create(device=%d) failed: %d" % (self.device.index, rc))
         self.h = h
         self.label_shards = None
+        self.fuse_bfrag = True
 
     def close(self):
         if getattr(self, "h", None):
@@ -349,12 +350,26 @@
         return int(N) <= int(self.lib.scoary_list_max_isolates())
 
     def perm_generate_tiles(self, masks, margins, N, P, perm_base, seed, out=None, trait_base=0,
-                            tile_range=None, strata=None):
+                            tile_range=None, strata=None, bfrag=None):
         torch = _torch()
         T = masks.shape[0]
         if out is None:
             out = self._empty((int(self.lib.scoary_list_tiles_words(N, P, T)),), torch.int32)
-        if strata is not None:
+        if bfrag is not None:
+            if tile_range is None:
+                tile_range = (0, self.tiles_per_batch(N, P, T)[0])
+            if strata is not None:
+                self._strata_fits(strata, T, N)
+                self._check(self.lib.scoary_perm_generate_tiles_strata_bfrag_range(
+                    self.h, self._ptr(masks), *self._strata_ptrs(strata), T, N, strata.S, P, perm_base, trait_base,
+                    ctypes.c_uint64(seed), int(tile_range[0]), int(tile_range[1]), self._ptr(out), self._ptr(bfrag),
+                    self._stream()), "scoary_perm_generate_tiles_strata_bfrag_range")
+            else:
+                self._check(self.lib.scoary_perm_generate_tiles_bfrag_range(
+                    self.h, self._ptr(masks), self._ptr(margins), T, N, P, perm_base, trait_base,
+                    ctypes.c_uint64(seed), int(tile_range[0]), int(tile_range[1]), self._ptr(out), self._ptr(bfrag),
+                    self._stream()), "scoary_perm_generate_tiles_bfrag_range")
+        elif strata is not None:
             self._strata_fits(strata, T, N)
             if tile_range is None:
                 tile_range = (0, self.tiles_per_batch(N, P, T)[0])
@@ -383,7 +398,7 @@
         return self._empty(((nbytes + 3) // 4,), torch.int32)
 
     def permute_lists(self, genes, tiles, crit, margins, P, r, scratch=None, lcrit=None,
-                      accumulate=True, bfrag=None):
+                      accumulate=True, bfrag=None, bfrag_ready=False):
         L = genes.lists
         T = (lcrit if lcrit is not None else crit).shape[0]
         if scratch is None:
@@ -394,15 +409,15 @@
             if bfrag is None:
                 bfrag = self._empty((int(self.lib.scoary_mfma_bfrag_bytes(genes.N, P, T)) // 4,), _torch().int32)
             routed = int(L.block_start[-1 if k_split >= genes.G else k_split // 256])
-        self._check(self.lib.scoary_permute_hybrid(
+        self._check(self.lib.scoary_permute_hybrid_bfrag(
             self.h, self._ptr(tiles), self._ptr(L.idx), L.entries, self._ptr(L.start),
             self._ptr(L.ngroups), self._ptr(L.order), self._ptr(L.flipped),
             self._ptr(crit) if lcrit is None else None,
             self._ptr(lcrit) if lcrit is not None else None,
             self._ptr(margins), self._ptr(scratch), genes.G, T, genes.N, P, self._ptr(r),
             1 if accumulate else 0, self._ptr(L.panels) if k_split > 0 else None,
-            self._ptr(bfrag) if k_split > 0 else None, k_split, routed, self._stream()),
-            "scoary_permute_hybrid")
+            self._ptr(bfrag) if k_split > 0 else None, k_split, routed, 1 if bfrag_ready and k_split > 0 else 0,
+            self._stream()), "scoary_permute_hybrid_bfrag")
         return r
 
     def trait_plan(self, traits, masks, N, out=None):
@@ -945,7 +960,7 @@
             ((L.panels,) if L is not None and L.panels is not None else ()) + \
             ((strata, strata.strata, strata.members, strata.offsets, strata.smargins) if strata is not None else ())
         scalars = (genes.G, genes.N, int(traits.shape[0]), int(permutations), int(seed), bool(use_lists),
-                   getattr(self, "_mfma_mode", "auto"), strata is not None,
+                   getattr(self, "_mfma_mode", "auto"), bool(self.fuse_bfrag), strata is not None,
                    tuple(getattr(x, "_version", 0) for x in refs))
         st = ws.auto
         same = st is not None and st["scalars"] == scalars and len(st["refs"]) == len(refs) and \
@@ -963,16 +978,20 @@
         st["graph"].launch()
         return st["res"]
 
-    def _label_tiles(self, ws, masks, margins, N, nb, base, seed, strata=None):
+    def _label_tiles(self, ws, masks, margins, N, nb, base, seed, strata=None, genes=None):
         sh = ws.label_shards
         if sh is None or sh.world == 1:
-            self.perm_generate_tiles(masks, margins, N, nb, base, seed, out=ws.tiles, strata=strata)
-            return
+            fuse = self.fuse_bfrag and ws.bfrag is not None and genes is not None and \
+                N <= int(self.lib.scoary_mfma_max_isolates()) and self.mfma_split(genes, masks.shape[0], nb) > 0
+            self.perm_generate_tiles(masks, margins, N, nb, base, seed, out=ws.tiles, strata=strata,
+                                     bfrag=ws.bfrag if fuse else None)
+            return fuse
         nflat, tile_words = self.tiles_per_batch(N, nb, masks.shape[0])
         _per, first, count = sh.share(nflat)
         self.perm_generate_tiles(masks, margins, N, nb, base, seed, out=ws.tiles,
                                  tile_range=(first, count), strata=strata)
         sh.all_gather(ws.tiles, nflat, tile_words)
+        return False
 
     def associate(self, genes, traits, masks, permutations=0, seed=0, perm_buffer=None,
                   use_lists=None, workspace=None, plan=None, graph=None, records=None, fwer=False,
@@ -1046,7 +1065,8 @@
             side = self._side_stream()
             side.wait_stream(main)
             with torch.cuda.stream(side):
-                self._label_tiles(ws, masks, margins, genes.N, min(ws.batch, permutations), 0, seed, strata)
+                ready = self._label_tiles(ws, masks, margins, genes.N, min(ws.batch, permutations), 0, seed, strata,
+                                          genes)
             p, odds, crit, lcrit = self.fisher(counts, out=(ws.p, ws.odds, ws.crit),
                                                lists=genes.lists, lcrit=ws.lcrit)
         else:
@@ -1061,10 +1081,10 @@
             while done < permutations:
                 nb = min(ws.batch, permutations - done)
                 if done > 0:
-                    self._label_tiles(ws, masks, margins, genes.N, nb, done, seed, strata)
+                    ready = self._label_tiles(ws, masks, margins, genes.N, nb, done, seed, strata, genes)
                 for regions, r in counted:
                     self.permute_lists(genes, ws.tiles, margins=margins, P=nb, r=r, scratch=ws.scratch,
-                                       accumulate=done > 0, bfrag=ws.bfrag, **regions)
+                                       accumulate=done > 0, bfrag=ws.bfrag, bfrag_ready=ready, **regions)
                 done += nb
         elif permutations > 0:
             ws.r.zero_()
```

Result: faster. 1973 billion tests/s, median of 6 (+1.7%).
